# michael-fonder/M4Depth

Measured on AMD Instinct MI355X. Metric: frames/s, higher is better.
Workload: dtype f32

## Files before the change

include/m4depth_hip.h:

```cpp
#ifndef M4DEPTH_HIP_H_
#define M4DEPTH_HIP_H_

#include <stdint.h>

#ifdef __cplusplus
extern "C" {
#endif

#define M4D_ABI_VERSION 6

int m4d_abi_version(void);
long long m4d_launch_count(void);
const char* m4d_build_info(void);


int m4d_backproject_fwd(const float* input, const float* coords, const int dims[6],
                        float* out, void* stream);

int m4d_backproject_bwd(const float* grad, const float* input, const float* coords,
                        const int dims[6], float* input_grad, float* coords_grad, void* stream);


int m4d_dense_image_warp(const float* image, const float* flow, int B, int H, int W, int C,
                         float* out, int32_t* index_out, void* stream);

int m4d_interpolate_bilinear(const float* grid, const float* query, int B, int H, int W, int C,
                             int N, float* out, int32_t* index_out, void* stream);


int m4d_parallax2depth(const float* disp, const float* rot, int rot_c, const float* trans,
                       const float* cam_f, const float* cam_c, int b, int h, int w,
                       float* out, void* stream);
int m4d_depth2parallax(const float* depth, const float* rot, int rot_c, const float* trans,
                       const float* cam_f, const float* cam_c, int b, int h, int w,
                       float* out, void* stream);
int m4d_prev_d2para(const float* prev_d, const float* rot, int rot_c, const float* trans,
                    const float* cam_f, const float* cam_c, int b, int h, int w,
                    float* out, void* stream);
int m4d_reproject_flow(const float* depth, const float* rot, int rot_c, const float* trans,
                       const float* cam_f, const float* cam_c, int b, int h, int w,
                       float* flow, float* proj_minus_rot, float* rot_coord, void* stream);
int m4d_recompute_depth(const float* depth, const float* rot, int rot_c, const float* trans,
                        const float* cam_f, const float* cam_c, int b, int h, int w,
                        float* out, void* stream);


int m4d_dscv_fwd(const float* c1, const float* c2, const float* disp_prev_t, const float* disp,
                 const float* rot, int rot_c, const float* trans, const float* cam_f,
                 const float* cam_c, int b, int h, int w, int C, int search_range, int nbre_cuts,
                 int cv_accum, float* cv, int cv_stride, float* prev_disp,
                 float* log_center, int log_stride, float log_scale,
                 int32_t* index_out, void* stream);

void m4d_dscv_set_variant(int variant);
void m4d_dscv_set_fallback_counter(unsigned int* device_counter);
void m4d_dscv_set_ablation(int mask);
void m4d_dscv_set_stamps(unsigned long long* device_buffer);

int m4d_sncv_fwd(const float* c1, const float* c2, int b, int h, int w, int C, int search_range,
                 int dilation_rate, int nbre_cuts, float* out, int out_stride, void* stream);
int m4d_dscv_sncv_fwd(const float* c1, const float* c2, const float* disp_prev_t, const float* disp,
                      const float* rot, int rot_c, const float* trans, const float* cam_f,
                      const float* cam_c, int b, int h, int w, int C, int search_range, int nbre_cuts,
                      int cv_accum, float* cv, int cv_stride, float* prev_disp,
                      float* log_center, int log_stride, float log_scale,
                      int sncv_search_range, float* sncv_out, int sncv_out_stride, void* stream);

int m4d_conv3x3_wino_bias_act(const float* x, const float* wu, const float* bias, int b, int h, int w,
                              int Cin, int Cout, int CoutPad, float slope, float* out, void* stream);
int m4d_conv3x3_wino2_bias_act(const float* x, const float* wu8, const float* bias, int b, int h, int w,
                               int Cin, int Cout, int CoutPad, float slope, float* out, void* stream);
void m4d_wino_set_stamps(unsigned long long* device_buffer);
int m4d_conv3x3_wino6_bias_act(const float* x, const void* wu6, const float* bias, int b, int h, int w,
                               int Cin, int Cout, int CoutPad, float slope, float* out, void* stream);
int m4d_conv3x3_wino6_bias_act_k(const float* x, const void* wu6, const float* bias, int b, int h, int w,
                                 int Cin, int Cout, int CoutPad, float slope, float* out, int kernel, void* stream);
long long m4d_wino6_persistent_min_units(void);
void m4d_wino6_set_stamps(unsigned long long* device_buffer);
int m4d_conv3x3_wino6_bias_act_ks(const float* x, const void* wu6, const float* bias, int b, int h, int w,
                                  int Cin, int Cout, int CoutPad, float slope, float* out, int kernel,
                                  int stagger_us, int stagger_phases, void* stream);

int m4d_refiner_tail(const float* x32, const float* w6p, const float* b6, const float* w7p, const float* b7,
                     const float* rot, int rot_c, const float* trans, const float* cam_f, const float* cam_c,
                     int b, int h, int w, float scale, float* parallax, float* depth, float* other,
                     float* depth_state, void* stream);
int m4d_refiner_tail6(const float* x32, const void* w6f, const float* b6, const void* w7f, const float* b7,
                      const float* rot, int rot_c, const float* trans, const float* cam_f, const float* cam_c,
                      int b, int h, int w, float scale, float* parallax, float* depth, float* other,
                      float* depth_state, void* stream);

int m4d_refiner_tail6_m(const float* x32, const void* w6f, const float* b6, const void* w7f, const float* b7,
                        const float* rot, int rot_c, const float* trans, const float* cam_f, const float* cam_c,
                        int b, int h, int w, float scale, float* parallax, float* depth, float* other,
                        float* depth_state, const unsigned char* reset, float reset_parallax, void* stream);
int m4d_refiner_tail_m(const float* x32, const float* w6p, const float* b6, const float* w7p, const float* b7,
                       const float* rot, int rot_c, const float* trans, const float* cam_f, const float* cam_c,
                       int b, int h, int w, float scale, float* parallax, float* depth, float* other,
                       float* depth_state, const unsigned char* reset, float reset_parallax, void* stream);
int m4d_level_post_m(const float* refiner_out, const float* rot, int rot_c, const float* trans,
                     const float* cam_f, const float* cam_c, int b, int h, int w, float scale,
                     float* parallax, float* depth, float* other, float* depth_state,
                     const unsigned char* reset, float reset_parallax, void* stream);
int m4d_stream_prepare(const unsigned char* new_traj, int force_all, const float* rot, int rot_c, const float* trans,
                       int b, unsigned char* reset, float* rot_out, float* trans_out, void* stream);


int m4d_dscv_bwd(const float* c1, const float* c2, const float* disp_prev_t, const float* disp,
                 const float* rot, int rot_c, const float* trans, const float* cam_f,
                 const float* cam_c, int b, int h, int w, int C, int search_range, int nbre_cuts,
                 const float* g_cv, int g_cv_stride, const float* g_prev_disp,
                 float* g_c1, float* g_c2, float* g_disp, float* g_disp_prev_t, void* stream);

int m4d_sncv_bwd(const float* c1, const float* c2, const float* out, int out_stride,
                 const float* g, int g_stride, int b, int h, int w, int C, int search_range,
                 int dilation_rate, int nbre_cuts, float slope, float* g_c1, float* g_c2,
                 void* stream);


int m4d_resize_bilinear_v1_bwd(const float* g_out, int b, int ih, int iw, int c, int oh, int ow,
                               float mul, float* g_in, void* stream);
int m4d_level_post_bwd(const float* refiner_out, const float* g_parallax, const float* g_depth,
                       const float* g_other, const float* rot, int rot_c, const float* trans,
                       const float* cam_f, const float* cam_c, int b, int h, int w, float scale,
                       float* g_refiner_out, void* stream);
int m4d_normalize_cuts_bwd(const float* x, const float* g, int b, int h, int w, int C, int nbre_cuts,
                           float* g_x, void* stream);
long long m4d_bias_act_bwd_workspace_floats(long long rows, int C);
int m4d_bias_act_bwd(const float* g, const float* out, long long rows, int C, float slope,
                     float* g_pre, float* g_bias, float* workspace, void* stream);
int m4d_pack_conv_weights(const float* w_ohwi, int O, int I, int transpose, float* wp, void* stream);
int m4d_pack_conv_weights_lat(const float* w_ohwi, int O, int I, int transpose, void* wp, void* stream);
long long m4d_loss_workspace_floats(void);
int m4d_loss_level_fwd(const float* pred_depth, const float* gt_depth, int b, int h, int w, int H, int W,
                       int velodyne, float* workspace, float* out2, void* stream);
int m4d_loss_level_bwd(const float* pred_depth, const float* gt_depth, const float* stats2,
                       const float* g_out, int b, int h, int w, int H, int W, int velodyne,
                       float* g_pred, void* stream);


int m4d_normalize_cuts(const float* x, int b, int h, int w, int C, int nbre_cuts,
                       float* out, void* stream);

int m4d_resize_bilinear_v1(const float* x, int b, int ih, int iw, int c, int oh, int ow,
                           float mul, float* out, void* stream);
int m4d_resize_nearest(const float* x, int b, int ih, int iw, int c, int oh, int ow,
                       float* out, void* stream);

int m4d_level_pre(const float* prev_l_depth, const float* prev_l_parallax, const float* prev_l_other,
                  int ph, int pw, const float* depth_prev_t, const float* trans,
                  const float* cam_f, const float* cam_c, int b, int h, int w,
                  float* para_prev_l, float* depth_prev_l, float* other_prev_l, float* para_prev_t,
                  float* f_input, int f_stride, int log_off, int other_off, float log_scale,
                  float* depth_state_reset, void* stream);
int m4d_level_pre_normalize(const float* prev_l_depth, const float* prev_l_parallax, const float* prev_l_other,
                            int ph, int pw, const float* depth_prev_t, const float* trans,
                            const float* cam_f, const float* cam_c, int b, int h, int w,
                            float* para_prev_l, float* depth_prev_l, float* other_prev_l, float* para_prev_t,
                            float* f_input, int f_stride, int log_off, int other_off, float log_scale,
                            float* depth_state_reset,
                            const float* norm_x, int C, int nbre_cuts, float* norm_out, void* stream);

typedef struct m4d_reset_level {
  const float* features;
  float* state_features;
  float* depth_state;
  float* parallax;
  float* depth;
  float* other;
  int h, w, C, nbre_cuts;
  float parallax_value;
} m4d_reset_level;
int m4d_pyramid_reset_supported(int C, int nbre_cuts);
int m4d_pyramid_reset(const m4d_reset_level* levels, int n_levels, int b, void* stream);

typedef struct { const float* x; float* out; long long pixels; int C, nbre_cuts; } m4d_norm_level;
int m4d_normalize_levels(const m4d_norm_level* levels, int n_levels, void* stream);
int m4d_level_front_small_supported(int C, int nbre_cuts, int dscv_range, int sncv_range);
int m4d_level_front_small(const float* norm_f, const float* prev_f, const float* depth_prev_t,
                          const float* prev_l_parallax, const float* prev_l_other, int ph, int pw,
                          const float* rot, int rot_c, const float* trans, const float* cam_f, const float* cam_c,
                          int b, int h, int w, int C, int nbre_cuts, int dscv_range, int sncv_range, int cv_accum,
                          float* f_input, int f_stride, float log_scale, void* stream);

int m4d_level_front_supported(int C, int nbre_cuts, int dscv_range, int sncv_range, int f_stride);
void m4d_front_set_stamps(unsigned long long* device_buffer);
int m4d_level_front(const float* raw_f, float* norm_out, const float* prev_f, const float* depth_prev_t,
                    const float* prev_l_parallax, const float* prev_l_other, int ph, int pw,
                    const float* rot, int rot_c, const float* trans, const float* cam_f, const float* cam_c,
                    int b, int h, int w, int C, int nbre_cuts, int cv_accum,
                    float* f_input, int f_stride, float log_scale, void* stream);
int m4d_level_front_r(const float* raw_f, float* norm_out, const float* prev_f, const float* depth_prev_t,
                      const float* prev_l_parallax, const float* prev_l_other, int ph, int pw,
                      const float* rot, int rot_c, const float* trans, const float* cam_f, const float* cam_c,
                      int b, int h, int w, int C, int nbre_cuts, int dscv_range, int sncv_range, int cv_accum,
                      float* f_input, int f_stride, float log_scale, void* stream);

int m4d_camera_pyramid(const float* cam_f, const float* cam_c, int b, int levels, float* f_out, float* c_out,
                       void* stream);

int m4d_level_post(const float* refiner_out, const float* rot, int rot_c, const float* trans,
                   const float* cam_f, const float* cam_c, int b, int h, int w, float scale,
                   float* parallax, float* depth, float* other, float* depth_state, void* stream);

int m4d_bias_act(const float* x, const float* bias, long long rows, int C, float slope,
                 float* out, void* stream);

int m4d_bias_act_padded(const float* x, const float* bias, int b, int h, int w, int C, float slope,
                        float* out, int out_h, int out_w, int off_y, int off_x, void* stream);

int m4d_conv3x3_bias_act(const float* x, const float* wp, const float* bias, int b, int h, int w,
                         int Cin, int Cout, int CoutPad, float slope, float* out, void* stream);
long long m4d_conv3x3_workspace_floats(int b, int h, int w, int CoutPad);
int m4d_conv3x3s_bias_act_ws(const float* x, const float* wp, const float* bias, int b, int h, int w,
                             int Cin, int Cout, int CoutPad, int stride, float slope, float* out,
                             float* workspace, long long workspace_floats, void* stream);
int m4d_conv3x3_bias_act_ws(const float* x, const float* wp, const float* bias, int b, int h, int w,
                            int Cin, int Cout, int CoutPad, float slope, float* out, float* workspace,
                            long long workspace_floats, void* stream);
int m4d_conv3x3_lat(const float* x, int s_in, long long x_slab_floats, const float* x_bias, float x_slope,
                    const void* wp, const float* bias, int b, int h, int w, int Cin, int Cout, float slope,
                    int mt, int kw, int s_out, float* out, long long out_slab_floats, void* stream);
int m4d_conv3x3s_lat(const float* x, int s_in, long long x_slab_floats, const float* x_bias, float x_slope,
                     const void* wp, const float* bias, int b, int h, int w, int Cin, int Cout, int stride, float slope,
                     int mt, int kw, int s_out, float* out, long long out_slab_floats, void* stream);
int m4d_partial_finish(const float* x, int s_in, long long x_slab_floats, const float* bias, float slope,
                       long long pixels, int C, float* out, void* stream);

int m4d_conv3x3_small_bias_act(const float* x, const float* wp, const float* bias, int b, int h, int w,
                               int Cin, int Cout, int CoutPad, float slope, float* out, void* stream);
int m4d_conv3x3s_small_bias_act(const float* x, const float* wp, const float* bias, int b, int h, int w,
                                int Cin, int Cout, int CoutPad, int stride, float slope, float* out, void* stream);
int m4d_conv3x3_small6_bias_act(const float* x, const void* wp6, const float* bias, int b, int h, int w,
                                int Cin, int Cout, int CoutPad, float slope, float* out, void* stream);

long long m4d_dinl_workspace_floats(int b, int C);
int m4d_dinl_fwd_padded(const float* x, const float* scale, const float* bias, int b, int h, int w, int C,
                        float slope, float* workspace, float* out, int out_h, int out_w, int off_y,
                        int off_x, void* stream);
int m4d_dinl_fwd(const float* x, const float* scale, const float* bias, int b, int h, int w, int C,
                 float slope, float* workspace, float* out, void* stream);

int m4d_enc_level0_fwd(const float* images, int bsz, long long stride_b, long long stride_t,
                       const float* w1_hwio, const float* bias1, const float* dn_scale, const float* dn_bias,
                       float dn_slope, const float* w2_hwio, const float* bias2, float slope,
                       int b, int h, int w, float* workspace, float* out, void* stream);
int m4d_enc_level0_stats(const float* images, int bsz, long long stride_b, long long stride_t,
                         const float* w1_hwio, const float* bias1, int b, int h, int w, float* workspace,
                         float* mean, float* var, void* stream);
int m4d_enc_level0_apply(const float* images, int bsz, long long stride_b, long long stride_t,
                         const float* w1_hwio, const float* bias1, const float* mean, const float* var,
                         const float* dn_scale, const float* dn_bias, float dn_slope, const float* w2_hwio,
                         const float* bias2, float slope, int b, int h, int w, float* out, void* stream);
int m4d_enc_head_fwd(const float* images, int bsz, long long stride_b, long long stride_t,
                     const float* w_hwio, const float* bias, int b, int h, int w, int C,
                     float* workspace, float* raw_out, void* stream);
int m4d_conv3x3s2_dinl_bias_act(const float* x_raw, const float* mean, const float* var, const float* dn_scale,
                                const float* dn_bias, float dn_slope, const float* wp, const float* bias,
                                int b, int h, int w, int Cout, int CoutPad, float slope, float* out, void* stream);

long long m4d_metrics_workspace_bytes(void);
int m4d_depth_metrics(const float* gt, const float* est, long long n, float max_d, void* workspace,
                      float* out7, float* total7, float count, float* mean7, void* stream);
int m4d_depth_metrics_strided(const float* gt, long long per_image, long long gt_image_stride, const float* est,
                              long long n, float max_d, void* workspace, float* out7, float* total7, float count,
                              float* mean7, void* stream);


long long m4d_conv3x3_wgrad_workspace_floats(int b, int h, int w, int cin, int cout, int stride);
int m4d_conv3x3_wgrad(const float* x, const float* g, int b, int h, int w, int cin, int cout, int stride,
                      float* workspace, long long workspace_floats, float* dw, void* stream);
int m4d_dilate2(const float* g, int b, int oh, int ow, int C, int h, int w, float* out, void* stream);


int m4d_decode_rgb8_resize(const uint8_t* images, int n, int ih, int iw, int oh, int ow, float* out,
                           void* stream);
int m4d_decode_depth_resize(const void* raw, int kind, int n, int ih, int iw, int oh, int ow,
                            const float* rgb_resized, const int crop[4], float* out, void* stream);

#ifdef __cplusplus
}
#endif
#endif
```

m4depth_amd/_lib.py:

```python
from __future__ import annotations

import ctypes
import os

import torch

_HERE = os.path.dirname(os.path.abspath(__file__))
LIB_FLAVOUR = os.environ.get("M4D_LIB_FLAVOUR", "product")
LIB_PATH = os.path.join(_HERE, "libm4depth_hip_exp.so" if LIB_FLAVOUR == "experiments" else "libm4depth_hip.so")

ABI_VERSION = 6

_c_fp = ctypes.c_void_p
_c_int = ctypes.c_int
_c_f = ctypes.c_float

class NormLevel(ctypes.Structure):
    _fields_ = [("x", ctypes.c_void_p), ("out", ctypes.c_void_p), ("pixels", ctypes.c_longlong), ("C", ctypes.c_int),
                ("nbre_cuts", ctypes.c_int)]


class ResetLevel(ctypes.Structure):
    _fields_ = [("features", ctypes.c_void_p), ("state_features", ctypes.c_void_p), ("depth_state", ctypes.c_void_p),
                ("parallax", ctypes.c_void_p), ("depth", ctypes.c_void_p), ("other", ctypes.c_void_p),
                ("h", ctypes.c_int), ("w", ctypes.c_int), ("C", ctypes.c_int), ("nbre_cuts", ctypes.c_int),
                ("parallax_value", ctypes.c_float)]


_SIGNATURES = {
    "m4d_backproject_fwd": [_c_fp, _c_fp, ctypes.POINTER(_c_int), _c_fp, _c_fp],
    "m4d_backproject_bwd": [_c_fp, _c_fp, _c_fp, ctypes.POINTER(_c_int), _c_fp, _c_fp, _c_fp],
    "m4d_dense_image_warp": [_c_fp, _c_fp, _c_int, _c_int, _c_int, _c_int, _c_fp, _c_fp, _c_fp],
    "m4d_interpolate_bilinear": [_c_fp, _c_fp, _c_int, _c_int, _c_int, _c_int, _c_int, _c_fp, _c_fp, _c_fp],
    "m4d_parallax2depth": [_c_fp, _c_fp, _c_int, _c_fp, _c_fp, _c_fp, _c_int, _c_int, _c_int, _c_fp, _c_fp],
    "m4d_depth2parallax": [_c_fp, _c_fp, _c_int, _c_fp, _c_fp, _c_fp, _c_int, _c_int, _c_int, _c_fp, _c_fp],
    "m4d_prev_d2para": [_c_fp, _c_fp, _c_int, _c_fp, _c_fp, _c_fp, _c_int, _c_int, _c_int, _c_fp, _c_fp],
    "m4d_recompute_depth": [_c_fp, _c_fp, _c_int, _c_fp, _c_fp, _c_fp, _c_int, _c_int, _c_int, _c_fp, _c_fp],
    "m4d_reproject_flow": [_c_fp, _c_fp, _c_int, _c_fp, _c_fp, _c_fp, _c_int, _c_int, _c_int, _c_fp, _c_fp, _c_fp, _c_fp],
    "m4d_dscv_fwd": [_c_fp, _c_fp, _c_fp, _c_fp, _c_fp, _c_int, _c_fp, _c_fp, _c_fp,
                     _c_int, _c_int, _c_int, _c_int, _c_int, _c_int, _c_int,
                     _c_fp, _c_int, _c_fp, _c_fp, _c_int, _c_f, _c_fp, _c_fp],
    "m4d_dscv_sncv_fwd": [_c_fp, _c_fp, _c_fp, _c_fp, _c_fp, _c_int, _c_fp, _c_fp, _c_fp,
                          _c_int, _c_int, _c_int, _c_int, _c_int, _c_int, _c_int,
                          _c_fp, _c_int, _c_fp, _c_fp, _c_int, _c_f, _c_int, _c_fp, _c_int, _c_fp],
    "m4d_sncv_fwd": [_c_fp, _c_fp, _c_int, _c_int, _c_int, _c_int, _c_int, _c_int, _c_int, _c_fp, _c_int, _c_fp],
    "m4d_dscv_bwd": [_c_fp, _c_fp, _c_fp, _c_fp, _c_fp, _c_int, _c_fp, _c_fp, _c_fp,
                     _c_int, _c_int, _c_int, _c_int, _c_int, _c_int,
                     _c_fp, _c_int, _c_fp, _c_fp, _c_fp, _c_fp, _c_fp, _c_fp],
    "m4d_sncv_bwd": [_c_fp, _c_fp, _c_fp, _c_int, _c_fp, _c_int, _c_int, _c_int, _c_int, _c_int, _c_int, _c_int,
                     _c_int, _c_f, _c_fp, _c_fp, _c_fp],
    "m4d_resize_bilinear_v1_bwd": [_c_fp, _c_int, _c_int, _c_int, _c_int, _c_int, _c_int, _c_f, _c_fp, _c_fp],
    "m4d_level_post_bwd": [_c_fp, _c_fp, _c_fp, _c_fp, _c_fp, _c_int, _c_fp, _c_fp, _c_fp, _c_int, _c_int, _c_int, _c_f,
                           _c_fp, _c_fp],
    "m4d_normalize_cuts_bwd": [_c_fp, _c_fp, _c_int, _c_int, _c_int, _c_int, _c_int, _c_fp, _c_fp],
    "m4d_bias_act_bwd": [_c_fp, _c_fp, ctypes.c_longlong, _c_int, _c_f, _c_fp, _c_fp, _c_fp, _c_fp],
    "m4d_pack_conv_weights": [_c_fp, _c_int, _c_int, _c_int, _c_fp, _c_fp],
    "m4d_pack_conv_weights_lat": [_c_fp, _c_int, _c_int, _c_int, _c_fp, _c_fp],
    "m4d_loss_level_fwd": [_c_fp, _c_fp, _c_int, _c_int, _c_int, _c_int, _c_int, _c_int, _c_fp, _c_fp, _c_fp],
    "m4d_loss_level_bwd": [_c_fp, _c_fp, _c_fp, _c_fp, _c_int, _c_int, _c_int, _c_int, _c_int, _c_int, _c_fp, _c_fp],
    "m4d_decode_rgb8_resize": [_c_fp, _c_int, _c_int, _c_int, _c_int, _c_int, _c_fp, _c_fp],
    "m4d_decode_depth_resize": [_c_fp, _c_int, _c_int, _c_int, _c_int, _c_int, _c_int, _c_fp, ctypes.POINTER(_c_int),
                                _c_fp, _c_fp],
    "m4d_normalize_cuts": [_c_fp, _c_int, _c_int, _c_int, _c_int, _c_int, _c_fp, _c_fp],
    "m4d_resize_bilinear_v1": [_c_fp, _c_int, _c_int, _c_int, _c_int, _c_int, _c_int, _c_f, _c_fp, _c_fp],
    "m4d_resize_nearest": [_c_fp, _c_int, _c_int, _c_int, _c_int, _c_int, _c_int, _c_fp, _c_fp],
    "m4d_bias_act": [_c_fp, _c_fp, ctypes.c_longlong, _c_int, _c_f, _c_fp, _c_fp],
    "m4d_dinl_fwd": [_c_fp, _c_fp, _c_fp, _c_int, _c_int, _c_int, _c_int, _c_f, _c_fp, _c_fp, _c_fp],
    "m4d_dinl_fwd_padded": [_c_fp, _c_fp, _c_fp, _c_int, _c_int, _c_int, _c_int, _c_f, _c_fp, _c_fp,
                            _c_int, _c_int, _c_int, _c_int, _c_fp],
    "m4d_bias_act_padded": [_c_fp, _c_fp, _c_int, _c_int, _c_int, _c_int, _c_f, _c_fp, _c_int, _c_int, _c_int, _c_int, _c_fp],
    "m4d_conv3x3_bias_act": [_c_fp, _c_fp, _c_fp, _c_int, _c_int, _c_int, _c_int, _c_int, _c_int, _c_f, _c_fp, _c_fp],
    "m4d_conv3x3_bias_act_ws": [_c_fp, _c_fp, _c_fp, _c_int, _c_int, _c_int, _c_int, _c_int, _c_int, _c_f, _c_fp,
                                _c_fp, ctypes.c_longlong, _c_fp],
    "m4d_conv3x3s_bias_act_ws": [_c_fp, _c_fp, _c_fp, _c_int, _c_int, _c_int, _c_int, _c_int, _c_int, _c_int, _c_f,
                                 _c_fp, _c_fp, ctypes.c_longlong, _c_fp],
    "m4d_conv3x3_small_bias_act": [_c_fp, _c_fp, _c_fp, _c_int, _c_int, _c_int, _c_int, _c_int, _c_int, _c_f, _c_fp, _c_fp],
    "m4d_conv3x3s_small_bias_act": [_c_fp, _c_fp, _c_fp, _c_int, _c_int, _c_int, _c_int, _c_int, _c_int, _c_int, _c_f, _c_fp, _c_fp],
    "m4d_conv3x3_small6_bias_act": [_c_fp, _c_fp, _c_fp, _c_int, _c_int, _c_int, _c_int, _c_int, _c_int, _c_f, _c_fp, _c_fp],
    "m4d_conv3x3_lat": [_c_fp, _c_int, ctypes.c_longlong, _c_fp, _c_f, _c_fp, _c_fp, _c_int, _c_int, _c_int, _c_int, _c_int, _c_f,
                        _c_int, _c_int, _c_int, _c_fp, ctypes.c_longlong, _c_fp],
    "m4d_conv3x3s_lat": [_c_fp, _c_int, ctypes.c_longlong, _c_fp, _c_f, _c_fp, _c_fp, _c_int, _c_int, _c_int, _c_int, _c_int, _c_int,
                         _c_f, _c_int, _c_int, _c_int, _c_fp, ctypes.c_longlong, _c_fp],
    "m4d_partial_finish": [_c_fp, _c_int, ctypes.c_longlong, _c_fp, _c_f, ctypes.c_longlong, _c_int, _c_fp, _c_fp],
    "m4d_conv3x3_wino_bias_act": [_c_fp, _c_fp, _c_fp, _c_int, _c_int, _c_int, _c_int, _c_int, _c_int, _c_f, _c_fp, _c_fp],
    "m4d_conv3x3_wino2_bias_act": [_c_fp, _c_fp, _c_fp, _c_int, _c_int, _c_int, _c_int, _c_int, _c_int, _c_f, _c_fp, _c_fp],
    "m4d_conv3x3_wino6_bias_act": [_c_fp, _c_fp, _c_fp, _c_int, _c_int, _c_int, _c_int, _c_int, _c_int, _c_f, _c_fp, _c_fp],
    "m4d_conv3x3_wino6_bias_act_k": [_c_fp, _c_fp, _c_fp, _c_int, _c_int, _c_int, _c_int, _c_int, _c_int, _c_f, _c_fp, _c_int, _c_fp],
    "m4d_conv3x3_wino6_bias_act_ks": [_c_fp, _c_fp, _c_fp, _c_int, _c_int, _c_int, _c_int, _c_int, _c_int, _c_f, _c_fp, _c_int,
                                      _c_int, _c_int, _c_fp],
    "m4d_enc_head_fwd": [_c_fp, _c_int, ctypes.c_longlong, ctypes.c_longlong, _c_fp, _c_fp, _c_int, _c_int, _c_int, _c_int,
                         _c_fp, _c_fp, _c_fp],
    "m4d_enc_level0_stats": [_c_fp, _c_int, ctypes.c_longlong, ctypes.c_longlong, _c_fp, _c_fp, _c_int, _c_int, _c_int, _c_fp, _c_fp, _c_fp,
                             _c_fp],
    "m4d_enc_level0_apply": [_c_fp, _c_int, ctypes.c_longlong, ctypes.c_longlong, _c_fp, _c_fp, _c_fp, _c_fp, _c_fp, _c_fp, _c_f, _c_fp,
                             _c_fp, _c_f, _c_int, _c_int, _c_int, _c_fp, _c_fp],
    "m4d_enc_level0_fwd": [_c_fp, _c_int, ctypes.c_longlong, ctypes.c_longlong, _c_fp, _c_fp, _c_fp, _c_fp, _c_f, _c_fp, _c_fp, _c_f,
                           _c_int, _c_int, _c_int, _c_fp, _c_fp, _c_fp],
    "m4d_conv3x3s2_dinl_bias_act": [_c_fp, _c_fp, _c_fp, _c_fp, _c_fp, _c_f, _c_fp, _c_fp, _c_int, _c_int, _c_int, _c_int, _c_int,
                                    _c_f, _c_fp, _c_fp],
    "m4d_refiner_tail": [_c_fp, _c_fp, _c_fp, _c_fp, _c_fp, _c_fp, _c_int, _c_fp, _c_fp, _c_fp, _c_int, _c_int, _c_int, _c_f,
                         _c_fp, _c_fp, _c_fp, _c_fp, _c_fp],
    "m4d_refiner_tail6": [_c_fp, _c_fp, _c_fp, _c_fp, _c_fp, _c_fp, _c_int, _c_fp, _c_fp, _c_fp, _c_int, _c_int, _c_int, _c_f,
                          _c_fp, _c_fp, _c_fp, _c_fp, _c_fp],
    "m4d_depth_metrics": [_c_fp, _c_fp, ctypes.c_longlong, _c_f, _c_fp, _c_fp, _c_fp, _c_f, _c_fp, _c_fp],
    "m4d_depth_metrics_strided": [_c_fp, ctypes.c_longlong, ctypes.c_longlong, _c_fp, ctypes.c_longlong, _c_f, _c_fp, _c_fp, _c_fp,
                                  _c_f, _c_fp, _c_fp],
    "m4d_level_pre": [_c_fp, _c_fp, _c_fp, _c_int, _c_int, _c_fp, _c_fp, _c_fp, _c_fp, _c_int, _c_int, _c_int,
                      _c_fp, _c_fp, _c_fp, _c_fp, _c_fp, _c_int, _c_int, _c_int, _c_f, _c_fp, _c_fp],
    "m4d_level_pre_normalize": [_c_fp, _c_fp, _c_fp, _c_int, _c_int, _c_fp, _c_fp, _c_fp, _c_fp, _c_int, _c_int, _c_int,
                                _c_fp, _c_fp, _c_fp, _c_fp, _c_fp, _c_int, _c_int, _c_int, _c_f, _c_fp,
                                _c_fp, _c_int, _c_int, _c_fp, _c_fp],
    "m4d_level_front_supported": [_c_int, _c_int, _c_int, _c_int, _c_int],
    "m4d_pyramid_reset_supported": [_c_int, _c_int],
    "m4d_pyramid_reset": [ctypes.POINTER(ResetLevel), _c_int, _c_int, _c_fp],
    "m4d_normalize_levels": [ctypes.POINTER(NormLevel), _c_int, _c_fp],
    "m4d_level_front_small_supported": [_c_int, _c_int, _c_int, _c_int],
    "m4d_level_front_small": [_c_fp, _c_fp, _c_fp, _c_fp, _c_fp, _c_int, _c_int, _c_fp, _c_int, _c_fp, _c_fp, _c_fp,
                              _c_int, _c_int, _c_int, _c_int, _c_int, _c_int, _c_int, _c_int, _c_fp, _c_int, _c_f, _c_fp],
    "m4d_level_front": [_c_fp, _c_fp, _c_fp, _c_fp, _c_fp, _c_fp, _c_int, _c_int, _c_fp, _c_int, _c_fp, _c_fp, _c_fp,
                        _c_int, _c_int, _c_int, _c_int, _c_int, _c_int, _c_fp, _c_int, _c_f, _c_fp],
    "m4d_level_front_r": [_c_fp, _c_fp, _c_fp, _c_fp, _c_fp, _c_fp, _c_int, _c_int, _c_fp, _c_int, _c_fp, _c_fp, _c_fp,
                          _c_int, _c_int, _c_int, _c_int, _c_int, _c_int, _c_int, _c_int, _c_fp, _c_int, _c_f, _c_fp],
    "m4d_conv3x3_wgrad": [_c_fp, _c_fp, _c_int, _c_int, _c_int, _c_int, _c_int, _c_int, _c_fp, ctypes.c_longlong, _c_fp, _c_fp],
    "m4d_dilate2": [_c_fp, _c_int, _c_int, _c_int, _c_int, _c_int, _c_int, _c_fp, _c_fp],
    "m4d_camera_pyramid": [_c_fp, _c_fp, _c_int, _c_int, _c_fp, _c_fp, _c_fp],
    "m4d_level_post": [_c_fp, _c_fp, _c_int, _c_fp, _c_fp, _c_fp, _c_int, _c_int, _c_int, _c_f,
                       _c_fp, _c_fp, _c_fp, _c_fp, _c_fp],
    "m4d_refiner_tail_m": [_c_fp, _c_fp, _c_fp, _c_fp, _c_fp, _c_fp, _c_int, _c_fp, _c_fp, _c_fp, _c_int, _c_int, _c_int, _c_f,
                           _c_fp, _c_fp, _c_fp, _c_fp, _c_fp, _c_f, _c_fp],
    "m4d_refiner_tail6_m": [_c_fp, _c_fp, _c_fp, _c_fp, _c_fp, _c_fp, _c_int, _c_fp, _c_fp, _c_fp, _c_int, _c_int, _c_int, _c_f,
                            _c_fp, _c_fp, _c_fp, _c_fp, _c_fp, _c_f, _c_fp],
    "m4d_level_post_m": [_c_fp, _c_fp, _c_int, _c_fp, _c_fp, _c_fp, _c_int, _c_int, _c_int, _c_f,
                         _c_fp, _c_fp, _c_fp, _c_fp, _c_fp, _c_f, _c_fp],
    "m4d_stream_prepare": [_c_fp, _c_int, _c_fp, _c_int, _c_fp, _c_int, _c_fp, _c_fp, _c_fp, _c_fp],
}

_EXPERIMENT_SIGNATURES = {"m4d_tape_begin": [], "m4d_tape_end": [], "m4d_tape_length": [_c_int], "m4d_tape_replay": [_c_int, _c_fp],
                          "m4d_tape_free": [_c_int]}
_EXPERIMENT_VOID_SIGNATURES = {"m4d_wino6_set_variant": [_c_int], "m4d_wino6_set_half_tile_max_workgroups": [_c_int]}
EXPERIMENT_SYMBOLS = list(_EXPERIMENT_SIGNATURES) + list(_EXPERIMENT_VOID_SIGNATURES)

_LL_SIGNATURES = {"m4d_launch_count": [], "m4d_wino6_persistent_min_units": [], "m4d_conv3x3_workspace_floats": [_c_int, _c_int, _c_int, _c_int],
                  "m4d_dinl_workspace_floats": [_c_int, _c_int], "m4d_metrics_workspace_bytes": [],
                  "m4d_bias_act_bwd_workspace_floats": [ctypes.c_longlong, _c_int], "m4d_loss_workspace_floats": [],
                  "m4d_conv3x3_wgrad_workspace_floats": [_c_int, _c_int, _c_int, _c_int, _c_int, _c_int]}
_VOID_SIGNATURES = {"m4d_dscv_set_variant": [_c_int], "m4d_dscv_set_fallback_counter": [_c_fp],
                    "m4d_dscv_set_ablation": [_c_int], "m4d_dscv_set_stamps": [_c_fp], "m4d_wino_set_stamps": [_c_fp],
                    "m4d_front_set_stamps": [_c_fp], "m4d_wino6_set_stamps": [_c_fp]}

EXPORTED_SYMBOLS = ["m4d_abi_version", "m4d_build_info"] + list(_SIGNATURES) + list(_VOID_SIGNATURES) + list(_LL_SIGNATURES)


def _load():
    if not os.path.isfile(LIB_PATH):
        raise ImportError(
            f"m4depth_amd: native library not found at {LIB_PATH}. Build it with "
            "`python -c 'import __graft_entry__ as g; g.build()'` or `make -C m4depth_amd/csrc`. "
            "There is no CPU / PyTorch fallback for the hot path.")
    lib = ctypes.CDLL(LIB_PATH)
    lib.m4d_abi_version.restype = _c_int
    lib.m4d_abi_version.argtypes = []
    lib.m4d_build_info.restype = ctypes.c_char_p
    lib.m4d_build_info.argtypes = []
    for name, args in _SIGNATURES.items():
        fn = getattr(lib, name)
        fn.restype = _c_int
        fn.argtypes = args
    for name, args in _LL_SIGNATURES.items():
        fn = getattr(lib, name)
        fn.restype = ctypes.c_longlong
        fn.argtypes = args
    for name, args in _VOID_SIGNATURES.items():
        fn = getattr(lib, name)
        fn.restype = None
        fn.argtypes = args
    if hasattr(lib, "m4d_tape_begin"):
        for name, args in _EXPERIMENT_SIGNATURES.items():
            fn = getattr(lib, name)
            fn.restype = _c_int
            fn.argtypes = args
        for name, args in _EXPERIMENT_VOID_SIGNATURES.items():
            fn = getattr(lib, name)
            fn.restype = None
            fn.argtypes = args
    if lib.m4d_abi_version() != ABI_VERSION:
        raise ImportError(f"m4depth_amd: ABI mismatch, library reports {lib.m4d_abi_version()}, binding expects {ABI_VERSION}")
    return lib


lib = _load()
has_experiments = hasattr(lib, "m4d_tape_begin")


def require_experiments(what):
    if not has_experiments:
        raise RuntimeError(f"{what} needs the experiments build of the library: make -C m4depth_amd/csrc EXPERIMENTS=1 "
                           "(-> libm4depth_hip_exp.so, sources in tools/experiments/csrc) and M4D_LIB_FLAVOUR=experiments in "
                           "the environment; the product library exports only the kernels it dispatches")


def build_info() -> str:
    return lib.m4d_build_info().decode()


def stream_ptr():
    return ctypes.c_void_p(torch.cuda.current_stream().cuda_stream)


def dptr(t, name="tensor", dtype=torch.float32):
    if t is None:
        return None
    if not isinstance(t, torch.Tensor):
        raise TypeError(f"{name}: expected a torch.Tensor, got {type(t).__name__}")
    if not t.is_cuda:
        raise RuntimeError(f"{name}: m4depth_amd ops run on the MI355X only (tensor is on {t.device}); "
                           "there is no CPU fallback")
    if t.dtype != dtype:
        raise TypeError(f"{name}: expected dtype {dtype}, got {t.dtype}")
    if not t.is_contiguous():
        raise ValueError(f"{name}: expected a dense row-major (NHWC) tensor, got strides {t.stride()}")
    return ctypes.c_void_p(t.data_ptr())


def check(rc, what):
    if rc != 0:
        raise RuntimeError(f"m4depth_amd: {what} failed with HIP error {rc}"
                           + (" (hipErrorInvalidValue: bad argument)" if rc == 1 else ""))


_capture_copies_ok = [False]


class framework_copies_in_capture:
    def __enter__(self):
        self._old = _capture_copies_ok[0]
        _capture_copies_ok[0] = True
        return self

    def __exit__(self, *exc):
        _capture_copies_ok[0] = self._old
        return False


def as_f32(t, name):
    if not isinstance(t, torch.Tensor):
        raise TypeError(f"{name}: expected a torch.Tensor")
    if t.dtype == torch.float32 and t.is_contiguous():
        return t
    if t.is_cuda and not _capture_copies_ok[0] and torch.cuda.is_current_stream_capturing():
        raise RuntimeError(f"{name}: a non-contiguous / non-float32 tensor (shape {tuple(t.shape)}, strides {t.stride()}, "
                           f"{t.dtype}) reached a kernel wrapper inside a hipGraph capture; it would be copied by a framework "
                           "kernel inside the graph -- make it dense before capturing")
    if t.dtype != torch.float32:
        t = t.float()
    return t if t.is_contiguous() else t.contiguous()
```

m4depth_amd/network.py:

```python
from __future__ import annotations

import ctypes
from collections import namedtuple

import numpy as np
import torch

from . import network_ops as nops
from ._lib import lib, dptr, stream_ptr, check, as_f32
from .synthetic import ENCODER_CHANNELS, REFINER_CHANNELS, f_input_channels, nbre_cuts_for

M4depthAblationParameters = namedtuple('M4depthAblationParameters',
                                       ('DINL', 'SNCV', 'time_recurr', 'normalize_features',
                                        'subdivide_features', 'level_memory'),
                                       defaults=(True, True, True, True, True, True))

_CV_ACCUM = {"fp32_round": 0, "fp16_seq": 1}

import os as _os

kernel_timer = None
debug_tap = None
winograd_conv = _os.environ.get("M4D_WINOGRAD", "1") == "1"


winograd2_min_workgroups = int(_os.environ.get("M4D_WINO2_MIN_WG", "60"))


conv_arith = _os.environ.get("M4D_CONV_ARITH", "bf16x3")
wino6_min_workgroups = int(_os.environ.get("M4D_WINO6_MIN_WG", "30"))
wino6_kernel = int(_os.environ.get("M4D_WINO6_KERNEL", "0"))
wino6_pair_min_units = int(_os.environ.get("M4D_WINO6_PAIR_MIN_UNITS", "0"))
wino6_pair_units = int(_os.environ.get("M4D_WINO6_PAIR_UNITS", "2"))
wino6_min_cout = int(_os.environ.get("M4D_WINO6_MIN_COUT", "32"))
if _os.environ.get("M4D_WINO6_VARIANT") or _os.environ.get("M4D_WINO6_HALF_MAX_WG"):
    from ._lib import require_experiments as _require_experiments
    _require_experiments("M4D_WINO6_VARIANT / M4D_WINO6_HALF_MAX_WG")
    if _os.environ.get("M4D_WINO6_VARIANT"):
        lib.m4d_wino6_set_variant(int(_os.environ["M4D_WINO6_VARIANT"]))
    if _os.environ.get("M4D_WINO6_HALF_MAX_WG"):
        lib.m4d_wino6_set_half_tile_max_workgroups(int(_os.environ["M4D_WINO6_HALF_MAX_WG"]))
_small_conv_split_env = _os.environ.get("M4D_SMALL_CONV_SPLIT", "1") == "1"
small_conv_split = _small_conv_split_env and conv_arith == "bf16x3"


tail_split = _os.environ.get("M4D_TAIL_SPLIT", "1") == "1"

encoder_batch_dispatch = _os.environ.get("M4D_ENCODER_BATCH_DISPATCH", "1") == "1"

import contextlib as _contextlib


@_contextlib.contextmanager
def conv_arithmetic(arith):
    global conv_arith, small_conv_split
    if arith not in ("bf16x3", "f32"):
        raise ValueError(f"conv arithmetic must be 'bf16x3' or 'f32', not {arith!r}")
    old = (conv_arith, small_conv_split)
    conv_arith, small_conv_split = arith, _small_conv_split_env and arith == "bf16x3"
    try:
        yield
    finally:
        conv_arith, small_conv_split = old


def _use_winograd(b, h, w, cin, cout, stride):
    if not winograd_conv or stride != 1 or cin < 16 or cin % 2 != 0:
        return 0
    n32 = -(-cout // 32)
    t16 = b * (-(-h // 16)) * (-(-w // 16))
    if conv_arith == "bf16x3" and cin % 16 == 0 and cin >= 32 and cout >= wino6_min_cout and t16 * (-(-cout // 64)) >= wino6_min_workgroups:
        return 6
    if cin % 4 == 0 and t16 * n32 >= winograd2_min_workgroups:
        return 2
    t8 = b * (-(-h // 8)) * (-(-w // 16))
    if cout % 64 == 0 and t8 * (cout // 64) >= 400:
        return 1
    if cout >= 96 and 400 <= t8 * n32 <= 3000:
        return 1
    return 0


pad_refiner_input = _os.environ.get("M4D_PAD_REFINER_INPUT", "1") == "1"

small_map_conv_pixels = int(_os.environ.get("M4D_CONV_SMALL_PX", "2048"))
small_map_stride2 = _os.environ.get("M4D_CONV_SMALL_S2", "1") == "1"

lat_conv_max_pixels = int(_os.environ.get("M4D_LAT_CONV_PX", "2048"))
lat_conv_narrow_max_pixels = int(_os.environ.get("M4D_LAT_CONV_NARROW_PX", "0"))
lat_conv_s2_max_pixels = int(_os.environ.get("M4D_LAT_CONV_S2_PX", "0"))
lat_conv_mw_max_pixels = int(_os.environ.get("M4D_LAT_CONV_MW_PX", "0"))

fused_cost_volumes = _os.environ.get("M4D_FUSED_COST_VOLUMES", "1") == "1"
small_level_front = _os.environ.get("M4D_SMALL_LEVEL_FRONT", "1") == "1"
fused_level_front = _os.environ.get("M4D_FUSED_LEVEL_FRONT", "1") == "1"

fused_front = _os.environ.get("M4D_FUSED_FRONT", "1") == "1"
fused_front_min_pixels = int(_os.environ.get("M4D_FUSED_FRONT_MIN_PX", "0"))
fused_front_coarse_min_pixels = int(_os.environ.get("M4D_FUSED_FRONT_COARSE_MIN_PX", "6000"))

fused_encoder_head = _os.environ.get("M4D_FUSED_ENCODER_HEAD", "1") == "1"

fused_refiner_tail = _os.environ.get("M4D_FUSED_TAIL", "1") == "1"

level_pipeline_streams = int(_os.environ.get("M4D_LEVEL_PIPELINE", "8"))
_pf = _os.environ.get("M4D_PIPE_FORK_FRAMES", "1,2")
pipeline_fork_frames = None if _pf == "all" else {int(v) for v in _pf.split(",") if v.strip() != ""}
pipeline_skip_implied_encoder_wait = _os.environ.get("M4D_PIPE_SKIP_ENC_WAIT", "1") == "1"
pipeline_merge_reset_frame = _os.environ.get("M4D_PIPE_MERGE_RESET", "1") == "1"
wino6_stagger_us = int(_os.environ.get("M4D_WINO6_STAGGER_US", "9"))
wino6_stagger_phases = int(_os.environ.get("M4D_WINO6_STAGGER_PHASES", "16"))
wino6_stagger_min_wg = int(_os.environ.get("M4D_WINO6_STAGGER_MIN_WG", "200"))
wino6_stagger_max_batch = int(_os.environ.get("M4D_WINO6_STAGGER_MAX_BATCH", "4"))
wino6_stagger_autotune = _os.environ.get("M4D_STAGGER_AUTOTUNE", "1") == "1"
segmented_step = _os.environ.get("M4D_SEGMENTED", "0") == "1"
segmented_resumed_first = _os.environ.get("M4D_SEG_RESUMED_FIRST", "1") == "1"
segmented_resumed_on_main = _os.environ.get("M4D_SEG_RESUMED_ON_MAIN", "0") == "1"
wino6_stagger_force = _os.environ.get("M4D_STAGGER_FORCE", "")
fused_pyramid_reset = _os.environ.get("M4D_FUSED_RESET", "1") == "1"
fused_encoder_level0 = _os.environ.get("M4D_FUSED_ENC0", "1") == "1"
pipeline_encoder_per_frame = _os.environ.get("M4D_PIPELINE_ENCODER", "0") == "1"
pipeline_encoder_split = int(_os.environ.get("M4D_PIPELINE_ENCODER_SPLIT", "2"))
encoder_stats_up_front = _os.environ.get("M4D_ENC_STATS_UP_FRONT", "1") == "1"
encoder_s1_partial_always = _os.environ.get("M4D_ENC_S1_PARTIAL", "0") == "1"


def _stack_frames(samples):
    ims = [s['RGB_im'] for s in samples]
    x0 = ims[0]
    if (x0.is_cuda and x0.dtype == torch.float32 and x0.dim() == 4 and x0[0].is_contiguous()
            and all(x.dtype == x0.dtype and x.shape == x0.shape and x.stride() == x0.stride()
                    and x.untyped_storage().data_ptr() == x0.untyped_storage().data_ptr() for x in ims)):
        if len(ims) == 1:
            return nops.FrameStack(x0.unsqueeze(1))
        st = ims[1].storage_offset() - x0.storage_offset()
        if st > 0 and all(ims[t].storage_offset() - x0.storage_offset() == t * st for t in range(len(ims))):
            b, h, w, c = x0.shape
            return nops.FrameStack(torch.as_strided(x0, (b, len(ims), h, w, c), (x0.stride(0), st, w * c, c, 1),
                                                    x0.storage_offset()))
    return torch.cat([as_f32(x, "RGB_im") for x in ims], dim=0)


def _timed(name, level, thunk):
    kt = kernel_timer
    return thunk() if kt is None else kt.run(name, level, thunk)


def _to_device_f32(x, device):
    if isinstance(x, torch.Tensor):
        return x.to(device=device, dtype=torch.float32)
    return torch.as_tensor(np.asarray(x), dtype=torch.float32, device=device)


def _stamp(*params):
    return tuple((p.data_ptr(), p._version, str(p.device)) for p in params)


class _PackCache:

    def __init__(self):
        self.entries = {}

    def get(self, key, stamp, build):
        hit = self.entries.get(key)
        if hit is not None and hit[0] == stamp:
            return hit[1]
        if torch.cuda.is_available() and torch.cuda.is_current_stream_capturing():
            raise RuntimeError("packed convolution weights are missing or stale inside a hipGraph capture: call "
                               "M4Depth.prepack() before capturing")
        fresh = build()
        if hit is not None:
            old = hit[1]
            olds, news = (old if isinstance(old, tuple) else (old,)), (fresh if isinstance(fresh, tuple) else (fresh,))
            if len(olds) == len(news) and all(isinstance(o, torch.Tensor) == isinstance(n, torch.Tensor) and (
                    not isinstance(o, torch.Tensor) or (o.shape == n.shape and o.device == n.device)) for o, n in zip(olds, news)):
                for o, n in zip(olds, news):
                    if isinstance(o, torch.Tensor):
                        o.copy_(n)
                fresh = old
        self.entries[key] = (stamp, fresh)
        return fresh

    def clear(self):
        self.entries.clear()


class _Conv3x3SameTF(torch.nn.Module):

    def __init__(self, out_channels, stride, in_channels=None):
        super().__init__()
        self.out_channels = out_channels
        self.stride = stride
        self.weight = None
        self.bias = None
        self._cache = _PackCache()
        self.tag = None
        self.small_maps_ok = False
        self.per_image_dispatch = False
        self.dispatch_batch = 1
        self.wino6_stagger_us = None
        if in_channels is not None:
            self._build(in_channels, None)

    def _build(self, in_channels, device):
        w = torch.empty(self.out_channels, in_channels, 3, 3, device=device)
        torch.nn.init.kaiming_normal_(w, nonlinearity='relu')
        self.weight = torch.nn.Parameter(w.contiguous(memory_format=torch.channels_last), requires_grad=False)
        self.bias = torch.nn.Parameter(torch.zeros(self.out_channels, device=device), requires_grad=False)
        self._cache.clear()

    def load_hwio(self, kernel, bias, device):
        w = _to_device_f32(kernel, device).permute(3, 2, 0, 1)
        b = _to_device_f32(bias, device).contiguous()
        if (self.weight is not None and self.bias is not None and self.weight.shape == w.shape and self.bias.shape == b.shape
                and self.weight.device == w.device):
            with torch.no_grad():
                self.weight.copy_(w)
                self.bias.copy_(b)
            return
        self.weight = torch.nn.Parameter(w.contiguous(memory_format=torch.channels_last), requires_grad=False)
        self.bias = torch.nn.Parameter(b, requires_grad=False)
        self._cache.clear()

    def invalidate_packed(self):
        with torch.no_grad():
            if self.weight is not None:
                self.weight.add_(0)

    def _hwio_numpy(self, cin_pad=None):
        hwio = self.weight.detach().permute(2, 3, 1, 0).cpu().numpy()
        if cin_pad is not None and cin_pad > hwio.shape[2]:
            hwio = np.concatenate([hwio, np.zeros(hwio.shape[:2] + (cin_pad - hwio.shape[2], hwio.shape[3]), hwio.dtype)], axis=2)
        return hwio

    def _packed_weights(self, cin_pad=None):
        if cin_pad is not None and cin_pad == self.weight.shape[1]:
            cin_pad = None

        def build():
            wp, cpad = nops.pack_conv_weights(self._hwio_numpy(cin_pad))
            return torch.from_numpy(wp).to(self.weight.device), cpad
        return self._cache.get(("direct", cin_pad), _stamp(self.weight), build)

    def _packed_weights_winograd(self, chunk=16, cin_pad=None):
        if cin_pad is not None and cin_pad == self.weight.shape[1]:
            cin_pad = None

        def build():
            wu, cpad = nops.pack_conv_weights_winograd(self._hwio_numpy(cin_pad), chunk=chunk)
            return torch.from_numpy(wu).to(self.weight.device), cpad
        return self._cache.get(("wino", chunk, cin_pad), _stamp(self.weight), build)

    def _packed_weights_small6(self, cin_pad=None):
        if cin_pad is not None and cin_pad == self.weight.shape[1]:
            cin_pad = None

        def build():
            wp, cpad = nops.pack_conv_weights_small6(self._hwio_numpy(cin_pad))
            return torch.from_numpy(wp.view("int16")).to(self.weight.device), cpad
        return self._cache.get(("small6", cin_pad), _stamp(self.weight), build)

    def _packed_weights_lat(self, cin_pad=None):
        if cin_pad is not None and cin_pad == self.weight.shape[1]:
            cin_pad = None

        def build():
            wp = nops.pack_conv_weights_lat(self._hwio_numpy(cin_pad))
            return torch.from_numpy(wp.view("int16")).to(self.weight.device)
        return self._cache.get(("lat", cin_pad), _stamp(self.weight), build)

    def lat_eligible(self, b, h, w, cin):
        if not (self.small_maps_ok and conv_arith == "bf16x3" and cin >= 16 and cin % 4 == 0 and self.stride in (1, 2)):
            return False
        eff_b = self.dispatch_batch if self.per_image_dispatch else b
        if self.stride == 2:
            opx = eff_b * (-(-h // 2)) * (-(-w // 2))
            return self._lat_mw(b, h, w, cin) or (small_map_stride2 and opx <= lat_conv_s2_max_pixels)
        limit = max(lat_conv_max_pixels, lat_conv_narrow_max_pixels) if self.out_channels <= 32 else lat_conv_max_pixels
        return eff_b * h * w <= limit

    def _lat_mw(self, b, h, w, cin):
        eff_b = self.dispatch_batch if self.per_image_dispatch else b
        return (self.stride == 2 and cin % 16 == 0 and cin <= 64 and self.out_channels <= 64
                and small_map_conv_pixels < eff_b * (-(-h // 2)) * (-(-w // 2)) <= lat_conv_mw_max_pixels)

    def _packed_weights_wino6(self, cin_pad=None):
        if cin_pad is not None and cin_pad == self.weight.shape[1]:
            cin_pad = None

        def build():
            wu, cpad = nops.pack_conv_weights_wino6(self._hwio_numpy(cin_pad))
            return torch.from_numpy(wu.view("int16")).to(self.weight.device), cpad
        return self._cache.get(("wino6", cin_pad), _stamp(self.weight), build)

    def _hwio_device(self):
        return self._cache.get(("hwio",), _stamp(self.weight), lambda: self.weight.detach().permute(2, 3, 1, 0).contiguous())

    def same_pads(self, h, w):
        s = self.stride
        ph = max((-(-h // s) - 1) * s + 3 - h, 0)
        pw = max((-(-w // s) - 1) * s + 3 - w, 0)
        return (ph // 2, ph - ph // 2), (pw // 2, pw - pw // 2)

    def launch_stagger_us(self, b, h, w):
        us = wino6_stagger_us if self.wino6_stagger_us is None else self.wino6_stagger_us
        if us <= 0 or b > wino6_stagger_max_batch:
            return 0
        units = b * (-(-h // 16)) * (-(-w // 16)) * (-(-self.out_channels // 64))
        return int(us) if units >= wino6_stagger_min_wg else 0

    def forward(self, x_nhwc, slope=None, final=True):
        if isinstance(x_nhwc, nops.PartialAct) and not self.lat_eligible(*x_nhwc.shape):
            x_nhwc = x_nhwc.dense()
        if not x_nhwc.is_cuda:
            raise RuntimeError("m4depth_amd convolutions run on the GPU only (libm4depth_hip.so): got a CPU tensor; "
                               "there is no CPU fallback")
        if self.weight is None:
            self._build(x_nhwc.shape[-1], x_nhwc.device)
        if self.stride not in (1, 2):
            raise ValueError(f"stride {self.stride} is not supported by the HIP convolution")
        b_, h_, w_, cin_ = x_nhwc.shape
        act = 1.0 if slope is None else slope
        eff_b = self.dispatch_batch if self.per_image_dispatch else b_
        if self.lat_eligible(b_, h_, w_, cin_):
            wl = self._packed_weights_lat(cin_)
            cfg = nops.lat_config(eff_b, h_, w_, cin_, self.out_channels, final, self.stride, mw=self._lat_mw(b_, h_, w_, cin_))
            return _timed("conv", self.tag, lambda: nops.conv3x3_lat(x_nhwc, wl, self.bias, self.out_channels, act, config=cfg,
                                                                     stride=self.stride))
        wino = _use_winograd(eff_b, h_, w_, cin_, self.out_channels, self.stride)
        if wino == 6:
            wu, cpad = self._packed_weights_wino6(cin_)
            stag = self.launch_stagger_us(b_, h_, w_)
            kern = wino6_kernel
            if kern == 0 and wino6_pair_min_units > 0 and b_ <= wino6_stagger_max_batch and cin_ >= 32:
                units = b_ * (-(-h_ // 16)) * (-(-w_ // 16)) * (cpad // 64)
                if wino6_pair_min_units <= units < int(lib.m4d_wino6_persistent_min_units()):
                    kern = 16 + max(1, min(wino6_pair_units, 15))
            return _timed("conv", self.tag, lambda: nops.conv3x3_wino6_bias_act(
                x_nhwc, wu, self.bias, self.out_channels, cpad, act, kernel=kern, stagger_us=stag,
                stagger_phases=wino6_stagger_phases))
        if wino:
            wu, cpad = self._packed_weights_winograd(16 if wino == 1 else 8, cin_)
            fn = nops.conv3x3_wino_bias_act if wino == 1 else nops.conv3x3_wino2_bias_act
            return _timed("conv", self.tag, lambda: fn(x_nhwc, wu, self.bias, self.out_channels, cpad, act))
        wp, cpad = self._packed_weights(cin_)
        if (self.small_maps_ok and self.stride == 1 and eff_b * h_ * w_ <= small_map_conv_pixels and 16 <= cin_ <= 256
                and cin_ % 4 == 0):
            if small_conv_split:
                wp6, cpad6 = self._packed_weights_small6(cin_)
                return _timed("conv", self.tag, lambda: nops.conv3x3_small6_bias_act(
                    x_nhwc, wp6, self.bias, self.out_channels, cpad6, act))
            return _timed("conv", self.tag, lambda: nops.conv3x3_small_bias_act(
                x_nhwc, wp, self.bias, self.out_channels, cpad, act))
        if (self.small_maps_ok and self.stride == 2 and small_map_stride2 and 16 <= cin_ <= 256 and cin_ % 4 == 0
                and eff_b * (-(-h_ // 2)) * (-(-w_ // 2)) <= small_map_conv_pixels):
            return _timed("conv", self.tag, lambda: nops.conv3x3_small_bias_act(
                x_nhwc, wp, self.bias, self.out_channels, cpad, act, stride=2))
        return _timed("conv", self.tag, lambda: nops.conv3x3_bias_act(
            x_nhwc, wp, self.bias, self.out_channels, cpad, act, stride=self.stride))


class DomainNormalization(torch.nn.Module):

    def __init__(self, regularizer_weight=0.0004):
        super().__init__()
        self.regularizer_weight = regularizer_weight
        self.scale = None
        self.bias = None

    def _build(self, channels, device):
        self.scale = torch.nn.Parameter(torch.ones(1, 1, 1, channels, device=device), requires_grad=False)
        self.bias = torch.nn.Parameter(torch.zeros(1, 1, 1, channels, device=device), requires_grad=False)

    def forward(self, f_map, slope=1.0):
        if self.scale is None:
            self._build(f_map.shape[-1], f_map.device)
        if not f_map.is_cuda:
            raise RuntimeError("m4depth_amd DomainNormalization runs on the GPU only (libm4depth_hip.so): got a CPU tensor; "
                               "there is no CPU fallback")
        if f_map.shape[-1] not in (16, 32):
            raise ValueError(f"DomainNormalization: the HIP kernel is instantiated for 16 and 32 channels, not {f_map.shape[-1]}")
        return nops.dinl_act(f_map, self.scale, self.bias, slope)


class FeaturePyramid(torch.nn.Module):

    def __init__(self, settings, regularizer_weight=0.0004, trainable=True):
        super().__init__()
        self.use_dinl = settings["ablation"].DINL
        self.out_sizes = ENCODER_CHANNELS[:settings["nbre_lvls"]]
        cin = [3] + self.out_sizes[:-1]
        self.conv_layers_s1 = torch.nn.ModuleList([_Conv3x3SameTF(n, 1, ci) for n, ci in zip(self.out_sizes, cin)])
        self.conv_layers_s2 = torch.nn.ModuleList([_Conv3x3SameTF(n, 2, n) for n in self.out_sizes])
        self.dn_layers = torch.nn.ModuleList([DomainNormalization(regularizer_weight) for _ in self.out_sizes])
        for conv in list(self.conv_layers_s1) + list(self.conv_layers_s2):
            conv.per_image_dispatch = True
            conv.small_maps_ok = True

    def set_sequence_batch(self, b):
        b = max(int(b), 1) if encoder_batch_dispatch else 1
        for conv in list(self.conv_layers_s1) + list(self.conv_layers_s2):
            conv.dispatch_batch = b

    def _head_ok(self, images):
        return (self.use_dinl and fused_encoder_head and images.is_cuda and images.shape[-1] == 3
                and self.conv_layers_s1[0].out_channels == 16 and self.conv_layers_s2[0].out_channels <= 32
                and self.conv_layers_s1[0].weight is not None)

    def head_stats(self, images):
        if not (self._head_ok(images) and fused_encoder_level0 and self.conv_layers_s2[0].out_channels == 16):
            return None
        conv_s1 = self.conv_layers_s1[0]
        return _timed("enc0_stats", 0, lambda: nops.encoder_level0_stats(images, conv_s1._hwio_device(), conv_s1.bias))

    def forward(self, images, head_stats=None):
        head_ok = self._head_ok(images)
        if isinstance(images, nops.FrameStack):
            feature_maps = images if head_ok else images.dense()
        else:
            feature_maps = as_f32(images, "images")
        outputs = []
        for i, (conv_s1, conv_s2, dn_layer) in enumerate(zip(self.conv_layers_s1, self.conv_layers_s2, self.dn_layers)):
            if i == 0 and head_ok:
                if dn_layer.scale is None:
                    dn_layer._build(16, feature_maps.device)
                if fused_encoder_level0 and conv_s2.out_channels == 16:
                    feature_maps = _timed("enc0", 0, lambda: nops.encoder_level0(
                        feature_maps, conv_s1._hwio_device(), conv_s1.bias, dn_layer.scale, dn_layer.bias,
                        conv_s2._hwio_device(), conv_s2.bias, 0.1, stats=head_stats))
                    outputs.append(feature_maps)
                    continue
                wp2, cpad2 = conv_s2._packed_weights()
                feature_maps = nops.encoder_head(feature_maps, conv_s1._hwio_device(), conv_s1.bias, dn_layer.scale, dn_layer.bias,
                                                 wp2, conv_s2.bias, conv_s2.out_channels, cpad2, 0.1)
                outputs.append(feature_maps)
                continue
            if self.use_dinl and i == 0:
                tmp = dn_layer(conv_s1(feature_maps), slope=0.1)
            else:
                fb, fh, fw = feature_maps.shape[:3]
                takes_slabs = conv_s2.lat_eligible(fb, fh, fw, conv_s1.out_channels)
                tmp = conv_s1(feature_maps, slope=0.1, final=not (takes_slabs or encoder_s1_partial_always))
            feature_maps = conv_s2(tmp, slope=0.1)
            outputs.append(feature_maps)
        return outputs


class DispRefiner(torch.nn.Module):

    def __init__(self, regularizer_weight=0.0004, in_channels=None):
        super().__init__()
        chans = REFINER_CHANNELS
        cin = [in_channels] + chans[:-1]
        self.prep_conv_layers = torch.nn.ModuleList([_Conv3x3SameTF(n, 1, ci) for n, ci in zip(chans[:3], cin[:3])])
        self.est_d_conv_layers = torch.nn.ModuleList([_Conv3x3SameTF(n, 1, ci) for n, ci in zip(chans[3:], cin[3:])])
        for conv in list(self.prep_conv_layers) + list(self.est_d_conv_layers):
            conv.small_maps_ok = True

    def forward(self, feature_map):
        prev_out = feature_map
        for conv in self.prep_conv_layers:
            prev_out = conv(prev_out, slope=0.1)
        prep = prev_out
        n = len(self.est_d_conv_layers)
        for i, conv in enumerate(self.est_d_conv_layers):
            prev_out = conv(prev_out, slope=0.1 if i < n - 1 else None, final=(i == n - 1))
        return [prev_out, prep]


class DepthEstimatorLevel(torch.nn.Module):

    def __init__(self, settings, depth, regularizer_weight=0.0004):
        super().__init__()
        self.is_training = settings["is_training"]
        self.ablation = settings["ablation"]
        self.dscv_range = int(settings.get("dscv_range", 4))
        self.sncv_range = int(settings.get("sncv_range", 3))
        self.cv_accum = settings.get("cv_accum", "fp32_round")
        self.lvl_depth = depth
        self.lvl_mul = depth - 3
        self.nbre_cuts = nbre_cuts_for(depth, self.ablation.subdivide_features)
        self.f_in = f_input_channels(self.nbre_cuts, self.dscv_range, self.sncv_range,
                                     self.ablation.level_memory, self.ablation.SNCV, self.ablation.time_recurr)
        self.disp_refiner = DispRefiner(regularizer_weight=regularizer_weight, in_channels=self.f_in)
        for i, conv in enumerate(list(self.disp_refiner.prep_conv_layers) + list(self.disp_refiner.est_d_conv_layers)):
            conv.tag = f"lvl{depth}.conv{i}"
        self.prev_f_maps = None
        self.depth_prev_t = None
        self._own = None
        self.last_f_input = None
        self.last_cv_inputs = None
        self.last_front_inputs = None

    def _ensure_state(self, shape, device):
        if self._own is None or tuple(self._own[0].shape) != tuple(shape) or self._own[0].device != device:
            b, h, w, c = shape
            self._own = [torch.zeros(shape, dtype=torch.float32, device=device), torch.empty(shape, dtype=torch.float32, device=device)]
            self.prev_f_maps = self._own[0]
            self.depth_prev_t = torch.ones((b, h, w, 1), dtype=torch.float32, device=device)

    @property
    def _spare_f(self):
        if self._own is None:
            return None
        return self._own[1] if self.prev_f_maps is self._own[0] else self._own[0]

    def reset_state(self):
        self.prev_f_maps = None
        self.depth_prev_t = None
        self._own = None

    def reset_job(self, curr_f_maps):
        if self.is_training or not fused_level_front or not self.ablation.normalize_features:
            return None
        if not isinstance(curr_f_maps, torch.Tensor) or not curr_f_maps.is_cuda or curr_f_maps.dim() != 4:
            return None
        b, h, w, c = curr_f_maps.shape
        if not lib.m4d_pyramid_reset_supported(c, self.nbre_cuts):
            return None
        self._ensure_state((b, h, w, c), curr_f_maps.device)
        return {"features": curr_f_maps, "cuts": self.nbre_cuts, "state_features": self._spare_f, "depth_state": self.depth_prev_t}

    def reset_commit(self):
        self.prev_f_maps = self._spare_f

    def _tail_weights(self, convs, split=False):
        def build():
            k6 = convs[5].weight.detach().permute(2, 3, 1, 0).cpu().numpy()
            k7 = convs[6].weight.detach().permute(2, 3, 1, 0).cpu().numpy()
            w6, w7 = nops.pack_refiner_tail_weights(k6, k7)
            dev = convs[5].weight.device
            return torch.from_numpy(w6).to(dev), torch.from_numpy(w7).to(dev)
        def build6():
            k6 = convs[5].weight.detach().permute(2, 3, 1, 0).cpu().numpy()
            k7 = convs[6].weight.detach().permute(2, 3, 1, 0).cpu().numpy()
            w6, w7 = nops.pack_refiner_tail_weights6(k6, k7)
            dev = convs[5].weight.device
            return torch.from_numpy(w6.view("int16")).to(dev), torch.from_numpy(w7.view("int16")).to(dev)
        if getattr(self, "_tail_cache", None) is None:
            self._tail_cache = _PackCache()
        if split:
            return self._tail_cache.get("tail6", _stamp(convs[5].weight, convs[6].weight), build6)
        return self._tail_cache.get("tail", _stamp(convs[5].weight, convs[6].weight), build)

    def _vector_processing(self, f_map, out=None):
        if self.ablation.normalize_features:
            return nops.normalize_cuts(f_map, self.nbre_cuts, out=out)
        if out is not None:
            out.copy_(f_map)
            return out
        return f_map

    def _front_by_size(self, b, h, w, c):
        k = self.nbre_cuts
        F_st = (self.f_in + 7) // 8 * 8 if pad_refiner_input else self.f_in
        return (fused_front and b * h * w > (fused_front_min_pixels if k <= 2 else max(fused_front_min_pixels, fused_front_coarse_min_pixels))
                and bool(lib.m4d_level_front_supported(c, k, self.dscv_range, self.sncv_range, F_st)))

    def wants_prenormalized(self, b, h, w, c):
        ab = self.ablation
        return (small_level_front and fused_cost_volumes and fused_level_front and not self.is_training
                and ab.SNCV and ab.time_recurr and ab.normalize_features and ab.level_memory
                and b * h * w <= 6000 and not self._front_by_size(b, h, w, c)
                and bool(lib.m4d_pyramid_reset_supported(c, self.nbre_cuts))
                and bool(lib.m4d_level_front_small_supported(c, self.nbre_cuts, self.dscv_range, self.sncv_range)))

    def forward(self, curr_f_maps, prev_l_est, rot, trans, camera, new_traj, prev_f_maps=None, prev_t_depth=None,
                curr_f_normalized=None, reset_mask=None, reset_parallax=None):
        curr_f_maps = as_f32(curr_f_maps, "curr_f_maps")
        b, h, w, c = curr_f_maps.shape
        dev = curr_f_maps.device
        k = self.nbre_cuts
        if reset_mask is not None and (self.is_training or prev_f_maps is not None or prev_t_depth is not None):
            raise RuntimeError("DepthEstimatorLevel: a reset mask is for inference on the level's own state (not training mode)")
        use_state = (not self.is_training) and prev_f_maps is None and prev_t_depth is None
        if not self.is_training:
            self._ensure_state((b, h, w, c), dev)
        nt = new_traj
        if reset_mask is not None:
            nt = False
        elif isinstance(nt, torch.Tensor):
            nt = bool(nt.reshape(-1)[0].item())
        elif not isinstance(nt, bool):
            nt = bool(np.asarray(nt).reshape(-1)[0])
        ab = self.ablation
        F_in = self.f_in
        F_st = (F_in + 7) // 8 * 8 if (pad_refiner_input and dev.type == "cuda" and not self.is_training) else F_in
        use_front = (fused_front and use_state and not nt and dev.type == "cuda" and self._spare_f is not None
                     and ab.SNCV and ab.time_recurr and ab.normalize_features and ab.level_memory
                     and b * h * w > (fused_front_min_pixels if k <= 2 else max(fused_front_min_pixels, fused_front_coarse_min_pixels))
                     and bool(lib.m4d_level_front_supported(c, k, self.dscv_range, self.sncv_range, F_st)))
        use_small = (curr_f_normalized is not None and not use_front and use_state and not nt and dev.type == "cuda"
                     and kernel_timer_allows_small_front() and self.wants_prenormalized(b, h, w, c)
                     and tuple(curr_f_normalized.shape) == (b, h, w, c))
        norm_job = None
        if use_front:
            curr_f = self._spare_f
        elif use_small:
            curr_f = as_f32(curr_f_normalized, "curr_f_normalized")
        elif (fused_level_front and self.ablation.normalize_features and dev.type == "cuda" and not self.is_training
                and prev_f_maps is None and self._spare_f is not None and c % self.nbre_cuts == 0):
            curr_f = self._spare_f
            norm_job = (curr_f_maps, self.nbre_cuts, curr_f)
        else:
            curr_f = self._vector_processing(curr_f_maps, out=self._spare_f if not self.is_training else None)
        if prev_f_maps is not None:
            prev_f_maps = self._vector_processing(as_f32(prev_f_maps, "prev_f_maps"))
        if use_state:
            prev_t_depth = self.depth_prev_t
            prev_f_maps = self.prev_f_maps

        if prev_t_depth is None or nt:
            para_prev_l, depth_prev_l, other_prev_l, _ = _timed("pre", "reset", lambda: nops.level_pre(
                prev_l_est, None, None, None, b, h, w, dev, normalize=norm_job,
                depth_state_reset=None if self.is_training else self.depth_prev_t))
            if not self.is_training:
                self.prev_f_maps = curr_f
            return {"depth": depth_prev_l, "parallax": para_prev_l, "other": other_prev_l}

        r = self.dscv_range
        ncp = 2 * r + 1
        if F_st != F_in:
            f_buf = nops.zeroed_workspace(("f_input", self.lvl_depth), (b, h, w, F_st), dev)
        else:
            f_buf = torch.empty((b, h, w, F_in), dtype=torch.float32, device=dev)
        f_input = f_buf
        log_off = ncp * k
        other_off = log_off + 1 if self.ablation.level_memory else -1
        sncv_off = log_off + 1 + (4 if self.ablation.level_memory else 0)
        scale = float(2.0 ** self.lvl_mul)
        if not use_front and not use_small:
            para_prev_l, depth_prev_l, other_prev_l, para_prev_t = _timed("pre", self.lvl_depth, lambda: nops.level_pre(
                prev_l_est, as_f32(prev_t_depth, "prev_t_depth"), trans, camera, b, h, w, dev,
                f_input=f_input, log_off=log_off, other_off=other_off, log_scale=scale, normalize=norm_job))
        rot_t = as_f32(rot, "rot")
        tr = as_f32(trans, "trans").reshape(b, 3)
        cf = as_f32(camera["f"], "camera['f']").reshape(b, 2)
        cc = as_f32(camera["c"], "camera['c']").reshape(b, 2)
        if rot_t.dim() != 2 or rot_t.shape[1] not in (3, 4):
            raise ValueError('Rotation must be expressed as a small angle (x,y,z) or a quaternion (w,x,y,z)')
        fin_ptr = f_input.data_ptr()
        time_recurr = self.ablation.time_recurr
        log_ptr = ctypes.c_void_p(fin_ptr + 4 * (F_in - 1)) if time_recurr else None
        prev_f = as_f32(prev_f_maps, "prev_f_maps")
        kt_on = kernel_timer is not None and getattr(kernel_timer, "enabled", True)
        if use_front:
            pp = po = None
            ph = pw = 0
            if prev_l_est is not None:
                pp = as_f32(prev_l_est["parallax"], "prev_l_est['parallax']")
                po = as_f32(prev_l_est["other"], "prev_l_est['other']")
                ph, pw = pp.shape[1:3]
            check(_timed("front", self.lvl_depth, lambda: lib.m4d_level_front_r(
                dptr(curr_f_maps, "curr_f_maps"), dptr(curr_f), dptr(prev_f), dptr(as_f32(prev_t_depth, "prev_t_depth")),
                dptr(pp), dptr(po), ph, pw, dptr(rot_t), rot_t.shape[1], dptr(tr), dptr(cf), dptr(cc),
                b, h, w, c, k, self.dscv_range, self.sncv_range, _CV_ACCUM[self.cv_accum], ctypes.c_void_p(fin_ptr), F_st, scale,
                stream_ptr())), "m4d_level_front_r")
            para_prev_t = para_prev_l = None
        elif use_small:
            pp = po = None
            ph = pw = 0
            if prev_l_est is not None:
                pp = as_f32(prev_l_est["parallax"], "prev_l_est['parallax']")
                po = as_f32(prev_l_est["other"], "prev_l_est['other']")
                ph, pw = pp.shape[1:3]
            check(_timed("dscv_sncv", self.lvl_depth, lambda: lib.m4d_level_front_small(
                dptr(curr_f), dptr(prev_f), dptr(as_f32(prev_t_depth, "prev_t_depth")), dptr(pp), dptr(po), ph, pw,
                dptr(rot_t), rot_t.shape[1], dptr(tr), dptr(cf), dptr(cc), b, h, w, c, k, self.dscv_range, self.sncv_range,
                _CV_ACCUM[self.cv_accum], ctypes.c_void_p(fin_ptr), F_st, scale, stream_ptr())), "m4d_level_front_small")
            para_prev_t = para_prev_l = None
        elif fused_cost_volumes and self.ablation.SNCV and dev.type == "cuda" and b * h * w <= 6000:
            check(_timed("dscv_sncv", self.lvl_depth, lambda: lib.m4d_dscv_sncv_fwd(
                dptr(curr_f), dptr(prev_f), dptr(para_prev_t), dptr(para_prev_l), dptr(rot_t), rot_t.shape[1],
                dptr(tr), dptr(cf), dptr(cc), b, h, w, c, r, k, _CV_ACCUM[self.cv_accum], ctypes.c_void_p(fin_ptr),
                F_st, None, log_ptr, F_st, scale, self.sncv_range, ctypes.c_void_p(fin_ptr + 4 * sncv_off), F_st,
                stream_ptr())), "m4d_dscv_sncv_fwd")
        else:
            check(_timed("dscv", self.lvl_depth, lambda: lib.m4d_dscv_fwd(
                dptr(curr_f), dptr(prev_f), dptr(para_prev_t), dptr(para_prev_l), dptr(rot_t), rot_t.shape[1],
                dptr(tr), dptr(cf), dptr(cc), b, h, w, c, r, k, _CV_ACCUM[self.cv_accum], ctypes.c_void_p(fin_ptr),
                F_st, None, log_ptr, F_st, scale, None, stream_ptr())), "m4d_dscv_fwd")
            if self.ablation.SNCV:
                check(_timed("sncv", self.lvl_depth, lambda: lib.m4d_sncv_fwd(
                    dptr(curr_f), dptr(curr_f), b, h, w, c, self.sncv_range, 1, k,
                    ctypes.c_void_p(fin_ptr + 4 * sncv_off), F_st, stream_ptr())), "m4d_sncv_fwd")
        self.last_f_input = f_input if F_st == F_in else f_input[..., :F_in]
        self.last_cv_inputs = (curr_f, prev_f, para_prev_t, para_prev_l, rot_t, tr, cf, cc)
        self.last_front_inputs = (curr_f_maps, prev_l_est, prev_t_depth)
        if debug_tap is not None:
            debug_tap("encoder_map", self.lvl_depth, curr_f_maps)
            debug_tap("f_input", self.lvl_depth, self.last_f_input)
        mask_kw = {} if reset_mask is None else {"reset": reset_mask, "reset_parallax": float(reset_parallax)}
        convs = list(self.disp_refiner.prep_conv_layers) + list(self.disp_refiner.est_d_conv_layers)
        if (fused_refiner_tail and dev.type == "cuda" and len(convs) == 7 and convs[5].weight is not None
                and tuple(convs[5].weight.shape[:2]) == (16, 32) and tuple(convs[6].weight.shape[:2]) == (5, 16)):
            x = f_input
            for ci, conv in enumerate(convs[:5]):
                x = conv(x, slope=0.1, final=(ci == 4))
                if debug_tap is not None:
                    debug_tap(f"refiner_conv{ci + 1}", self.lvl_depth, x.dense() if isinstance(x, nops.PartialAct) else x)
            split = tail_split and conv_arith == "bf16x3"
            w6p, w7p = self._tail_weights(convs, split)
            tail_fn = nops.refiner_tail6 if split else nops.refiner_tail
            para_curr_l, depth, other = _timed("tail", self.lvl_depth, lambda: tail_fn(
                x, w6p, convs[5].bias, w7p, convs[6].bias, rot_t, tr, {"f": cf, "c": cc}, scale,
                depth_state=self.depth_prev_t if not self.is_training else None, **mask_kw))
        else:
            prev_out = self.disp_refiner(f_input)
            para_curr_l, depth, other = _timed("post", self.lvl_depth, lambda: nops.level_post(
                prev_out[0], rot_t, tr, {"f": cf, "c": cc}, scale, depth_state=self.depth_prev_t if not self.is_training else None,
                **mask_kw))
        if not self.is_training:
            self.prev_f_maps = curr_f
        return {"other": other, "depth": depth, "parallax": para_curr_l}


def kernel_timer_allows_small_front():
    return True


class DepthEstimatorPyramid(torch.nn.Module):

    def __init__(self, settings, regularizer_weight=0.0004, trainable=True):
        super().__init__()
        self.levels = torch.nn.ModuleList(
            [DepthEstimatorLevel(settings, i + 1, regularizer_weight=regularizer_weight)
             for i in range(settings["nbre_lvls"])])
        self.is_training = settings["is_training"]
        self.is_unsupervised = False

    def prenormalize(self, pyr, bsz):
        if self.is_training or pyr is None or not isinstance(pyr[0], torch.Tensor) or not pyr[0].is_cuda:
            return None
        jobs = [(lvl, t) for lvl, t in enumerate(pyr[:len(self.levels)])
                if t.dim() == 4 and self.levels[lvl].wants_prenormalized(bsz, t.shape[1], t.shape[2], t.shape[3])]
        if not jobs:
            return None
        outs = _timed("norm", "levels", lambda: nops.normalize_levels([(t, self.levels[lvl].nbre_cuts) for lvl, t in jobs]))
        res = [None] * len(pyr)
        for (lvl, _), o in zip(jobs, outs):
            res[lvl] = o
        return res

    @staticmethod
    def _frame_slice(npyr, j, bsz):
        return None if npyr is None else [None if t is None else t[j * bsz:(j + 1) * bsz] for t in npyr]

    def pipeline_streams_for(self, traj_samples, dev):
        n_streams = level_pipeline_streams if (dev.type == "cuda" and not self.is_training and len(traj_samples) > 1
                                               and not (kernel_timer is not None and getattr(kernel_timer, "enabled", True))) else 0
        if n_streams < 2:
            return 0
        frames = len(traj_samples)
        if frames <= n_streams:
            return frames
        return 0 if torch.cuda.is_current_stream_capturing() else n_streams

    def forward(self, f_maps_pyrs, traj_samples, camera, training=False, encoder=None, n_maps_pyrs=None):
        d_est_seq = []
        n_lvls = len(self.levels)
        dev = camera["f"].device
        if isinstance(camera["f"], torch.Tensor) and camera["f"].is_cuda:
            local_cameras = nops.camera_pyramid(camera, n_lvls)
        else:
            local_cameras = [{"f": camera["f"] / 2. ** (lvl + 1), "c": camera["c"] / 2. ** (lvl + 1)}
                             for lvl in range(n_lvls)]
        n_pipe = self.pipeline_streams_for(traj_samples, dev)
        if n_pipe >= 2:
            return self._forward_pipelined(f_maps_pyrs, traj_samples, local_cameras, n_pipe, encoder, n_maps_pyrs)
        if f_maps_pyrs is None:
            f_maps_pyrs = [encoder(sample['RGB_im']) for sample in traj_samples]
        if n_maps_pyrs is None:
            n_maps_pyrs = [None] * len(f_maps_pyrs)
        for seq_i, (f_pyr_curr, sample) in enumerate(zip(f_maps_pyrs, traj_samples)):
            rot = sample['rot']
            trans = sample['trans']
            cnter = float(n_lvls)
            d_est_curr = None
            fused = self._reset_all_levels(f_pyr_curr, sample["new_traj"])
            if fused is not None:
                d_est_seq.append(fused[::-1])
                continue
            for l in range(n_lvls):
                lvl = n_lvls - 1 - l
                f_maps_curr, level = f_pyr_curr[lvl], self.levels[lvl]
                f_maps_prev = None
                d_est_prev = None
                if self.is_training and seq_i != 0:
                    f_maps_prev = f_maps_pyrs[seq_i - 1][-l - 1]
                    d_est_prev = d_est_seq[-1][-l - 1]["depth"]
                local_camera = local_cameras[lvl]
                d_est = None if d_est_curr is None else dict(d_est_curr[-1])
                if l == 0 and n_maps_pyrs[seq_i] is None and not self.is_training:
                    n_maps_pyrs[seq_i] = self.prenormalize(f_pyr_curr, f_pyr_curr[0].shape[0])
                n_curr = None if n_maps_pyrs[seq_i] is None else n_maps_pyrs[seq_i][lvl]
                est = level(f_maps_curr, d_est, rot, trans, local_camera, sample["new_traj"],
                            prev_f_maps=f_maps_prev, prev_t_depth=d_est_prev, curr_f_normalized=n_curr)
                d_est_curr = [est] if d_est_curr is None else d_est_curr + [est]
                cnter -= 1.
            d_est_seq.append(d_est_curr[::-1])
        return d_est_seq

    def _reset_all_levels(self, f_pyr, new_traj):
        if not fused_pyramid_reset or self.is_training:
            return None
        nt = new_traj
        if isinstance(nt, torch.Tensor):
            nt = bool(nt.reshape(-1)[0].item())
        elif not isinstance(nt, bool):
            nt = bool(np.asarray(nt).reshape(-1)[0])
        if not nt or not isinstance(f_pyr[0], torch.Tensor) or not f_pyr[0].is_cuda:
            return None
        order = list(range(len(self.levels) - 1, -1, -1))
        jobs = [self.levels[lvl].reset_job(as_f32(f_pyr[lvl], "curr_f_maps")) for lvl in order]
        if any(j is None for j in jobs):
            return None
        ests = _timed("pre", "reset", lambda: nops.pyramid_reset(jobs, jobs[0]["features"].shape[0]))
        for lvl in order:
            self.levels[lvl].reset_commit()
        return ests

    def ensure_stream_state(self, f_pyr):
        fresh = False
        for lvl, level in enumerate(self.levels):
            before = level._own
            level._ensure_state(tuple(f_pyr[lvl].shape), f_pyr[lvl].device)
            fresh = fresh or level._own is not before
        return fresh

    def stream_forward(self, f_pyr, sample, local_cameras, reset_mask):
        if self.is_training:
            raise RuntimeError("stream_forward is inference only: the model is in training mode")
        n_lvls = len(self.levels)
        self.ensure_stream_state(f_pyr)
        bsz = f_pyr[0].shape[0]
        jobs = [lvl for lvl in range(n_lvls)
                if self.levels[lvl].wants_prenormalized(bsz, f_pyr[lvl].shape[1], f_pyr[lvl].shape[2], f_pyr[lvl].shape[3])]
        n_curr = [None] * n_lvls
        if jobs:
            outs = _timed("norm", "levels", lambda: nops.normalize_levels(
                [(f_pyr[lvl], self.levels[lvl].nbre_cuts) for lvl in jobs], outs=[self.levels[lvl]._spare_f for lvl in jobs]))
            for lvl, o in zip(jobs, outs):
                n_curr[lvl] = o
        ests = []
        pv = 1.0
        for lvl in range(n_lvls - 1, -1, -1):
            d_est = None if not ests else dict(ests[-1])
            ests.append(self.levels[lvl](f_pyr[lvl], d_est, sample["rot"], sample["trans"], local_cameras[lvl], None,
                                         curr_f_normalized=n_curr[lvl], reset_mask=reset_mask, reset_parallax=pv))
            pv *= 2.0
        return ests[::-1]

    def _forward_pipelined(self, f_maps_pyrs, traj_samples, local_cameras, n_streams, encoder=None, n_maps_pyrs=None,
                           resume=None):
        n_lvls = len(self.levels)
        main = torch.cuda.current_stream()
        if getattr(self, "_streams", None) is None or len(self._streams) < n_streams:
            self._streams = [torch.cuda.Stream() for _ in range(n_streams)]
        streams = self._streams[:n_streams]
        keep = []
        fork = torch.cuda.Event()
        fork.record(main)
        keep.append(fork)
        n_fr = len(traj_samples)
        ran = set() if resume is None else {(f, l) for f, ests in resume.items() for l in range(len(ests))}

        def is_reset(f):
            nt = traj_samples[f]["new_traj"]
            return bool(nt.reshape(-1)[0].item()) if isinstance(nt, torch.Tensor) else bool(np.asarray(nt).reshape(-1)[0])
        stream_of = list(range(n_fr))
        if resume is not None and segmented_resumed_on_main:
            stream_of = [-1 if 0 < len(resume.get(f, [])) < n_lvls else f for f in range(n_fr)]
        if pipeline_merge_reset_frame and resume is None:
            for f in range(n_fr - 1):
                if is_reset(f) and not is_reset(f + 1):
                    stream_of[f] = f + 1

        def launches_encoder(f):
            return f_maps_pyrs is None or (f_maps_pyrs[f] is None and (f == 0 or f_maps_pyrs[f - 1] is not None))

        def needs_fork(i_st):
            hosted = [f for f in range(n_fr) if stream_of[f] % n_streams == i_st]
            if resume is not None:
                return True
            if i_st == 0 or i_st >= n_fr or f_maps_pyrs is None:
                return True
            if any(f == 0 or launches_encoder(f) for f in hosted):
                return True
            return pipeline_fork_frames is None or i_st in pipeline_fork_frames
        active = [i_st for i_st in range(len(streams))
                  if resume is None or any((f, l) not in ran for f in range(n_fr)
                                           if stream_of[f] >= 0 and stream_of[f] % n_streams == i_st for l in range(n_lvls))]
        for i_st in active:
            if needs_fork(i_st):
                streams[i_st].wait_event(fork)
        done = {}
        late_encoder = None
        n_pyrs = list(n_maps_pyrs) if n_maps_pyrs is not None else [None] * n_fr
        f_pyrs = [None] * n_fr if resume is None else list(f_maps_pyrs)
        d_est = [None] * n_fr
        if resume is not None:
            for f, ests in resume.items():
                d_est[f] = list(ests)
        order = [(seq_i, diag - seq_i) for diag in range(n_fr + n_lvls - 1)
                 for seq_i in range(max(0, diag - n_lvls + 1), min(n_fr, diag + 1))]

        if pipeline_merge_reset_frame:
            merged = [f for f in range(n_fr) if stream_of[f] != f and f == 0]
            order = [(f, l) for f in merged for l in range(n_lvls)] + [(f, l) for (f, l) in order if f not in merged]
        fused_reset_frames = set()
        order = [cell for cell in order if cell not in ran]
        if resume is not None and segmented_resumed_first:
            part = {f for f in resume if 0 < len(resume[f]) < n_lvls}
            order = [c for c in order if c[0] in part] + [c for c in order if c[0] not in part]
        for seq_i, l in order:
            lvl = n_lvls - 1 - l
            sample = traj_samples[seq_i]
            st = main if stream_of[seq_i] < 0 else streams[stream_of[seq_i] % n_streams]
            with torch.cuda.stream(st):
                if l == 0:
                    if f_maps_pyrs is None:
                        f_pyrs[seq_i] = encoder(sample['RGB_im'])
                        n_pyrs[seq_i] = self.prenormalize(f_pyrs[seq_i], sample['RGB_im'].shape[0])
                    elif f_maps_pyrs[seq_i] is not None:
                        f_pyrs[seq_i] = f_maps_pyrs[seq_i]
                    elif f_pyrs[seq_i] is None:
                        rest = [i for i in range(seq_i, n_fr) if f_maps_pyrs[i] is None]
                        bsz = sample['RGB_im'].shape[0]
                        tail = encoder(_stack_frames([traj_samples[i] for i in rest]))
                        ntail = self.prenormalize(tail, bsz)
                        for j, i in enumerate(rest):
                            f_pyrs[i] = [lvl[j * bsz:(j + 1) * bsz] for lvl in tail]
                            n_pyrs[i] = self._frame_slice(ntail, j, bsz)
                        enc_done = torch.cuda.Event()
                        enc_done.record(st)
                        keep.append(enc_done)
                        late_encoder = (seq_i, enc_done)
                    elif not (pipeline_skip_implied_encoder_wait and seq_i - 1 >= late_encoder[0]):
                        st.wait_event(late_encoder[1])
                if seq_i > 0 and stream_of[seq_i - 1] != stream_of[seq_i] and (seq_i - 1, l) not in ran:
                    st.wait_event(done[(seq_i - 1, lvl)])
                if l == 0 and seq_i == 0:
                    fused = self._reset_all_levels(f_pyrs[seq_i], sample["new_traj"])
                    if fused is not None:
                        d_est[seq_i] = fused
                        ev = torch.cuda.Event()
                        ev.record(st)
                        for any_lvl in range(n_lvls):
                            done[(seq_i, any_lvl)] = ev
                        fused_reset_frames.add(seq_i)
                if seq_i in fused_reset_frames:
                    continue
                prev = None if d_est[seq_i] is None else dict(d_est[seq_i][-1])
                est = self.levels[lvl](f_pyrs[seq_i][lvl], prev, sample['rot'], sample['trans'], local_cameras[lvl],
                                       sample["new_traj"],
                                       curr_f_normalized=None if n_pyrs[seq_i] is None else n_pyrs[seq_i][lvl])
                ev = torch.cuda.Event()
                ev.record(st)
                done[(seq_i, lvl)] = ev
                d_est[seq_i] = [est] if d_est[seq_i] is None else d_est[seq_i] + [est]
        d_est_seq = [ests[::-1] for ests in d_est]
        for st in (streams[i_st] for i_st in active):
            ev = torch.cuda.Event()
            ev.record(st)
            main.wait_event(ev)
            keep.append(ev)
        keep.extend(done.values())
        self._events = keep
        if not torch.cuda.is_current_stream_capturing():
            for ests in d_est_seq:
                for est in ests:
                    for t in est.values():
                        t.record_stream(main)
        return d_est_seq


class M4Depth(torch.nn.Module):

    def __init__(self, depth_type="map", nbre_levels=6, is_training=False, ablation_settings=None,
                 dscv_range=4, sncv_range=3, cv_accum="fp32_round"):
        super().__init__()
        self.ablation_settings = M4depthAblationParameters() if ablation_settings is None else ablation_settings
        self.model_settings = {
            "nbre_lvls": nbre_levels,
            "is_training": is_training,
            "ablation": self.ablation_settings,
            "dscv_range": dscv_range,
            "sncv_range": sncv_range,
            "cv_accum": cv_accum,
        }
        self.depth_type = depth_type
        self.encoder = FeaturePyramid(self.model_settings, regularizer_weight=0.)
        self.d_estimator = DepthEstimatorPyramid(self.model_settings, regularizer_weight=0.)
        self.step_counter = 0
        self.compiled_metrics = []
        self.last_estimates = None
        self.wino6_stagger_us = None

    def load_numpy_weights(self, weights, device):
        for i in range(self.model_settings["nbre_lvls"]):
            self.encoder.conv_layers_s1[i].load_hwio(weights[f"enc.s1.{i}.kernel"], weights[f"enc.s1.{i}.bias"], device)
            self.encoder.conv_layers_s2[i].load_hwio(weights[f"enc.s2.{i}.kernel"], weights[f"enc.s2.{i}.bias"], device)
        dn = self.encoder.dn_layers[0]
        sc = _to_device_f32(weights["enc.dn.0.scale"], device).reshape(1, 1, 1, -1)
        bi = _to_device_f32(weights["enc.dn.0.bias"], device).reshape(1, 1, 1, -1)
        if dn.scale is not None and dn.scale.shape == sc.shape and dn.scale.device == sc.device:
            with torch.no_grad():
                dn.scale.copy_(sc)
                dn.bias.copy_(bi)
        else:
            dn.scale = torch.nn.Parameter(sc, requires_grad=False)
            dn.bias = torch.nn.Parameter(bi, requires_grad=False)
        for lvl in self.d_estimator.levels:
            convs = list(lvl.disp_refiner.prep_conv_layers) + list(lvl.disp_refiner.est_d_conv_layers)
            for i, conv in enumerate(convs):
                conv.load_hwio(weights[f"lvl.{lvl.lvl_depth}.conv.{i}.kernel"], weights[f"lvl.{lvl.lvl_depth}.conv.{i}.bias"], device)
        return self.prepack()

    def prepack(self):
        for conv in self.modules():
            if isinstance(conv, _Conv3x3SameTF) and conv.weight is not None and conv.weight.is_cuda:
                cin = conv.weight.shape[1]
                conv._packed_weights()
                if small_conv_split and conv.small_maps_ok and conv.stride == 1 and 16 <= cin <= 256 and cin % 4 == 0:
                    conv._packed_weights_small6()
                if conv.small_maps_ok and conv_arith == "bf16x3" and cin >= 16 and cin % 4 == 0 and (
                        (conv.stride == 1 and max(lat_conv_max_pixels, lat_conv_narrow_max_pixels) > 0)
                        or (conv.stride == 2 and max(lat_conv_s2_max_pixels, lat_conv_mw_max_pixels) > 0)):
                    conv._packed_weights_lat()
                if cin == 3 or (conv.stride == 2 and cin == 16 and conv.out_channels == 16):
                    conv._hwio_device()
                if conv.stride == 1 and cin >= 16 and cin % 2 == 0:
                    conv._packed_weights_winograd(16)
                    if cin % 4 == 0:
                        conv._packed_weights_winograd(8)
                    if cin % 16 == 0 and cin >= 32 and conv.out_channels >= min(wino6_min_cout, 32):
                        conv._packed_weights_wino6()
        for lvl in self.d_estimator.levels:
            convs = list(lvl.disp_refiner.prep_conv_layers) + list(lvl.disp_refiner.est_d_conv_layers)
            c0 = convs[0] if convs else None
            if pad_refiner_input and c0 is not None and c0.weight is not None and c0.weight.is_cuda and c0.weight.shape[1] % 8 != 0:
                cin_pad = (c0.weight.shape[1] + 7) // 8 * 8
                c0._packed_weights(cin_pad)
                c0._packed_weights_winograd(16, cin_pad)
                c0._packed_weights_winograd(8, cin_pad)
                if small_conv_split and cin_pad <= 256:
                    c0._packed_weights_small6(cin_pad)
                if conv_arith == "bf16x3" and lat_conv_max_pixels > 0:
                    c0._packed_weights_lat(cin_pad)
                if cin_pad % 16 == 0 and cin_pad >= 32 and c0.out_channels >= min(wino6_min_cout, 32):
                    c0._packed_weights_wino6(cin_pad)
            if len(convs) == 7 and convs[5].weight is not None and convs[5].weight.is_cuda \
                    and tuple(convs[5].weight.shape[:2]) == (16, 32) and tuple(convs[6].weight.shape[:2]) == (5, 16):
                lvl._tail_weights(convs, tail_split and conv_arith == "bf16x3")
        return self

    def invalidate_packed(self):
        for conv in self.modules():
            if isinstance(conv, _Conv3x3SameTF):
                conv.invalidate_packed()
        return self.prepack()

    def weights_stamp(self):
        return tuple((c.weight.data_ptr(), c.weight._version) for c in self.modules()
                     if isinstance(c, _Conv3x3SameTF) and c.weight is not None)

    def load_tf_checkpoint(self, prefix_or_dir, device):
        from . import tf_checkpoint as TC
        prefix = prefix_or_dir
        if _os.path.isdir(prefix_or_dir):
            prefix = TC.latest_checkpoint(prefix_or_dir)
            if prefix is None:
                raise FileNotFoundError(f"no checkpoint state in {prefix_or_dir}")
        return self.load_numpy_weights(TC.load_m4depth_weights(prefix, self.model_settings["nbre_lvls"]), device)

    def numpy_weights(self):
        def hwio(conv):
            return conv.weight.detach().permute(2, 3, 1, 0).cpu().numpy().copy(), conv.bias.detach().cpu().numpy().copy()
        out = {}
        for i in range(self.model_settings["nbre_lvls"]):
            out[f"enc.s1.{i}.kernel"], out[f"enc.s1.{i}.bias"] = hwio(self.encoder.conv_layers_s1[i])
            out[f"enc.s2.{i}.kernel"], out[f"enc.s2.{i}.bias"] = hwio(self.encoder.conv_layers_s2[i])
        dn = self.encoder.dn_layers[0]
        out["enc.dn.0.scale"] = dn.scale.detach().reshape(-1).cpu().numpy().copy()
        out["enc.dn.0.bias"] = dn.bias.detach().reshape(-1).cpu().numpy().copy()
        for lvl in self.d_estimator.levels:
            convs = list(lvl.disp_refiner.prep_conv_layers) + list(lvl.disp_refiner.est_d_conv_layers)
            for i, conv in enumerate(convs):
                out[f"lvl.{lvl.lvl_depth}.conv.{i}.kernel"], out[f"lvl.{lvl.lvl_depth}.conv.{i}.bias"] = hwio(conv)
        return out

    def reset_state(self):
        for lvl in self.d_estimator.levels:
            lvl.reset_state()

    def set_wino6_stagger(self, us):
        for conv in self.modules():
            if isinstance(conv, _Conv3x3SameTF):
                conv.wino6_stagger_us = None if us is None else int(us)
        self.wino6_stagger_us = None if us is None else int(us)
        return self

    def forward(self, data, training=False):
        if training and self.model_settings["is_training"] and torch.is_grad_enabled() \
                and any(p.requires_grad for p in self.parameters()):
            from . import training as TR
            self.step_counter += 1
            return TR.model_forward_train(self, data[0], data[1])
        with torch.no_grad():
            return self._forward_inference(data, training)

    def _forward_inference(self, data, training=False):
        traj_samples, camera = data[0], data[1]
        self.step_counter += 1
        traj_samples = [dict(s, rot=as_f32(s["rot"], "rot"), trans=as_f32(s["trans"], "trans"))
                        if isinstance(s.get("rot"), torch.Tensor) and isinstance(s.get("trans"), torch.Tensor) else s
                        for s in traj_samples]
        n_fr = len(traj_samples)
        dev = camera["f"].device
        late_encoder_fn = self.encoder
        n_maps_pyrs = None
        same_shape = all(s['RGB_im'].shape == traj_samples[0]['RGB_im'].shape for s in traj_samples)
        self.encoder.set_sequence_batch(traj_samples[0]['RGB_im'].shape[0])
        if pipeline_encoder_per_frame and self.d_estimator.pipeline_streams_for(traj_samples, dev) >= 2:
            f_maps_pyrs = None
        elif pipeline_encoder_split > 0 and n_fr > pipeline_encoder_split and same_shape \
                and self.d_estimator.pipeline_streams_for(traj_samples, dev) >= 2:
            k = pipeline_encoder_split
            bsz = traj_samples[0]['RGB_im'].shape[0]
            stats = self.encoder.head_stats(_stack_frames(traj_samples)) if encoder_stats_up_front else None
            if stats is not None:
                head = self.encoder(_stack_frames(traj_samples[:k]), head_stats=(stats[0][:k * bsz], stats[1][:k * bsz]))
                late_stats = (stats[0][k * bsz:], stats[1][k * bsz:])
                late_encoder_fn = lambda images: self.encoder(images, head_stats=late_stats)
            else:
                head = self.encoder(_stack_frames(traj_samples[:k]))
            f_maps_pyrs = [[lvl[t * bsz:(t + 1) * bsz] for lvl in head] for t in range(k)] + [None] * (n_fr - k)
            nhead = None if training else self.d_estimator.prenormalize(head, bsz)
            n_maps_pyrs = [self.d_estimator._frame_slice(nhead, t, bsz) for t in range(k)] + [None] * (n_fr - k)
        elif n_fr > 1 and same_shape:
            bsz = traj_samples[0]['RGB_im'].shape[0]
            stacked = self.encoder(_stack_frames(traj_samples))
            f_maps_pyrs = [[lvl[t * bsz:(t + 1) * bsz] for lvl in stacked] for t in range(n_fr)]
            nst = None if training else self.d_estimator.prenormalize(stacked, bsz)
            n_maps_pyrs = [self.d_estimator._frame_slice(nst, t, bsz) for t in range(n_fr)]
        else:
            f_maps_pyrs = [self.encoder(sample['RGB_im']) for sample in traj_samples]
        d_maps_pyrs = self.d_estimator(f_maps_pyrs, traj_samples, camera, training, encoder=late_encoder_fn,
                                       n_maps_pyrs=n_maps_pyrs)
        self.last_estimates = d_maps_pyrs
        if training:
            return d_maps_pyrs
        h, w = traj_samples[-1]['RGB_im'].shape[1:3]
        return {"depth": _timed("resize", 0, lambda: nops.resize_nearest(d_maps_pyrs[-1][0]["depth"], h, w))}

    def compile(self, metrics=None, optimizer=None, **_unused):
        self.compiled_metrics = list(metrics or [])
        self.optimizer = optimizer

    def m4depth_loss(self, gts, preds):
        from . import training as TR
        return TR.m4depth_loss(gts, preds, self.depth_type)

    def train_step(self, data, grad_sync=None):
        from . import training as TR
        if getattr(self, "optimizer", None) is None:
            raise RuntimeError("train_step: compile the model with an optimizer first")
        return TR.train_step(self, data, self.optimizer, grad_sync)

    def _update_metrics(self, gt_raw, est_raw, max_d=80.):
        from . import metrics as MT
        ms = self.compiled_metrics
        default = (len(ms) == 7 and gt_raw.is_cuda and isinstance(ms[0], MT.AbsRelError) and isinstance(ms[1], MT.SqRelError)
                   and isinstance(ms[2], MT.RootMeanSquaredError) and isinstance(ms[3], MT.RootMeanSquaredLogError)
                   and all(isinstance(ms[4 + i], MT.ThresholdRelError) and ms[4 + i].threshold == i + 1 for i in range(3)))
        if default:
            acc = getattr(self, "_metric_acc", None)
            shared = (acc is not None and acc.device == gt_raw.device and all(
                m.total is not None and m.total.data_ptr() == acc[i].data_ptr() and m.count == ms[0].count
                for i, m in enumerate(ms)))
            if not shared and all(m.total is None for m in ms):
                acc = self._metric_acc = torch.zeros(7, dtype=torch.float32, device=gt_raw.device)
                for i, m in enumerate(ms):
                    m.total = acc[i]
                    m.count = 0
                shared = True
            if shared:
                self._metric_mean = torch.empty(7, dtype=torch.float32, device=gt_raw.device)
                nops.depth_metrics(gt_raw, est_raw, max_d, total=acc, count=ms[0].count + 1, mean=self._metric_mean)
                for m in ms:
                    m.count += 1
                self._metric_mean_count = ms[0].count
            else:
                vals = nops.depth_metrics(gt_raw, est_raw, max_d)
                self._metric_acc = None
                for i, m in enumerate(ms):
                    m._update(vals[i])
            return
        gt = torch.clamp(gt_raw, 0.0, max_d)
        est = torch.clamp(est_raw, 0.001, max_d)
        for m in ms:
            m.update_state(gt, est)

    def _metric_results(self):
        ms = self.compiled_metrics
        acc = getattr(self, "_metric_acc", None)
        if acc is not None and ms and all(m.total is not None and m.total.data_ptr() == acc[i].data_ptr()
                                          and m.count == ms[0].count for i, m in enumerate(ms)):
            if getattr(self, "_metric_mean_count", -1) == ms[0].count and ms[0].count > 0:
                res = self._metric_mean
            else:
                res = acc / float(max(ms[0].count, 1))
            return {m.name: res[i] for i, m in enumerate(ms)}
        return {m.name: m.result() for m in ms}

    @torch.no_grad()
    def test_step(self, data):
        if data["depth"].dim() == 5:
            seq_len = data["depth"].shape[1]
            traj_samples = [{} for _ in range(seq_len)]
            for key in ["depth", "RGB_im", "new_traj", "rot", "trans"]:
                for i, item in enumerate(torch.unbind(data[key], dim=1)):
                    traj_samples[i][key] = item
            preds = self([traj_samples, data["camera"]], training=False)
            gt = data["depth"][:, -1]
            est = preds["depth"]
            new_traj = False
        else:
            preds = self([[data], data["camera"]], training=False)
            gt = data["depth"]
            est = preds["depth"]
            nt = data["new_traj"]
            new_traj = bool(nt.reshape(-1)[0].item()) if isinstance(nt, torch.Tensor) else bool(np.asarray(nt).reshape(-1)[0])
        if not new_traj:
            self._update_metrics(gt, est, 80.)
        return self._metric_results()

    def _stream_inputs(self, frame):
        if self.model_settings["is_training"] or self.d_estimator.is_training:
            raise RuntimeError("stream_step: streaming inference needs a model built with is_training=False")
        if not isinstance(frame, dict):
            raise TypeError("stream_step: expected a dict frame")
        for k in ("RGB_im", "rot", "trans", "new_traj", "camera"):
            if k not in frame:
                raise KeyError(f"stream_step: the frame has no '{k}'")
        rgb = frame["RGB_im"]
        if not isinstance(rgb, torch.Tensor) or rgb.dim() != 4 or rgb.shape[-1] != 3:
            raise ValueError(f"stream_step: RGB_im must be a [b,H,W,3] tensor, got {tuple(getattr(rgb, 'shape', ()))}")
        b = rgb.shape[0]
        want = {"rot": None, "trans": (b, 3), "new_traj": (b,)}
        tensors = {"RGB_im": rgb, "rot": frame["rot"], "trans": frame["trans"], "new_traj": frame["new_traj"],
                   "camera['f']": frame["camera"]["f"], "camera['c']": frame["camera"]["c"]}
        for k, t in tensors.items():
            if not isinstance(t, torch.Tensor):
                raise TypeError(f"stream_step: {k} must be a torch.Tensor")
        rot = frame["rot"]
        if rot.dim() != 2 or rot.shape[0] != b or rot.shape[1] not in (3, 4):
            raise ValueError(f"stream_step: rot must be [b,3] or [b,4] with b = {b}, got {tuple(rot.shape)}")
        for k in ("trans", "new_traj"):
            if tuple(frame[k].shape) != want[k]:
                raise ValueError(f"stream_step: {k} must have shape {want[k]}, got {tuple(frame[k].shape)}")
        if frame["new_traj"].dtype not in (torch.bool, torch.uint8):
            raise TypeError(f"stream_step: new_traj must be bool or uint8, got {frame['new_traj'].dtype}")
        for k in ("f", "c"):
            if tuple(frame["camera"][k].shape) != (b, 2):
                raise ValueError(f"stream_step: camera['{k}'] must have shape ({b}, 2), got {tuple(frame['camera'][k].shape)}")
        for k, t in tensors.items():
            if not t.is_cuda:
                raise RuntimeError(f"stream_step: {k} is on {t.device}; streaming inference runs on the MI355X (no host reads, "
                                   "no CPU fallback): move the frame to the device first")
        return frame

    @torch.no_grad()
    def stream_step(self, frame, out=None, force_reset=False):
        frame = self._stream_inputs(frame)
        self.step_counter += 1
        rgb = frame["RGB_im"]
        b, h, w = rgb.shape[:3]
        self.encoder.set_sequence_batch(b)
        f_pyr = self.encoder(rgb)
        force = self.d_estimator.ensure_stream_state(f_pyr) or bool(force_reset)
        reset, rot, trans = nops.stream_prepare(frame["new_traj"], force, frame["rot"], frame["trans"])
        local_cameras = nops.camera_pyramid(frame["camera"], len(self.d_estimator.levels))
        ests = self.d_estimator.stream_forward(f_pyr, {"rot": rot, "trans": trans}, local_cameras, reset)
        self.last_estimates = [ests]
        self.last_reset_mask = reset
        depth = _timed("resize", 0, lambda: nops.resize_nearest(ests[0]["depth"], h, w, out=out))
        return {"depth": depth, "new_traj": frame["new_traj"]}

    @torch.no_grad()
    def predict_step(self, data):
        preds = self([[data], data["camera"]], training=False)
        return {"image": data["RGB_im"], "depth": preds["depth"], "new_traj": data["new_traj"]}

    def graphed_test_step(self, data, runner):
        est = runner(data)
        self._update_metrics(data["depth"][:, -1], est, 80.)
        return self._metric_results()

    def evaluate(self, dataset):
        for m in self.compiled_metrics:
            m.reset_state()
        out = {}
        for batch in dataset:
            out = self.test_step(batch)
        return [float(out[m.name]) for m in self.compiled_metrics]


class GraphedSequence:

    def __init__(self, model, example, warmup=2, autotune=None):
        self.model = model
        nt = example["new_traj"]
        self.new_traj = nt.clone() if isinstance(nt, torch.Tensor) else torch.as_tensor(np.asarray(nt))
        self._rot = as_f32(example["rot"], "rot").transpose(0, 1).clone(memory_format=torch.contiguous_format)
        self._trans = as_f32(example["trans"], "trans").transpose(0, 1).clone(memory_format=torch.contiguous_format)
        self.static = {"RGB_im": example["RGB_im"].clone(), "rot": self._rot.transpose(0, 1), "trans": self._trans.transpose(0, 1)}
        self.camera = {k: as_f32(v, f"camera[{k}]").clone() for k, v in example["camera"].items()}
        self.seq_len = self.static["RGB_im"].shape[1]
        model.prepack()
        self.stream = torch.cuda.Stream()
        self.stream.wait_stream(torch.cuda.current_stream())
        with torch.cuda.stream(self.stream):
            for _ in range(max(warmup, 1)):
                self._run()
        torch.cuda.current_stream().wait_stream(self.stream)
        torch.cuda.synchronize()
        self.capture_passes = 1
        self.stagger_autotune_ms = None
        batch = int(self.static["RGB_im"].shape[0])
        model_us = getattr(model, "wino6_stagger_us", None)
        base_us = wino6_stagger_us if model_us is None else model_us
        if self.wants_autotune(batch, base_us, autotune):
            self._capture_autotuned(base_us)
        else:
            self.graph, self.depth = self._capture()
            self.stagger_us = base_us if batch <= wino6_stagger_max_batch else 0
        self.weights_stamp = model.weights_stamp()

    @staticmethod
    def wants_autotune(batch, stagger_us, autotune=None):
        want = wino6_stagger_autotune if autotune is None else bool(autotune)
        return bool(want and stagger_us > 0 and batch <= wino6_stagger_max_batch)

    def _capture(self):
        graph = torch.cuda.CUDAGraph()
        with torch.cuda.graph(graph, stream=self.stream):
            out = self._run()
        return graph, out

    def _inspection_state(self):
        lv = self.model.d_estimator.levels
        return (self.model.last_estimates,
                [(l.last_f_input, l.last_cv_inputs, getattr(l, "last_front_inputs", None), l.prev_f_maps) for l in lv])

    def _restore_inspection_state(self, state):
        self.model.last_estimates = state[0]
# ... 447 lines not shown
```

m4depth_amd/network_ops.py:

```python
from __future__ import annotations

import ctypes

import torch

from ._lib import lib, dptr, stream_ptr, check, as_f32


def normalize_cuts(x, nbre_cuts, out=None):
    x = as_f32(x, "x")
    b, h, w, C = x.shape
    if C % nbre_cuts != 0:
        raise ValueError(f"nbre_cuts={nbre_cuts} does not divide the {C} feature channels")
    if out is None:
        out = torch.empty_like(x)
    check(lib.m4d_normalize_cuts(dptr(x, "x"), b, h, w, C, int(nbre_cuts), dptr(out, "out"), stream_ptr()),
          "m4d_normalize_cuts")
    return out


def resize_bilinear_v1(x, out_h, out_w, mul=1.0):
    x = as_f32(x, "x")
    b, ih, iw, c = x.shape
    out = torch.empty((b, out_h, out_w, c), dtype=torch.float32, device=x.device)
# ... 16 lines not shown

def level_pre(prev_l_est, depth_prev_t, trans, camera, b, h, w, device, f_input=None, log_off=0,
              other_off=-1, log_scale=1.0, normalize=None, depth_state_reset=None):
    para = torch.empty((b, h, w, 1), dtype=torch.float32, device=device)
    depth = torch.empty_like(para)
    other = torch.empty((b, h, w, 4), dtype=torch.float32, device=device)
    para_t = torch.empty_like(para) if depth_prev_t is not None else None
    if prev_l_est is not None:
        pd = as_f32(prev_l_est["depth"], "prev_l_est['depth']")
        pp = as_f32(prev_l_est["parallax"], "prev_l_est['parallax']")
        po = as_f32(prev_l_est["other"], "prev_l_est['other']")
        ph, pw = pd.shape[1:3]
    else:
        pd = pp = po = None
        ph = pw = 0
    tr = f = c = None
    if depth_prev_t is not None:
        tr = as_f32(trans, "trans").reshape(b, 3)
        f = as_f32(camera["f"], "camera['f']").reshape(b, 2)
        c = as_f32(camera["c"], "camera['c']").reshape(b, 2)
    f_stride = f_input.shape[-1] if f_input is not None else 0
    if normalize is not None:
        raw, cuts, nout = normalize
        raw = as_f32(raw, "curr_f_maps")
        check(lib.m4d_level_pre_normalize(dptr(pd), dptr(pp), dptr(po), ph, pw, dptr(depth_prev_t, "depth_prev_t"), dptr(tr),
                                          dptr(f), dptr(c), b, h, w, dptr(para), dptr(depth), dptr(other), dptr(para_t),
                                          dptr(f_input, "f_input"), f_stride, int(log_off), int(other_off), float(log_scale),
                                          dptr(depth_state_reset, "depth_state_reset"), dptr(raw, "curr_f_maps"), int(raw.shape[-1]), int(cuts), dptr(nout, "normalised features"),
                                          stream_ptr()), "m4d_level_pre_normalize")
        return para, depth, other, para_t
    check(lib.m4d_level_pre(dptr(pd), dptr(pp), dptr(po), ph, pw, dptr(depth_prev_t, "depth_prev_t"), dptr(tr),
                            dptr(f), dptr(c), b, h, w, dptr(para), dptr(depth), dptr(other), dptr(para_t),
                            dptr(f_input, "f_input"), f_stride, int(log_off), int(other_off), float(log_scale),
                            dptr(depth_state_reset, "depth_state_reset"), stream_ptr()), "m4d_level_pre")
    return para, depth, other, para_t


def pyramid_reset(levels, b):
    from ._lib import ResetLevel
    n = len(levels)
    arr = (ResetLevel * n)()
    ests = []
    pv = 1.0
    for i, lv in enumerate(levels):
        f = as_f32(lv["features"], "curr_f_maps")
        bb, h, w, c = f.shape
        if bb != b:
            raise ValueError("pyramid_reset: batch mismatch")
        para = torch.empty((b, h, w, 1), dtype=torch.float32, device=f.device)
        depth = torch.empty_like(para)
        other = torch.empty((b, h, w, 4), dtype=torch.float32, device=f.device)
        arr[i] = ResetLevel(dptr(f, "curr_f_maps").value, dptr(lv["state_features"], "state_features").value,
                            dptr(lv["depth_state"], "depth_state").value, dptr(para).value, dptr(depth).value, dptr(other).value,
                            h, w, c, int(lv["cuts"]), pv)
        ests.append({"depth": depth, "parallax": para, "other": other})
        pv *= 2.0
    check(lib.m4d_pyramid_reset(arr, n, int(b), stream_ptr()), "m4d_pyramid_reset")
    return ests


def normalize_levels(maps, outs=None):
    from ._lib import NormLevel
    n = len(maps)
    arr = (NormLevel * n)()
    dests, outs = outs, []
    for i, (x, cuts) in enumerate(maps):
        x = as_f32(x, "features")
        out = torch.empty_like(x) if dests is None else dests[i]
        if tuple(out.shape) != tuple(x.shape):
            raise ValueError(f"normalize_levels: destination {i} has shape {tuple(out.shape)}, the map {tuple(x.shape)}")
        arr[i] = NormLevel(dptr(x, "features").value, dptr(out).value, int(x.shape[0] * x.shape[1] * x.shape[2]), int(x.shape[3]), int(cuts))
        outs.append(out)
    check(lib.m4d_normalize_levels(arr, n, stream_ptr()), "m4d_normalize_levels")
    return outs


def _reset_mask(reset, b, depth_state):
    if reset.dtype == torch.bool:
        reset = reset.view(torch.uint8)
    if tuple(reset.shape) != (b,):
        raise ValueError(f"reset mask must have shape ({b},), got {tuple(reset.shape)}")
    if depth_state is None:
        raise ValueError("a masked level close writes the reset samples' depth_state: depth_state is required")
    return dptr(reset, "reset", torch.uint8)


def level_post(refiner_out, rot, trans, camera, scale, depth_state=None, reset=None, reset_parallax=1.0):
    ro = as_f32(refiner_out, "refiner_out")
    b, h, w, five = ro.shape
    if five != 5:
        raise ValueError(f"refiner output must have 5 channels, got {five}")
    rot = as_f32(rot, "rot")
    tr = as_f32(trans, "trans").reshape(b, 3)
    f = as_f32(camera["f"], "camera['f']").reshape(b, 2)
    c = as_f32(camera["c"], "camera['c']").reshape(b, 2)
    para = torch.empty((b, h, w, 1), dtype=torch.float32, device=ro.device)
    depth = torch.empty_like(para)
    other = torch.empty((b, h, w, 4), dtype=torch.float32, device=ro.device)
    if reset is not None:
        rp = _reset_mask(reset, b, depth_state)
        check(lib.m4d_level_post_m(dptr(ro), dptr(rot, "rot"), rot.shape[1], dptr(tr), dptr(f), dptr(c), b, h, w,
                                   float(scale), dptr(para), dptr(depth), dptr(other), dptr(depth_state, "depth_state"),
                                   rp, float(reset_parallax), stream_ptr()), "m4d_level_post_m")
        return para, depth, other
    check(lib.m4d_level_post(dptr(ro), dptr(rot, "rot"), rot.shape[1], dptr(tr), dptr(f), dptr(c), b, h, w,
                             float(scale), dptr(para), dptr(depth), dptr(other), dptr(depth_state, "depth_state"),
                             stream_ptr()), "m4d_level_post")
    return para, depth, other


def bias_act_(x, bias, slope=0.1):
    C = x.shape[-1]
    rows = x.numel() // C
    check(lib.m4d_bias_act(dptr(x, "x"), dptr(bias, "bias"), rows, C, float(slope), dptr(x, "x"), stream_ptr()),
          "m4d_bias_act")
    return x


_ws_cache = {}


def _workspace(key, nbytes, device):
    k = (key, device, torch.cuda.current_stream(device).cuda_stream if device.type == "cuda" else 0)
    ws = _ws_cache.get(k)
    if ws is None or ws.numel() * 4 < nbytes:
        ws = torch.empty((nbytes + 3) // 4, dtype=torch.float32, device=device)
        _ws_cache[k] = ws
    return ws


_zero_ws_cache = {}


def zeroed_workspace(key, shape, device):
    k = (key, tuple(shape), device, torch.cuda.current_stream(device).cuda_stream if device.type == "cuda" else 0)
    buf = _zero_ws_cache.get(k)
    if buf is None:
        buf = torch.zeros(tuple(shape), dtype=torch.float32, device=device)
        _zero_ws_cache[k] = buf
    return buf


def dinl_act(x, scale, bias, slope=1.0, out=None, offset=(0, 0)):
    x = as_f32(x, "x")
    b, h, w, C = x.shape
    ws = _workspace("dinl", 4 * int(lib.m4d_dinl_workspace_floats(b, C)), x.device)
    if out is None:
        out = torch.empty_like(x)
    check(lib.m4d_dinl_fwd_padded(dptr(x, "x"), dptr(scale.reshape(-1), "scale"), dptr(bias.reshape(-1), "bias"),
                                  b, h, w, C, float(slope), dptr(ws), dptr(out, "out"), out.shape[1], out.shape[2],
                                  int(offset[0]), int(offset[1]), stream_ptr()), "m4d_dinl_fwd_padded")
    return out


def bias_act_padded(x, bias, slope, out, offset=(0, 0)):
    b, h, w, C = x.shape
    check(lib.m4d_bias_act_padded(dptr(x, "x"), dptr(bias, "bias"), b, h, w, C, float(slope), dptr(out, "out"),
                                  out.shape[1], out.shape[2], int(offset[0]), int(offset[1]), stream_ptr()),
          "m4d_bias_act_padded")
    return out


def depth_metrics(gt, est, max_d=80.0, total=None, count=0, mean=None):
    est = as_f32(est, "est")
    if gt.numel() != est.numel():
        raise ValueError(f"gt {tuple(gt.shape)} and est {tuple(est.shape)} differ in size")
    ws = _workspace("metrics", int(lib.m4d_metrics_workspace_bytes()), est.device)
    out = torch.empty(7, dtype=torch.float32, device=est.device)
    if (gt.is_cuda and gt.dtype == torch.float32 and gt.dim() >= 2 and not gt.is_contiguous() and gt[0].is_contiguous()
            and gt.stride(0) >= gt[0].numel()):
        check(lib.m4d_depth_metrics_strided(ctypes.c_void_p(gt.data_ptr()), gt[0].numel(), gt.stride(0), dptr(est, "est"),
                                            gt.numel(), float(max_d), dptr(ws), dptr(out), dptr(total, "total"), float(count),
                                            dptr(mean, "mean"), stream_ptr()), "m4d_depth_metrics_strided")
        return out
    gt = as_f32(gt, "gt")
    check(lib.m4d_depth_metrics(dptr(gt, "gt"), dptr(est, "est"), gt.numel(), float(max_d), dptr(ws), dptr(out),
                                dptr(total, "total"), float(count), dptr(mean, "mean"), stream_ptr()), "m4d_depth_metrics")
    return out


def pack_conv_weights(kernel_hwio):
    import numpy as np
    k = np.asarray(kernel_hwio, dtype=np.float32)
    assert k.shape[:2] == (3, 3)
    cin, cout = k.shape[2], k.shape[3]
    nch = -(-cin // 16)
    cpad = -(-cout // 32) * 32
    full = np.zeros((3, 3, nch * 16, cpad), np.float32)
    full[:, :, :cin, :cout] = k
    perm = np.array([0, 2, 4, 6, 8, 10, 12, 14, 1, 3, 5, 7, 9, 11, 13, 15])
    w = full.reshape(9, nch, 16, cpad)[:, :, perm, :]
    return np.ascontiguousarray(w.transpose(1, 0, 3, 2)), cpad


def conv3x3_bias_act(x, wp, bias, cout, cout_pad, slope=0.1, stride=1):
    x = as_f32(x, "x")
    b, h, w, cin = x.shape
    oh, ow = -(-h // stride), -(-w // stride)
    out = torch.empty((b, oh, ow, cout), dtype=torch.float32, device=x.device)
    ws = None
    ws_floats = 0
    if b * oh * ow <= 16384:
        ws_floats = int(lib.m4d_conv3x3_workspace_floats(b, oh, ow, int(cout_pad)))
        ws = _workspace("conv_splitk", 4 * ws_floats, x.device)
    check(lib.m4d_conv3x3s_bias_act_ws(dptr(x, "x"), dptr(wp, "wp"), dptr(bias, "bias"), b, h, w, cin, int(cout),
                                       int(cout_pad), int(stride), float(slope), dptr(out), dptr(ws), ws_floats,
                                       stream_ptr()), "m4d_conv3x3s_bias_act_ws")
    return out


def conv3x3_small_bias_act(x, wp, bias, cout, cout_pad, slope=0.1, stride=1):
    x = as_f32(x, "x")
    b, h, w, cin = x.shape
    out = torch.empty((b, -(-h // stride), -(-w // stride), cout), dtype=torch.float32, device=x.device)
    check(lib.m4d_conv3x3s_small_bias_act(dptr(x, "x"), dptr(wp, "wp"), dptr(bias, "bias"), b, h, w, cin, int(cout),
                                          int(cout_pad), int(stride), float(slope), dptr(out), stream_ptr()),
          "m4d_conv3x3s_small_bias_act")
    return out


_WINO_G = [[1.0, 0.0, 0.0], [0.5, 0.5, 0.5], [0.5, -0.5, 0.5], [0.0, 0.0, 1.0]]


_WINO_SKEW = 64


def pack_conv_weights_winograd(kernel_hwio, chunk=16):
    import numpy as np
    k = np.asarray(kernel_hwio, dtype=np.float64)
    assert k.shape[:2] == (3, 3)
    cin, cout = k.shape[2], k.shape[3]
    G = np.array(_WINO_G, np.float64)
    U = np.einsum('ij,jkco,lk->ilco', G, k, G)
    nch = -(-cin // chunk)
    cpad = -(-cout // 32) * 32
    full = np.zeros((16, nch * chunk, cpad), np.float32)
    full[:, :cin, :cout] = U.reshape(16, cin, cout).astype(np.float32)
    w = np.ascontiguousarray(full.reshape(16, nch, chunk, cpad).transpose(1, 0, 3, 2))
    if chunk == 8:
        skewed = np.zeros((nch, 16, cpad * chunk + _WINO_SKEW), np.float32)
        skewed[:, :, :cpad * chunk] = w.reshape(nch, 16, cpad * chunk)
        return skewed, cpad
    return w, cpad


def conv3x3_wino_bias_act(x, wu, bias, cout, cout_pad, slope=0.1):
    x = as_f32(x, "x")
    b, h, w, cin = x.shape
    out = torch.empty((b, h, w, cout), dtype=torch.float32, device=x.device)
    check(lib.m4d_conv3x3_wino_bias_act(dptr(x, "x"), dptr(wu, "wu"), dptr(bias, "bias"), b, h, w, cin, int(cout),
                                        int(cout_pad), float(slope), dptr(out), stream_ptr()), "m4d_conv3x3_wino_bias_act")
    return out


def conv3x3_wino2_bias_act(x, wu8, bias, cout, cout_pad, slope=0.1):
    x = as_f32(x, "x")
    b, h, w, cin = x.shape
    out = torch.empty((b, h, w, cout), dtype=torch.float32, device=x.device)
    check(lib.m4d_conv3x3_wino2_bias_act(dptr(x, "x"), dptr(wu8, "wu8"), dptr(bias, "bias"), b, h, w, cin, int(cout),
                                         int(cout_pad), float(slope), dptr(out), stream_ptr()), "m4d_conv3x3_wino2_bias_act")
    return out


def split_bf16x3(v):
    import numpy as np

    def bf16_rn(x):
        u = x.view(np.uint32).astype(np.uint64)
        return (((u + 0x7FFF + ((u >> 16) & 1)) >> 16) & 0xFFFF).astype(np.uint16)

    def widen(b):
        return (b.astype(np.uint32) << 16).view(np.float32)
    v = np.ascontiguousarray(v, dtype=np.float32)
    if not np.isfinite(v).all():
        raise ValueError("split_bf16x3: non-finite float32 value (NaN / Inf weights cannot be split into bf16 terms)")
    v = np.where(np.abs(v) < np.float32(2.0 ** -110), np.float32(0.0), v)
    p1 = bf16_rn(v)
    r1 = v - widen(p1)
    p2 = bf16_rn(r1)
    r2 = r1 - widen(p2)
    p3 = bf16_rn(r2)
    if not np.array_equal(widen(p3), r2):
        raise ValueError("split_bf16x3: a float32 value is not the exact sum of three bf16 terms")
    return np.stack([p1, p2, p3])


def pack_conv_weights_wino6(kernel_hwio):
    import numpy as np
    k = np.asarray(kernel_hwio, dtype=np.float64)
    assert k.shape[:2] == (3, 3)
    cin, cout = k.shape[2], k.shape[3]
    G = np.array(_WINO_G, np.float64)
    U = np.einsum('ij,jkco,lk->ilco', G, k, G)
    nch, ng = -(-cin // 16), -(-cout // 64)
    cpad = ng * 64
    full = np.zeros((16, nch * 16, cpad), np.float32)
    full[:, :cin, :cout] = U.reshape(16, cin, cout).astype(np.float32)
    parts = split_bf16x3(full)
    parts = parts.reshape(3, 16, nch, 2, 8, ng, 2, 32)
    w = np.ascontiguousarray(parts.transpose(2, 5, 1, 6, 0, 3, 7, 4))
    return w.reshape(nch, ng, 16, 2, 3, 64, 8), cpad


def pack_conv_weights_small6(kernel_hwio):
    import numpy as np
    k = np.asarray(kernel_hwio, dtype=np.float32)
    assert k.shape[:2] == (3, 3)
    cin, cout = k.shape[2], k.shape[3]
    nch = -(-cin // 16)
    cpad = -(-cout // 32) * 32
    full = np.zeros((9, nch * 16, cpad), np.float32)
    full[:, :cin, :cout] = k.reshape(9, cin, cout)
    parts = split_bf16x3(full).reshape(3, 9, nch, 16, cpad)
    return np.ascontiguousarray(parts.transpose(2, 1, 4, 0, 3)), cpad


def pack_conv_weights_lat(kernel_hwio):
    import numpy as np
    k = np.asarray(kernel_hwio, dtype=np.float32)
    assert k.shape[:2] == (3, 3)
    cin, cout = k.shape[2], k.shape[3]
    nch, ng = -(-cin // 16), -(-cout // 32)
    full = np.zeros((9, nch * 16, ng * 32), np.float32)
    full[:, :cin, :cout] = k.reshape(9, cin, cout)
    parts = split_bf16x3(full).reshape(3, 9, nch, 2, 8, ng, 32)
    return np.ascontiguousarray(parts.transpose(5, 2, 1, 0, 3, 6, 4)).reshape(ng, nch, 9, 3, 64, 8)


class PartialAct:

    def __init__(self, slabs, bias, slope):
        self.slabs, self.bias, self.slope = slabs, bias, 1.0 if slope is None else float(slope)

    @property
    def shape(self):
        return self.slabs.shape[1:]

    @property
    def is_cuda(self):
        return self.slabs.is_cuda

    @property
    def device(self):
        return self.slabs.device

    def dense(self):
        S, b, h, w, C = self.slabs.shape
        out = torch.empty((b, h, w, C), dtype=torch.float32, device=self.slabs.device)
        check(lib.m4d_partial_finish(dptr(self.slabs, "slabs"), S, b * h * w * C, dptr(self.bias, "bias"), self.slope,
                                     b * h * w, C, dptr(out), stream_ptr()), "m4d_partial_finish")
        return out


def _lat_halo_pixels(mt, stride):
    mtx, mty = (2 if mt >= 4 else 1), (2 if mt >= 2 else 1)
    return ((8 * mtx - 1) * stride + 3) * ((4 * mty - 1) * stride + 3)


import os as _os
lat_max_workgroups = int(_os.environ.get("M4D_LAT_MAX_WG", "256"))


def lat_config(b, h, w, cin, cout, final=False, stride=1, mw=False):
    n_chunks, n_groups = -(-cin // 16), -(-cout // 32)
    oh, ow = -(-h // stride), -(-w // stride)
    if mw:
        return 8, 1, 1
    s_out = 1 if final else min(4, n_chunks)
    while s_out > 1 and (s_out - 1) * (-(-n_chunks // s_out)) >= n_chunks:
        s_out -= 1
    cps = -(-n_chunks // s_out)
    kw = 1 if cps <= 1 else (2 if cps <= 2 else 4)

    def wgs(mt, kw):
        mtx, mty = (2 if mt == 4 else 1), (2 if mt >= 2 else 1)
        tiles = b * (-(-oh // (4 * mty))) * (-(-ow // (8 * mtx)))
        return tiles * (-(-n_groups // (4 // kw))) * s_out

    def fits(mt, kw):
        return 2 * kw * _lat_halo_pixels(mt, stride) * 96 <= 160 * 1024
    mt = 1
    while (wgs(mt, kw) > lat_max_workgroups or not fits(mt, kw)) and kw > 1:
        kw //= 2
    while wgs(mt, kw) > lat_max_workgroups and mt < 4 and fits(mt * 2, kw):
        mt *= 2
    return mt, kw, s_out


def conv3x3_lat(x, wp, bias, cout, slope=0.1, final=False, config=None, stride=1):
    if isinstance(x, PartialAct):
        xs, s_in, x_bias, x_slope = x.slabs, x.slabs.shape[0], x.bias, x.slope
        b, h, w, cin = x.shape
        slab = b * h * w * cin
    else:
        xs = as_f32(x, "x")
        s_in, x_bias, x_slope = 1, None, 1.0
        b, h, w, cin = xs.shape
        slab = 0
    mt, kw, s_out = config if config is not None else lat_config(b, h, w, cin, cout, final, stride)
    act = 1.0 if slope is None else float(slope)
    oh, ow = -(-h // stride), -(-w // stride)
    out = torch.empty((s_out, b, oh, ow, cout), dtype=torch.float32, device=xs.device)
    check(lib.m4d_conv3x3s_lat(dptr(xs, "x"), s_in, slab, dptr(x_bias, "x_bias"), float(x_slope), dptr(wp, "wp", torch.int16),
                               dptr(bias, "bias"), b, h, w, cin, int(cout), int(stride), act, mt, kw, s_out, dptr(out),
                               b * oh * ow * int(cout), stream_ptr()), "m4d_conv3x3s_lat")
    return out[0] if s_out == 1 else PartialAct(out, bias, act)


def conv3x3_small6_bias_act(x, wp6, bias, cout, cout_pad, slope=0.1):
    x = as_f32(x, "x")
    b, h, w, cin = x.shape
    out = torch.empty((b, h, w, cout), dtype=torch.float32, device=x.device)
    check(lib.m4d_conv3x3_small6_bias_act(dptr(x, "x"), dptr(wp6, "wp6", torch.int16), dptr(bias, "bias"), b, h, w, cin, int(cout),
                                          int(cout_pad), float(slope), dptr(out), stream_ptr()), "m4d_conv3x3_small6_bias_act")
    return out


def conv3x3_wino6_bias_act(x, wu6, bias, cout, cout_pad, slope=0.1, kernel=0, stagger_us=0, stagger_phases=16):
    x = as_f32(x, "x")
    b, h, w, cin = x.shape
    out = torch.empty((b, h, w, cout), dtype=torch.float32, device=x.device)
    check(lib.m4d_conv3x3_wino6_bias_act_ks(dptr(x, "x"), dptr(wu6, "wu6", torch.int16), dptr(bias, "bias"), b, h, w, cin,
                                            int(cout), int(cout_pad), float(slope), dptr(out), int(kernel), int(stagger_us),
                                            int(stagger_phases), stream_ptr()),
          "m4d_conv3x3_wino6_bias_act_ks")
    return out


class FrameStack:

    def __init__(self, frames):
        if frames.dim() != 5 or frames.dtype != torch.float32 or not frames[0, 0].is_contiguous():
            raise ValueError("FrameStack: expected a float32 [b,T,H,W,3] view with dense frames")
        self.frames = frames

    @property
    def shape(self):
        bsz, t, h, w, c = self.frames.shape
        return (bsz * t, h, w, c)

    @property
    def is_cuda(self):
        return self.frames.is_cuda

    @property
    def device(self):
        return self.frames.device

    def dense(self):
        bsz, t, h, w, c = self.frames.shape
        return self.frames.transpose(0, 1).reshape(bsz * t, h, w, c)


def encoder_head(images, w_hwio, bias1, dn_scale, dn_bias, wp2, bias2, cout2, cout2_pad, slope=0.1):
    if isinstance(images, FrameStack):
        fr = images.frames
        bsz = fr.shape[0]
        stride_b, stride_t = fr.stride(0), fr.stride(1)
        b, h, w, c3 = images.shape
        img_ptr = ctypes.c_void_p(fr.data_ptr())
        if not fr.is_cuda:
            raise RuntimeError("images: m4depth_amd ops run on the MI355X only; there is no CPU fallback")
        images_dev = fr.device
    else:
        images = as_f32(images, "images")
        b, h, w, c3 = images.shape
        bsz, stride_b, stride_t = b, h * w * c3, 0
        img_ptr = dptr(images, "images")
        images_dev = images.device
    if c3 != 3:
        raise ValueError(f"encoder_head expects RGB images, got {c3} channels")
    C = bias1.numel()
    ws = _workspace("dinl", 4 * int(lib.m4d_dinl_workspace_floats(b, C)), images_dev)
    raw = torch.empty((b, h, w, C), dtype=torch.float32, device=images_dev)
    check(lib.m4d_enc_head_fwd(img_ptr, int(bsz), int(stride_b), int(stride_t), dptr(w_hwio, "w_hwio"), dptr(bias1, "bias"),
                               b, h, w, C, dptr(ws), dptr(raw), stream_ptr()), "m4d_enc_head_fwd")
    total = int(lib.m4d_dinl_workspace_floats(b, C))
    mean = ws[total - 2 * b * C: total - b * C]
    var = ws[total - b * C: total]
    oh, ow = -(-h // 2), -(-w // 2)
    out = torch.empty((b, oh, ow, cout2), dtype=torch.float32, device=images_dev)
    check(lib.m4d_conv3x3s2_dinl_bias_act(dptr(raw), dptr(mean), dptr(var), dptr(dn_scale.reshape(-1), "dn_scale"),
                                          dptr(dn_bias.reshape(-1), "dn_bias"), float(slope), dptr(wp2, "wp"), dptr(bias2, "bias"),
                                          b, h, w, int(cout2), int(cout2_pad), float(slope), dptr(out), stream_ptr()),
          "m4d_conv3x3s2_dinl_bias_act")
    return out


def _image_batch_address(images):
    if isinstance(images, FrameStack):
        fr = images.frames
        if not fr.is_cuda:
            raise RuntimeError("images: m4depth_amd ops run on the MI355X only; there is no CPU fallback")
        return ctypes.c_void_p(fr.data_ptr()), fr.shape[0], fr.stride(0), fr.stride(1), tuple(images.shape), fr.device
    images = as_f32(images, "images")
    b, h, w, c3 = images.shape
    return dptr(images, "images"), b, h * w * c3, 0, (b, h, w, c3), images.device


def encoder_level0_stats(images, w1_hwio, bias1):
    img_ptr, bsz, stride_b, stride_t, (b, h, w, c3), dev = _image_batch_address(images)
    if c3 != 3 or bias1.numel() != 16:
        raise ValueError("encoder_level0_stats expects RGB images and a 3->16 convolution")
    ws = _workspace("dinl", 4 * int(lib.m4d_dinl_workspace_floats(b, 16)), dev)
    mean = torch.empty((b, 16), dtype=torch.float32, device=dev)
    var = torch.empty((b, 16), dtype=torch.float32, device=dev)
    check(lib.m4d_enc_level0_stats(img_ptr, int(bsz), int(stride_b), int(stride_t), dptr(w1_hwio, "w1_hwio"), dptr(bias1, "bias1"),
                                   b, h, w, dptr(ws), dptr(mean), dptr(var), stream_ptr()), "m4d_enc_level0_stats")
    return mean, var


def encoder_level0(images, w1_hwio, bias1, dn_scale, dn_bias, w2_hwio, bias2, slope=0.1, stats=None):
    img_ptr, bsz, stride_b, stride_t, (b, h, w, c3), images_dev = _image_batch_address(images)
    if c3 != 3 or bias1.numel() != 16 or bias2.numel() != 16 or tuple(w2_hwio.shape) != (3, 3, 16, 16):
        raise ValueError("encoder_level0 expects RGB images and 3->16 / 16->16 convolutions")
    out = torch.empty((b, -(-h // 2), -(-w // 2), 16), dtype=torch.float32, device=images_dev)
    if stats is not None:
        mean, var = stats
        if tuple(mean.shape) != (b, 16) or tuple(var.shape) != (b, 16):
            raise ValueError(f"encoder_level0: statistics of {tuple(mean.shape)} for {b} images")
        check(lib.m4d_enc_level0_apply(img_ptr, int(bsz), int(stride_b), int(stride_t), dptr(w1_hwio, "w1_hwio"), dptr(bias1, "bias1"),
                                       dptr(mean, "mean"), dptr(var, "var"), dptr(dn_scale.reshape(-1), "dn_scale"),
                                       dptr(dn_bias.reshape(-1), "dn_bias"), float(slope), dptr(w2_hwio, "w2_hwio"),
                                       dptr(bias2, "bias2"), float(slope), b, h, w, dptr(out), stream_ptr()), "m4d_enc_level0_apply")
        return out
    ws = _workspace("dinl", 4 * int(lib.m4d_dinl_workspace_floats(b, 16)), images_dev)
    check(lib.m4d_enc_level0_fwd(img_ptr, int(bsz), int(stride_b), int(stride_t), dptr(w1_hwio, "w1_hwio"), dptr(bias1, "bias1"),
                                 dptr(dn_scale.reshape(-1), "dn_scale"), dptr(dn_bias.reshape(-1), "dn_bias"), float(slope),
                                 dptr(w2_hwio, "w2_hwio"), dptr(bias2, "bias2"), float(slope), b, h, w, dptr(ws), dptr(out),
                                 stream_ptr()), "m4d_enc_level0_fwd")
    return out


def pack_refiner_tail_weights(k6_hwio, k7_hwio):
    import numpy as np
    k6 = np.asarray(k6_hwio, np.float32)
    k7 = np.asarray(k7_hwio, np.float32)
    assert k6.shape == (3, 3, 32, 16) and k7.shape == (3, 3, 16, 5), (k6.shape, k7.shape)
    w6 = np.ascontiguousarray(k6.reshape(9, 32, 16).transpose(0, 2, 1))
    w7 = np.zeros((9, 16, 16), np.float32)
    w7[:, :5, :] = k7.reshape(9, 16, 5).transpose(0, 2, 1)
    return w6, w7


def pack_refiner_tail_weights6(k6_hwio, k7_hwio):
    import numpy as np
    k6 = np.asarray(k6_hwio, np.float32)
    k7 = np.asarray(k7_hwio, np.float32)
    assert k6.shape == (3, 3, 32, 16) and k7.shape == (3, 3, 16, 5), (k6.shape, k7.shape)
    p6 = split_bf16x3(k6.reshape(9, 4, 8, 16))
    w6 = np.ascontiguousarray(p6.transpose(1, 0, 2, 4, 3)).reshape(9, 3, 64, 8)
    full7 = np.zeros((10, 16, 8), np.float32)
    full7[:9, :, :5] = k7.reshape(9, 16, 5)
    p7 = split_bf16x3(full7.reshape(5, 2, 2, 8, 8))
    w7 = np.ascontiguousarray(p7.transpose(1, 0, 2, 3, 5, 4)).reshape(5, 3, 4, 8, 8)
    return w6, w7


def refiner_tail6(x32, w6f, b6, w7f, b7, rot, trans, camera, scale, depth_state=None, reset=None, reset_parallax=1.0):
    x = as_f32(x32, "x32")
    b, h, w, c = x.shape
    if c != 32:
        raise ValueError(f"refiner_tail6 expects the 32-channel refiner activation, got {c} channels")
    rot = as_f32(rot, "rot")
    tr = as_f32(trans, "trans").reshape(b, 3)
    f = as_f32(camera["f"], "camera['f']").reshape(b, 2)
    cc = as_f32(camera["c"], "camera['c']").reshape(b, 2)
    para = torch.empty((b, h, w, 1), dtype=torch.float32, device=x.device)
    depth = torch.empty_like(para)
    other = torch.empty((b, h, w, 4), dtype=torch.float32, device=x.device)
    if reset is not None:
        rp = _reset_mask(reset, b, depth_state)
        check(lib.m4d_refiner_tail6_m(dptr(x, "x32"), dptr(w6f, "w6f", torch.int16), dptr(b6, "b6"), dptr(w7f, "w7f", torch.int16),
                                      dptr(b7, "b7"), dptr(rot, "rot"), rot.shape[1], dptr(tr), dptr(f), dptr(cc), b, h, w, float(scale),
                                      dptr(para), dptr(depth), dptr(other), dptr(depth_state, "depth_state"), rp,
                                      float(reset_parallax), stream_ptr()), "m4d_refiner_tail6_m")
        return para, depth, other
    check(lib.m4d_refiner_tail6(dptr(x, "x32"), dptr(w6f, "w6f", torch.int16), dptr(b6, "b6"), dptr(w7f, "w7f", torch.int16),
                                dptr(b7, "b7"), dptr(rot, "rot"), rot.shape[1], dptr(tr), dptr(f), dptr(cc), b, h, w, float(scale),
                                dptr(para), dptr(depth), dptr(other), dptr(depth_state, "depth_state"), stream_ptr()),
          "m4d_refiner_tail6")
    return para, depth, other


def refiner_tail(x32, w6p, b6, w7p, b7, rot, trans, camera, scale, depth_state=None, reset=None, reset_parallax=1.0):
    x = as_f32(x32, "x32")
    b, h, w, c = x.shape
    if c != 32:
        raise ValueError(f"refiner_tail expects the 32-channel refiner activation, got {c} channels")
    rot = as_f32(rot, "rot")
    tr = as_f32(trans, "trans").reshape(b, 3)
    f = as_f32(camera["f"], "camera['f']").reshape(b, 2)
    cc = as_f32(camera["c"], "camera['c']").reshape(b, 2)
    para = torch.empty((b, h, w, 1), dtype=torch.float32, device=x.device)
    depth = torch.empty_like(para)
    other = torch.empty((b, h, w, 4), dtype=torch.float32, device=x.device)
    if reset is not None:
        rp = _reset_mask(reset, b, depth_state)
        check(lib.m4d_refiner_tail_m(dptr(x, "x32"), dptr(w6p, "w6p"), dptr(b6, "b6"), dptr(w7p, "w7p"), dptr(b7, "b7"),
                                     dptr(rot, "rot"), rot.shape[1], dptr(tr), dptr(f), dptr(cc), b, h, w, float(scale),
                                     dptr(para), dptr(depth), dptr(other), dptr(depth_state, "depth_state"), rp,
                                     float(reset_parallax), stream_ptr()), "m4d_refiner_tail_m")
        return para, depth, other
    check(lib.m4d_refiner_tail(dptr(x, "x32"), dptr(w6p, "w6p"), dptr(b6, "b6"), dptr(w7p, "w7p"), dptr(b7, "b7"),
                               dptr(rot, "rot"), rot.shape[1], dptr(tr), dptr(f), dptr(cc), b, h, w, float(scale),
                               dptr(para), dptr(depth), dptr(other), dptr(depth_state, "depth_state"), stream_ptr()),
          "m4d_refiner_tail")
    return para, depth, other


def camera_pyramid(camera, levels):
    f = as_f32(camera["f"], "camera['f']")
    c = as_f32(camera["c"], "camera['c']")
    b = f.shape[0]
    out = torch.empty((2, levels, b, 2), dtype=torch.float32, device=f.device)
    check(lib.m4d_camera_pyramid(dptr(f.reshape(b, 2), "camera['f']"), dptr(c.reshape(b, 2), "camera['c']"), b, int(levels),
                                 dptr(out[0]), dptr(out[1]), stream_ptr()), "m4d_camera_pyramid")
    return [{"f": out[0, l], "c": out[1, l]} for l in range(levels)]


def stream_prepare(new_traj, force_all, rot, trans):
    rot = as_f32(rot, "rot")
    tr = as_f32(trans, "trans")
    if rot.dim() != 2 or rot.shape[1] not in (3, 4):
        raise ValueError('Rotation must be expressed as a small angle (x,y,z) or a quaternion (w,x,y,z)')
    b = rot.shape[0]
    if tuple(tr.shape) != (b, 3):
        raise ValueError(f"stream_prepare: trans must have shape ({b}, 3), got {tuple(tr.shape)}")
    nt = new_traj.view(torch.uint8) if new_traj.dtype == torch.bool else new_traj
    if tuple(nt.shape) != (b,):
        raise ValueError(f"stream_prepare: new_traj must have shape ({b},), got {tuple(nt.shape)}")
    reset = torch.empty((b,), dtype=torch.uint8, device=rot.device)
    rot_out = torch.empty_like(rot)
    tr_out = torch.empty_like(tr)
    check(lib.m4d_stream_prepare(dptr(nt, "new_traj", torch.uint8), int(bool(force_all)), dptr(rot, "rot"), rot.shape[1],
                                 dptr(tr, "trans"), b, dptr(reset, "reset", torch.uint8), dptr(rot_out), dptr(tr_out), stream_ptr()),
          "m4d_stream_prepare")
    return reset, rot_out, tr_out
```

m4depth_amd/training.py:

```python
from __future__ import annotations

import ctypes

import numpy as np
import torch
import torch.nn.functional as F

from . import network_ops as nops
from ._lib import lib, dptr, stream_ptr, check, as_f32
from .depth_operations import get_parallax_sweeping_cv, cost_volume, prev_d2para, depth2parallax

def _same_pads(h, w, s):
    ph = max((-(-h // s) - 1) * s + 3 - h, 0)
    pw = max((-(-w // s) - 1) * s + 3 - w, 0)
    return ph // 2, ph - ph // 2, pw // 2, pw - pw // 2


def _packed(cache, weight, transpose):
    key = ("bwd" if transpose else "fwd", weight.data_ptr(), weight._version)
    hit = cache.get(key)
    if hit is None:
        O, I = weight.shape[0], weight.shape[1]
        w_ohwi = weight.detach().permute(0, 2, 3, 1).contiguous()
        K, N = (O, I) if transpose else (I, O)
        n_pad = -(-N // 32) * 32
        wp = torch.empty((-(-K // 16), 9, n_pad, 16), dtype=torch.float32, device=weight.device)
        check(lib.m4d_pack_conv_weights(dptr(w_ohwi, "weight"), O, I, int(transpose), dptr(wp), stream_ptr()),
              "m4d_pack_conv_weights")
        hit = (wp, n_pad)
        cache[key] = hit
    return hit


def _packed_lat(cache, weight, transpose):
    key = ("bwd_lat" if transpose else "fwd_lat", weight.data_ptr(), weight._version)
    hit = cache.get(key)
    if hit is None:
        O, I = weight.shape[0], weight.shape[1]
        w_ohwi = weight.detach().permute(0, 2, 3, 1).contiguous()
        K, N = (O, I) if transpose else (I, O)
        hit = torch.empty((-(-N // 32), -(-K // 16), 9, 3, 64, 8), dtype=torch.int16, device=weight.device)
        check(lib.m4d_pack_conv_weights_lat(dptr(w_ohwi, "weight"), O, I, int(transpose), dptr(hit, "wp", torch.int16), stream_ptr()),
              "m4d_pack_conv_weights_lat")
        cache[key] = hit
    return hit


def _lat_ok(b, h, w, cin, stride):
    from . import network as net
    return (stride == 1 and net.conv_arith == "bf16x3" and cin >= 16 and cin % 4 == 0 and b * h * w <= net.lat_conv_max_pixels
            and train_lat_convs)


import os as _os
train_lat_convs = _os.environ.get("M4D_TRAIN_LAT_CONVS", "1") == "1"


class _ConvBiasAct(torch.autograd.Function):

    @staticmethod
    def forward(ctx, x, weight, bias, stride, slope, cache):
        cout = weight.shape[0]
        b, h, w, cin = x.shape
        if _lat_ok(b, h, w, cin, stride):
            out = nops.conv3x3_lat(x, _packed_lat(cache, weight, False), bias.detach(), cout, slope, final=True)
        else:
            wp, n_pad = _packed(cache, weight, False)
            out = nops.conv3x3_bias_act(x, wp, bias.detach(), cout, n_pad, slope, stride=stride)
        ctx.save_for_backward(x, weight, out)
        ctx.cfg = (stride, slope, cache)
        return out

    @staticmethod
    def backward(ctx, g):
        x, weight, out = ctx.saved_tensors
        stride, slope, cache = ctx.cfg
        b, h, w, cin = x.shape
        cout = weight.shape[0]
        oh, ow = out.shape[1:3]
        g = as_f32(g, "grad")
        rows = g.numel() // cout
        gp = torch.empty_like(g)
        g_bias = torch.empty(cout, dtype=torch.float32, device=g.device)
        ws = nops._workspace("bias_bwd", 4 * int(lib.m4d_bias_act_bwd_workspace_floats(rows, cout)), g.device)
        check(lib.m4d_bias_act_bwd(dptr(g, "grad"), dptr(out), rows, cout, float(slope), dptr(gp), dptr(g_bias), dptr(ws),
                                   stream_ptr()), "m4d_bias_act_bwd")
        g = gp
        g_x = None
        if ctx.needs_input_grad[0]:
            zero = cache.get(("zero", cin))
            if zero is None:
                zero = torch.zeros(cin, dtype=torch.float32, device=x.device)
                cache[("zero", cin)] = zero
            gd = g
            if stride == 2:
                gd = torch.empty((b, h, w, cout), dtype=torch.float32, device=g.device)
                check(lib.m4d_dilate2(dptr(g), b, oh, ow, cout, h, w, dptr(gd), stream_ptr()), "m4d_dilate2")
            if _lat_ok(b, h, w, cout, 1) and stride == 1:
                g_x = nops.conv3x3_lat(gd, _packed_lat(cache, weight, True), zero, cin, 1.0, final=True)
            else:
                wp, n_pad = _packed(cache, weight, True)
                g_x = nops.conv3x3_bias_act(gd, wp, zero, cin, n_pad, 1.0, stride=1)
        g_w = None
        if ctx.needs_input_grad[1]:
            g_w = torch.empty_strided(tuple(weight.shape), (9 * cin, 1, 3 * cin, cin), dtype=torch.float32, device=x.device)
            n_ws = int(lib.m4d_conv3x3_wgrad_workspace_floats(b, h, w, cin, cout, stride))
            wsg = nops._workspace("wgrad", 4 * n_ws, x.device)
            check(lib.m4d_conv3x3_wgrad(dptr(x), dptr(g), b, h, w, cin, cout, stride, dptr(wsg), n_ws,
                                        ctypes.c_void_p(g_w.data_ptr()), stream_ptr()), "m4d_conv3x3_wgrad")
        return g_x, g_w, g_bias, None, None, None


def conv_bias_act(conv, x, slope, cache):
    if conv.weight is None:
        conv._build(x.shape[-1], x.device)
    return _ConvBiasAct.apply(as_f32(x, "x"), conv.weight, conv.bias, conv.stride, 1.0 if slope is None else slope, cache)


class _UpsampleV1(torch.autograd.Function):

    @staticmethod
    def forward(ctx, x, h, w, mul):
        ctx.cfg = (tuple(x.shape), h, w, mul)
        return nops.resize_bilinear_v1(x, h, w, mul)

    @staticmethod
    def backward(ctx, g):
        (b, ih, iw, c), h, w, mul = ctx.cfg
        g = as_f32(g, "grad")
        g_in = torch.empty((b, ih, iw, c), dtype=torch.float32, device=g.device)
        check(lib.m4d_resize_bilinear_v1_bwd(dptr(g, "grad"), b, ih, iw, c, h, w, float(mul), dptr(g_in), stream_ptr()),
              "m4d_resize_bilinear_v1_bwd")
        return g_in, None, None, None


def _upsample2_v1(x, h, w, mul=1.0):
    return _UpsampleV1.apply(as_f32(x, "x"), int(h), int(w), float(mul))


class _NormalizeCuts(torch.autograd.Function):

    @staticmethod
    def forward(ctx, x, k):
        ctx.save_for_backward(x)
        ctx.k = k
        return nops.normalize_cuts(x, k)

    @staticmethod
    def backward(ctx, g):
        (x,) = ctx.saved_tensors
        b, h, w, c = x.shape
        g = as_f32(g, "grad")
        gx = torch.empty_like(x)
        check(lib.m4d_normalize_cuts_bwd(dptr(x), dptr(g, "grad"), b, h, w, c, ctx.k, dptr(gx), stream_ptr()),
              "m4d_normalize_cuts_bwd")
        return gx, None


def _normalize_cuts(x, k):
    return _NormalizeCuts.apply(as_f32(x, "x"), int(k))


class _LevelPost(torch.autograd.Function):

    @staticmethod
    def forward(ctx, ro, rot, trans, f, c, scale):
        para, depth, other = nops.level_post(ro, rot, trans, {"f": f, "c": c}, scale)
        ctx.save_for_backward(ro, rot, trans, f, c)
        ctx.scale = scale
        return para, depth, other

    @staticmethod
    def backward(ctx, g_para, g_depth, g_other):
        ro, rot, trans, f, c = ctx.saved_tensors
        b, h, w, _ = ro.shape
        gs = [None if g is None else as_f32(g, "grad") for g in (g_para, g_depth, g_other)]
        g_ro = torch.empty_like(ro)
        check(lib.m4d_level_post_bwd(dptr(ro), dptr(gs[0]), dptr(gs[1]), dptr(gs[2]), dptr(rot, "rot"), rot.shape[1],
                                     dptr(trans), dptr(f), dptr(c), b, h, w, float(ctx.scale), dptr(g_ro), stream_ptr()),
              "m4d_level_post_bwd")
        return g_ro, None, None, None, None, None


class _LevelL1(torch.autograd.Function):

    @staticmethod
    def forward(ctx, pred, gt, velodyne):
        b, h, w, _ = pred.shape
        H, W = gt.shape[1:3]
        ws = nops._workspace("loss", 4 * int(lib.m4d_loss_workspace_floats()), pred.device)
        out2 = torch.empty(2, dtype=torch.float32, device=pred.device)
        check(lib.m4d_loss_level_fwd(dptr(pred, "pred"), dptr(gt, "gt"), b, h, w, H, W, int(velodyne), dptr(ws), dptr(out2),
                                     stream_ptr()), "m4d_loss_level_fwd")
        ctx.save_for_backward(pred, gt, out2)
        ctx.velodyne = velodyne
        return out2[0]

    @staticmethod
    def backward(ctx, g):
        pred, gt, out2 = ctx.saved_tensors
        b, h, w, _ = pred.shape
        H, W = gt.shape[1:3]
        g = as_f32(g, "grad").reshape(1)
        g_pred = torch.empty_like(pred)
        check(lib.m4d_loss_level_bwd(dptr(pred), dptr(gt), dptr(out2), dptr(g, "grad"), b, h, w, H, W, int(ctx.velodyne),
                                     dptr(g_pred), stream_ptr()), "m4d_loss_level_bwd")
        return g_pred, None, None


def level_forward_train(level, curr_f_maps, prev_l_est, rot, trans, camera, prev_f_maps, prev_t_depth, cache):
    b, h, w, c = curr_f_maps.shape
    dev = curr_f_maps.device
    k = level.nbre_cuts
    vp = (lambda t: _normalize_cuts(t, k)) if level.ablation.normalize_features else (lambda t: t)
    curr_f = vp(curr_f_maps)
    if prev_l_est is None:
        para_prev_l = torch.ones((b, h, w, 1), device=dev)
        depth_prev_l = torch.full((b, h, w, 1), 1000., device=dev)
        other_prev_l = torch.zeros((b, h, w, 4), device=dev)
    else:
        other_prev_l = _upsample2_v1(prev_l_est["other"], h, w)
        para_prev_l = _upsample2_v1(prev_l_est["parallax"], h, w, 2.)
        depth_prev_l = _upsample2_v1(prev_l_est["depth"], h, w)
    if prev_t_depth is None:
        return {"depth": depth_prev_l, "parallax": para_prev_l, "other": other_prev_l}
    prev_f = vp(prev_f_maps)
    scale = float(2.0 ** level.lvl_mul)
    with torch.no_grad():
        para_prev_t = prev_d2para(prev_t_depth.detach().contiguous(), rot, trans, camera)
    cv, para_reproj = get_parallax_sweeping_cv(curr_f.contiguous(), prev_f.contiguous(), para_prev_t,
                                               para_prev_l.contiguous(), rot, trans, camera, level.dscv_range,
                                               nbre_cuts=k, cv_accum=level.cv_accum)
    feats = [cv, torch.log(para_prev_l * scale)]
    if level.ablation.level_memory:
        feats.append(other_prev_l)
    if level.ablation.SNCV:
        cf = curr_f.contiguous()
        feats.append(cost_volume(cf, cf, level.sncv_range, nbre_cuts=k))
    if level.ablation.time_recurr:
        r = level.dscv_range
        feats.append(torch.log(para_reproj[..., r:r + 1] * scale))
    x = torch.cat(feats, dim=3)
    convs = list(level.disp_refiner.prep_conv_layers) + list(level.disp_refiner.est_d_conv_layers)
    for i, conv in enumerate(convs):
        x = conv_bias_act(conv, x, 0.1 if i < len(convs) - 1 else None, cache)
    rot_t = as_f32(rot, "rot")
    para_curr, depth, other = _LevelPost.apply(x, rot_t, as_f32(trans, "trans").reshape(b, 3),
                                               as_f32(camera["f"], "f").reshape(b, 2),
                                               as_f32(camera["c"], "c").reshape(b, 2), scale)
    return {"other": other, "depth": depth, "parallax": para_curr}


def dinl_autograd(dn, f_map):
    mean = f_map.mean(dim=(1, 2), keepdim=True)
    centred = f_map - mean
    var = (centred * centred).mean(dim=(1, 2), keepdim=True)
    n = centred / (var + 1e-12)
    ss = (n * n).sum(dim=-1, keepdim=True)
    n = n * torch.rsqrt(torch.clamp_min(ss, 1e-12))
    return dn.scale * n + dn.bias


def encoder_forward_train(encoder, images, cache):
    fm = as_f32(images, "images")
    outs = []
    for i, (c1, c2, dn) in enumerate(zip(encoder.conv_layers_s1, encoder.conv_layers_s2, encoder.dn_layers)):
        if encoder.use_dinl and i == 0:
            t = conv_bias_act(c1, fm, None, cache)
            if dn.scale is None:
                dn._build(t.shape[-1], t.device)
            t = F.leaky_relu(dinl_autograd(dn, t), 0.1)
        else:
            t = conv_bias_act(c1, fm, 0.1, cache)
        fm = conv_bias_act(c2, t, 0.1, cache)
        outs.append(fm)
    return outs


def model_forward_train(model, traj_samples, camera):
    cache = model.__dict__.setdefault("_train_cache", {})
    for key in [k for k in cache if k[0] in ("fwd", "bwd")]:
        del cache[key]
    pyrs = [encoder_forward_train(model.encoder, s["RGB_im"], cache) for s in traj_samples]
    levels = model.d_estimator.levels
    L = len(levels)
    cams = [{"f": as_f32(camera["f"], "f") / 2. ** (lvl + 1), "c": as_f32(camera["c"], "c") / 2. ** (lvl + 1)}
            for lvl in range(L)]
    d_est_seq = []
    for seq_i, (f_pyr, sample) in enumerate(zip(pyrs, traj_samples)):
        d_est_curr = None
        for l in range(L):
            lvl = L - 1 - l
            f_prev = d_prev = None
            if seq_i != 0:
                f_prev = pyrs[seq_i - 1][lvl]
                d_prev = d_est_seq[-1][lvl]["depth"]
            prev = None if d_est_curr is None else dict(d_est_curr[-1])
            est = level_forward_train(levels[lvl], f_pyr[lvl], prev, sample["rot"], sample["trans"], cams[lvl],
                                      f_prev, d_prev, cache)
            d_est_curr = [est] if d_est_curr is None else d_est_curr + [est]
        d_est_seq.append(d_est_curr[::-1])
    return d_est_seq


def m4depth_loss(gts, preds, depth_type="map"):
    l1_loss = 0.
    velodyne = depth_type == "velodyne"
    for gt, pred_pyr in zip(gts[1:], preds[1:]):
        gt_d = as_f32(gt["depth"], "gt depth")
        for i, pred in enumerate(pred_pyr):
            term = _LevelL1.apply(as_f32(pred["depth"], "pred depth"), gt_d, velodyne)
            l1_loss = l1_loss + term * ((0.64 / (2. ** (i - 1))) / float(len(gts) - 1))
    return l1_loss


def unstack_sequence(data):
    T = data["depth"].shape[1]
    out = [{} for _ in range(T)]
    for key in ("depth", "RGB_im", "new_traj", "rot", "trans"):
        for i in range(T):
            out[i][key] = data[key][:, i]
    return out


def set_trainable(model, flag=True):
    for p in model.parameters():
        p.requires_grad_(flag)
    return model


def train_step(model, data, optimizer, grad_sync=None):
    from .metrics import RootMeanSquaredLogError
    traj_samples = unstack_sequence(data)
    with torch.no_grad():
        gts = [{"depth": s["depth"], "parallax": depth2parallax(s["depth"], s["rot"], s["trans"], data["camera"])}
               for s in traj_samples]
    with torch.enable_grad():
        preds = model_forward_train(model, traj_samples, data["camera"])
        loss = m4depth_loss(gts, preds, model.depth_type)
    optimizer.zero_grad(set_to_none=True)
    loss.backward()
    if grad_sync is not None:
        grad_sync([p for g in optimizer.param_groups for p in g["params"]])
    optimizer.step()
    model.step_counter += 1
    with torch.no_grad():
        gt = gts[-1]["depth"]
        est = nops.resize_nearest(preds[-1][0]["depth"].detach().contiguous(), gt.shape[1], gt.shape[2])
        gt_c = torch.clamp(gt, 0.0, 80.)
        est_c = torch.clamp(est, 0.001, 80.)
        if not getattr(model, "compiled_metrics", None):
            model.compiled_metrics = [RootMeanSquaredLogError()]
        for m in model.compiled_metrics:
# ... 58 lines not shown
```

Baseline: 1665.

## Add f16x2 split-precision Winograd conv kernel selectable via conv_arith

```diff
diff --git a/include/m4depth_hip.h b/include/m4depth_hip.h
--- a/include/m4depth_hip.h
+++ b/include/m4depth_hip.h
@@ -80,6 +80,9 @@
 int m4d_conv3x3_wino6_bias_act_ks(const float* x, const void* wu6, const float* bias, int b, int h, int w,
                                   int Cin, int Cout, int CoutPad, float slope, float* out, int kernel,
                                   int stagger_us, int stagger_phases, void* stream);
+int m4d_conv3x3_winof16_bias_act_ks(const float* x, const void* wuh, const float* bias, int b, int h, int w,
+                                    int Cin, int Cout, int CoutPad, float slope, float* out,
+                                    int stagger_us, int stagger_phases, void* stream);
 
 int m4d_refiner_tail(const float* x32, const float* w6p, const float* b6, const float* w7p, const float* b7,
                      const float* rot, int rot_c, const float* trans, const float* cam_f, const float* cam_c,
diff --git a/m4depth_amd/_lib.py b/m4depth_amd/_lib.py
--- a/m4depth_amd/_lib.py
+++ b/m4depth_amd/_lib.py
@@ -88,6 +88,8 @@
     "m4d_conv3x3_wino6_bias_act_k": [_c_fp, _c_fp, _c_fp, _c_int, _c_int, _c_int, _c_int, _c_int, _c_int, _c_f, _c_fp, _c_int, _c_fp],
     "m4d_conv3x3_wino6_bias_act_ks": [_c_fp, _c_fp, _c_fp, _c_int, _c_int, _c_int, _c_int, _c_int, _c_int, _c_f, _c_fp, _c_int,
                                       _c_int, _c_int, _c_fp],
+    "m4d_conv3x3_winof16_bias_act_ks": [_c_fp, _c_fp, _c_fp, _c_int, _c_int, _c_int, _c_int, _c_int, _c_int, _c_f, _c_fp,
+                                        _c_int, _c_int, _c_fp],
     "m4d_enc_head_fwd": [_c_fp, _c_int, ctypes.c_longlong, ctypes.c_longlong, _c_fp, _c_fp, _c_int, _c_int, _c_int, _c_int,
                          _c_fp, _c_fp, _c_fp],
     "m4d_enc_level0_stats": [_c_fp, _c_int, ctypes.c_longlong, ctypes.c_longlong, _c_fp, _c_fp, _c_int, _c_int, _c_int, _c_fp, _c_fp, _c_fp,
diff --git a/m4depth_amd/csrc/m4d_wino_f16.hip b/m4depth_amd/csrc/m4d_wino_f16.hip
--- /dev/null
+++ b/m4depth_amd/csrc/m4d_wino_f16.hip
@@ -0,0 +1,451 @@
+#include <cstdlib>
+#include "m4d_common.h"
+#include "../../include/m4depth_hip.h"
+
+namespace {
+
+typedef float f32x16 __attribute__((ext_vector_type(16)));
+typedef _Float16 f16x8 __attribute__((ext_vector_type(8)));
+typedef unsigned u32x4 __attribute__((ext_vector_type(4)));
+typedef int i32x4 __attribute__((ext_vector_type(4)));
+
+struct WinoF16Args {
+  const float* x; const unsigned char* wu; const short* wexp; const float* bias; float* out;
+  int b, h, w, Cin, Cout, CoutPad, n_chunks, tiles_x, tiles_y;
+  float slope;
+  int phases;
+  int stagger;
+};
+
+constexpr int kT = 16, kH = kT + 2;
+constexpr int kJ = 10;
+constexpr int kPix = 5;
+constexpr int kRow = 2 * kJ * kPix;
+constexpr int kRawUsed = kH * kRow;
+constexpr int kRawDma = 29;
+constexpr int kRawK = 4;
+constexpr int kRawSlots = kRawDma * 64;
+constexpr int kFrag = 4 * 1024;
+constexpr int kBRingBytes = 4 * kFrag;
+constexpr int kBRingOff = 2 * kRawSlots * 16;
+constexpr int kEpiBytes = (4 * 4 * 2 * 32 * 36 + 32) * 4;
+constexpr int kPmOff = kEpiBytes;
+constexpr int kTsOff = kPmOff + kH * kH * 4;
+constexpr int kLdsBytes = kTsOff + 16 * 64 * 4;
+static_assert(kBRingOff + 4 * kBRingBytes <= kEpiBytes, "the K loop's LDS lies inside the epilogue's");
+static_assert(kLdsBytes <= 160 * 1024, "LDS budget of one CU");
+
+__device__ __forceinline__ void split2_pair(float v0, float v1, float S, unsigned& hi, unsigned& lo) {
+  asm("v_fma_mixlo_f16 %0, %1, %2, 0" : "=v"(hi) : "v"(v0), "v"(S));
+  asm("v_fma_mixhi_f16 %0, %1, %2, 0" : "+v"(hi) : "v"(v1), "v"(S));
+  asm("v_fma_mixlo_f16 %0, %1, %2, -%3 op_sel_hi:[0,0,1]" : "=v"(lo) : "v"(v0), "v"(S), "v"(hi));
+  asm("v_fma_mixhi_f16 %0, %1, %2, -%3 op_sel:[0,0,1] op_sel_hi:[0,0,1]" : "+v"(lo) : "v"(v1), "v"(S), "v"(hi));
+}
+
+__device__ __forceinline__ float max3_abs(float m, float a, float b) {
+  asm("v_max3_f32 %0, %0, |%1|, |%2|" : "+v"(m) : "v"(a), "v"(b));
+  return m;
+}
+
+__global__ void __launch_bounds__(512) __attribute__((amdgpu_waves_per_eu(2, 2)))
+conv3x3_winof16_kernel(const WinoF16Args a) {
+  extern __shared__ __align__(16) float lds[];
+  asm volatile("" : : "s"(a.x), "s"(a.wu), "s"(a.out), "s"(a.bias));
+  if (a.stagger > 0 && blockIdx.y == 0 && blockIdx.x < 256) {
+    const unsigned phase = (blockIdx.x >> 3) & (unsigned)(a.phases - 1);
+    const unsigned long long t_end = wall_clock64() + (unsigned long long)(phase * (unsigned)a.stagger) / (unsigned)a.phases;
+    for (int spin = 0; spin < 512 && wall_clock64() < t_end; ++spin) __builtin_amdgcn_s_sleep(16);
+  }
+  float4* raw = reinterpret_cast<float4*>(lds);
+  unsigned* pm = reinterpret_cast<unsigned*>(reinterpret_cast<unsigned char*>(lds) + kPmOff);
+  int* ts = reinterpret_cast<int*>(reinterpret_cast<unsigned char*>(lds) + kTsOff);
+  const unsigned lds_base = (unsigned)(size_t)(__attribute__((address_space(3))) float*)lds;
+
+  const int t = threadIdx.x, lane = t & 63;
+  const int wv = __builtin_amdgcn_readfirstlane(t >> 6);
+  const int pr = wv & 3, mt = wv >> 2;
+  const int m = lane & 31, kh = lane >> 5;
+  const int n_tiles = a.tiles_x * a.tiles_y, n_groups = a.CoutPad / 64;
+  int tile, ng;
+  {
+    const int L = blockIdx.x;
+    if ((n_tiles & 7) == 0) {
+      const int xcd = L & 7, idx = L >> 3;
+      tile = xcd * (n_tiles >> 3) + idx / n_groups;
+      ng = idx % n_groups;
+    } else {
+      tile = L / n_groups;
+      ng = L % n_groups;
+    }
+  }
+  const int tile_y = (tile / a.tiles_x) * kT, tile_x = (tile % a.tiles_x) * kT;
+  const int bi = blockIdx.y;
+  const int n = a.n_chunks, last = n - 1;
+  const float* ximg = a.x + (long long)bi * a.h * a.w * a.Cin;
+
+  i32x4 rsrc;
+  {
+    const unsigned long long xa = (unsigned long long)ximg;
+    rsrc[0] = __builtin_amdgcn_readfirstlane((int)(xa & 0xffffffffull));
+    rsrc[1] = __builtin_amdgcn_readfirstlane((int)((xa >> 32) & 0xffffull));
+    rsrc[2] = a.h * a.w * a.Cin * 4;
+    rsrc[3] = 0x00020000;
+  }
+  unsigned rvoff[kRawK];
+#pragma unroll
+  for (int k = 0; k < kRawK; ++k) {
+    const int i = min(wv + 8 * k, kRawDma - 1);
+    const int s = i * 64 + lane;
+    const int pix = s / kPix, q = s - pix * kPix;
+    const int hy = pix / (2 * kJ), r2 = pix - hy * (2 * kJ);
+    const int e = r2 / kJ, j = r2 - e * kJ;
+    const int hx = 2 * j + e;
+    const int gy = tile_y - 1 + hy, gx = tile_x - 1 + hx;
+    const bool ok = s < kRawUsed && q < 4 && j < 9 && gy >= 0 && gy < a.h && gx >= 0 && gx < a.w;
+    rvoff[k] = ok ? (unsigned)(((gy * a.w + gx) * a.Cin + q * 4) * 4) : 0x80000000u;
+  }
+  auto raw_dma = [&](int chunk, int buf, int k) {
+    const int i = min(wv + 8 * k, kRawDma - 1);
+    const unsigned lds_dst = lds_base + (unsigned)((buf * kRawSlots + i * 64) * 16);
+    asm volatile("s_mov_b32 m0, %1\n\ts_nop 0\n\tbuffer_load_dwordx4 %0, %2, %3 offen lds"
+                 : : "v"(rvoff[k]), "s"(lds_dst), "s"(rsrc), "s"(chunk * 64) : "memory", "m0");
+  };
+
+  const int ra = pr == 0 ? 0 : (pr == 2 ? 2 : 1);
+  const int rb_ = pr == 0 ? 2 : (pr == 1 ? 2 : (pr == 2 ? 1 : 3));
+  const float sgn = pr == 1 ? 1.f : -1.f;
+  const int ty0 = m >> 3, tx = m & 7;
+  const int src0 = (8 * mt + 2 * ty0) * kRow + tx * kPix + 2 * kh;
+
+  float tv[4][8];
+  auto read_t = [&](const float4* rbuf, int c0) {
+#pragma unroll
+    for (int qq = 0; qq < 2; ++qq)
+#pragma unroll
+      for (int cc = 0; cc < 2; ++cc) {
+        const int c = c0 + 2 * cc;
+        const int s = src0 + qq + ((c & 1) * kJ + (c >> 1)) * kPix;
+        const float4 da = rbuf[s + ra * kRow], db = rbuf[s + rb_ * kRow];
+        tv[c][4 * qq + 0] = __builtin_fmaf(sgn, db.x, da.x);
+        tv[c][4 * qq + 1] = __builtin_fmaf(sgn, db.y, da.y);
+        tv[c][4 * qq + 2] = __builtin_fmaf(sgn, db.z, da.z);
+        tv[c][4 * qq + 3] = __builtin_fmaf(sgn, db.w, da.w);
+      }
+  };
+  float Sc[4];
+  auto gen_pair = [&](int c, int e, u32x4 (&A)[2]) {
+    float v[2];
+#pragma unroll
+    for (int h = 0; h < 2; ++h) {
+      const int ch = 2 * e + h;
+      v[h] = c == 0 ? tv[0][ch] - tv[2][ch] : c == 1 ? tv[1][ch] + tv[2][ch] : c == 2 ? tv[2][ch] - tv[1][ch] : tv[1][ch] - tv[3][ch];
+    }
+    unsigned p_hi, p_lo;
+    split2_pair(v[0], v[1], Sc[c], p_hi, p_lo);
+    A[0][e] = p_hi; A[1][e] = p_lo;
+  };
+
+  const long long w_pos = kFrag;
+  const long long w_chunk = (long long)n_groups * 16 * w_pos;
+  const unsigned char* wc = a.wu + ((long long)ng * 16 + 4 * pr) * w_pos;
+  const unsigned bring = lds_base + (unsigned)(kBRingOff + pr * kBRingBytes);
+  const unsigned char* bring_p = reinterpret_cast<const unsigned char*>(lds) + kBRingOff + pr * kBRingBytes;
+  const unsigned bl = (unsigned)lane * 16u;
+  const bool half = __builtin_amdgcn_readfirstlane(ng * 64 + 32 >= a.Cout ? 1 : 0) != 0;
+  const unsigned bl_dma = (half && mt == 1) ? 0u : bl + (unsigned)mt * 2048u;
+  auto b_dma = [&](const unsigned char* gsrc, int slot) {
+    asm volatile("s_mov_b32 m0, %1\n\ts_nop 0\n\t"
+                 "global_load_lds_dwordx4 %0, %2\n\tglobal_load_lds_dwordx4 %0, %2 offset:1024"
+                 : : "v"(bl_dma), "s"(bring + (unsigned)(slot * kFrag) + (unsigned)mt * 2048u), "s"(gsrc) : "memory", "m0");
+  };
+  f16x8 B0[2][2], B1[2];
+  auto frag = [&](int slot, int nt, int part) {
+    return *reinterpret_cast<const f16x8*>(bring_p + slot * kFrag + (nt * 2 + part) * 1024 + bl);
+  };
+#define M4D_WF_WAIT(nn) asm volatile("s_waitcnt vmcnt(" #nn ") lgkmcnt(0)" ::: "memory")
+
+  f32x16 acc[4][2];
+
+#pragma unroll
+  for (int k = 0; k < kRawK; ++k) raw_dma(0, 0, k);
+  b_dma(wc, 0);
+  b_dma(wc + w_pos, 1);
+  b_dma(wc + 2 * w_pos, 2);
+#pragma unroll
+  for (int k = 0; k < kRawK; ++k) raw_dma(min(1, last), 1, k);
+  b_dma(wc + 3 * w_pos, 3);
+  static_assert(kRawK == 4, "the vmcnt counts below assume 4 raw-halo pieces + 2 fragment pieces per position");
+
+  {
+    const int g = t & 7, p0 = t >> 3, nq = a.Cin >> 2;
+    constexpr int kR = (kH * kH + 63) / 64;
+    int poff[kR];
+    bool pv[kR];
+    float mx[kR];
+#pragma unroll
+    for (int r = 0; r < kR; ++r) {
+      const int p = p0 + 64 * r, hy = p / kH, hx = p - hy * kH;
+      const int gy = tile_y - 1 + hy, gx = tile_x - 1 + hx;
+      pv[r] = p < kH * kH && gy >= 0 && gy < a.h && gx >= 0 && gx < a.w;
+      poff[r] = pv[r] ? (gy * a.w + gx) * a.Cin : 0;
+      mx[r] = 0.f;
+    }
+#pragma unroll 2
+    for (int q = g; q < nq; q += 8) {
+#pragma unroll
+      for (int r = 0; r < kR; ++r) {
+        const float4 v = *reinterpret_cast<const float4*>(ximg + poff[r] + 4 * q);
+        mx[r] = max3_abs(max3_abs(mx[r], v.x, v.y), v.z, v.w);
+      }
+    }
+#pragma unroll
+    for (int r = 0; r < kR; ++r) {
+      unsigned u = pv[r] ? min(__float_as_uint(mx[r]), 0x7f7fffffu) : 0u;
+      u = max(u, (unsigned)__builtin_amdgcn_update_dpp(0, (int)u, 0x141, 0xf, 0xf, false));
+      u = max(u, (unsigned)__builtin_amdgcn_update_dpp(0, (int)u, 0xb1, 0xf, 0xf, false));
+      u = max(u, (unsigned)__builtin_amdgcn_update_dpp(0, (int)u, 0x4e, 0xf, 0xf, false));
+      const int p = p0 + 64 * r;
+      if (g == 0 && p < kH * kH) pm[p] = u;
+    }
+  }
+  __syncthreads();
+  {
+    const unsigned* row = pm + 2 * (4 * mt + ty0) * kH + 2 * tx;
+    unsigned cm[4];
+#pragma unroll
+    for (int j = 0; j < 4; ++j) cm[j] = max(row[ra * kH + j], row[rb_ * kH + j]);
+    const unsigned um[4] = {max(cm[0], cm[2]), max(cm[1], cm[2]), max(cm[1], cm[2]), max(cm[1], cm[3])};
+#pragma unroll
+    for (int c = 0; c < 4; ++c) {
+      const int s = min(139 - (int)(um[c] >> 23), 126);
+      Sc[c] = __uint_as_float((unsigned)(s + 127) << 23);
+      if (kh == 0) ts[(pr * 4 + c) * 64 + mt * 32 + m] = -s;
+    }
+  }
+  M4D_WF_WAIT(0);
+  __syncthreads();
+  u32x4 A[2][2];
+
+  auto pin_a = [&](u32x4 (&X)[2]) {
+#pragma unroll
+    for (int part = 0; part < 2; ++part) asm volatile("" : "+v"(X[part]));
+  };
+  auto pin_t = [&](int c0) {
+#pragma unroll
+    for (int cc = 0; cc < 2; ++cc)
+#pragma unroll
+      for (int e = 0; e < 8; ++e) asm volatile("" : "+v"(tv[c0 + 2 * cc][e]));
+  };
+#define M4D_WF_MFMA(c, ap, bv)                                                                                         \
+  _Pragma("unroll") for (int nt = 0; nt < NTL; ++nt)                                                                   \
+    acc[c][nt] = __builtin_amdgcn_mfma_f32_32x32x16_f16(__builtin_bit_cast(f16x8, A[(c) & 1][ap]), bv[nt], acc[c][nt], 0, 0, 0);
+#define M4D_WF_MFMA0(c, ap, bv)                                                                                        \
+  _Pragma("unroll") for (int nt = 0; nt < NTL; ++nt)                                                                   \
+    acc[c][nt] = __builtin_amdgcn_mfma_f32_32x32x16_f16(__builtin_bit_cast(f16x8, A[(c) & 1][ap]), bv[nt],             \
+                                                        FIRST ? f32x16{} : acc[c][nt], 0, 0, 0);
+#define M4D_WF_PIPE(valu)                                                                                              \
+  _Pragma("unroll") for (int i_ = 0; i_ < NTL; ++i_) {                                                                 \
+    __builtin_amdgcn_sched_group_barrier(0x008, 1, 0);                                                                 \
+    __builtin_amdgcn_sched_group_barrier(0x002, (valu) * (2 / NTL), 0);                                                \
+  }
+#define M4D_WF_BLOCK0(c, cn, next_slot, valu, NEXT)                                                                    \
+  if (NEXT) { B0[((c) & 1) ^ 1][0] = frag(next_slot, 0, 0); if (NTL == 2) B0[((c) & 1) ^ 1][1] = frag(next_slot, 1, 0);    \
+              gen_pair(cn, 0, A[((c) & 1) ^ 1]); gen_pair(cn, 1, A[((c) & 1) ^ 1]); }                                    \
+  M4D_WF_MFMA0(c, 1, B0[(c) & 1])                                                                                      \
+  if (NEXT) { asm volatile("" : "+v"(A[((c) & 1) ^ 1][0][0]), "+v"(A[((c) & 1) ^ 1][0][1]),                              \
+                                "+v"(A[((c) & 1) ^ 1][1][0]), "+v"(A[((c) & 1) ^ 1][1][1])); M4D_WF_PIPE(valu) }        \
+  __builtin_amdgcn_sched_barrier(0);
+#define M4D_WF_BLOCK1(c, cn, valu, NEXT)                                                                               \
+  if (NEXT) { gen_pair(cn, 2, A[((c) & 1) ^ 1]); }                                                                     \
+  M4D_WF_MFMA(c, 0, B1)                                                                                                \
+  if (NEXT) { asm volatile("" : "+v"(A[((c) & 1) ^ 1][0][2]), "+v"(A[((c) & 1) ^ 1][1][2])); M4D_WF_PIPE(valu) }        \
+  __builtin_amdgcn_sched_barrier(0);
+#define M4D_WF_BLOCK2(c, cn, next_slot, valu, NEXT)                                                                    \
+  if (NEXT) { B1[0] = frag(next_slot, 0, 1); if (NTL == 2) B1[1] = frag(next_slot, 1, 1);                                \
+              gen_pair(cn, 3, A[((c) & 1) ^ 1]); }                                                                     \
+  M4D_WF_MFMA(c, 0, B0[(c) & 1])                                                                                       \
+  if (NEXT) { pin_a(A[((c) & 1) ^ 1]); M4D_WF_PIPE(valu) }                                                             \
+  __builtin_amdgcn_sched_barrier(0);
+
+  auto k_loop = [&](auto ntl_tag) __attribute__((always_inline)) {
+  constexpr int NTL = decltype(ntl_tag)::value;
+  asm volatile("" ::: "memory");
+  read_t(raw, 0);
+  read_t(raw, 1);
+#pragma unroll
+  for (int nt = 0; nt < NTL; ++nt) { B0[0][nt] = frag(0, nt, 0); B1[nt] = frag(0, nt, 1); }
+#pragma unroll
+  for (int e = 0; e < 4; ++e) gen_pair(0, e, A[0]);
+  asm volatile("s_waitcnt lgkmcnt(0)" ::: "memory");
+  auto chunk_body = [&](int chunk, auto first_tag, auto last_tag) __attribute__((always_inline)) {
+    constexpr bool FIRST = decltype(first_tag)::value != 0, LAST = decltype(last_tag)::value != 0;
+    const unsigned char* wn = chunk < last ? wc + w_chunk : wc;
+    const int rnext_c = min(chunk + 2, last);
+    const float4* rnext = raw + ((chunk + 1) & 1) * kRawSlots;
+    __builtin_amdgcn_s_barrier();
+    M4D_WF_BLOCK0(0, 1, 1, 2, true)
+    if (!LAST) raw_dma(rnext_c, chunk & 1, 0);
+    M4D_WF_BLOCK1(0, 1, 1, true)
+    if (!LAST) b_dma(wn, 0);
+    M4D_WF_BLOCK2(0, 1, 1, 1, true)
+    if (!LAST) M4D_WF_WAIT(6);
+    else M4D_WF_WAIT(3);
+    __builtin_amdgcn_s_barrier();
+    M4D_WF_BLOCK0(1, 2, 2, 2, true)
+    if (!LAST) raw_dma(rnext_c, chunk & 1, 1);
+    M4D_WF_BLOCK1(1, 2, 1, true)
+    if (!LAST) b_dma(wn + w_pos, 1);
+    M4D_WF_BLOCK2(1, 2, 2, 1, true)
+    if (!LAST) M4D_WF_WAIT(6);
+    else M4D_WF_WAIT(0);
+    __builtin_amdgcn_s_barrier();
+    M4D_WF_BLOCK0(2, 3, 3, 2, true)
+    if (!LAST) { raw_dma(rnext_c, chunk & 1, 2); read_t(rnext, 0); }
+    M4D_WF_BLOCK1(2, 3, 5, true)
+    if (!LAST) { b_dma(wn + 2 * w_pos, 2); pin_t(0); }
+    M4D_WF_BLOCK2(2, 3, 3, 5, true)
+    if (!LAST) M4D_WF_WAIT(6);
+    else asm volatile("s_waitcnt lgkmcnt(0)" ::: "memory");
+    __builtin_amdgcn_s_barrier();
+    M4D_WF_BLOCK0(3, 0, 0, 2, !LAST)
+    if (!LAST) { raw_dma(rnext_c, chunk & 1, 3); read_t(rnext, 1); }
+    M4D_WF_BLOCK1(3, 0, 5, !LAST)
+    if (!LAST) { b_dma(wn + 3 * w_pos, 3); pin_t(1); }
+    M4D_WF_BLOCK2(3, 0, 0, 5, !LAST)
+    if (!LAST) M4D_WF_WAIT(6);
+    if (!LAST) wc = wn;
+  };
+  chunk_body(0, m4d_int<1>{}, m4d_int<0>{});
+  if (n > 1) {
+    for (int chunk = 1; chunk < last; ++chunk) chunk_body(chunk, m4d_int<0>{}, m4d_int<0>{});
+    chunk_body(last, m4d_int<0>{}, m4d_int<1>{});
+  }
+  };
+  if (half) k_loop(m4d_int<1>{}); else k_loop(m4d_int<2>{});
+#undef M4D_WF_MFMA
+#undef M4D_WF_MFMA0
+#undef M4D_WF_BLOCK0
+#undef M4D_WF_BLOCK1
+#undef M4D_WF_BLOCK2
+#undef M4D_WF_PIPE
+  M4D_WF_WAIT(0);
+#undef M4D_WF_WAIT
+  __syncthreads();
+
+  const int cq16 = half ? (t & 7) : (t & 15);
+  const int co = ng * 64 + 4 * cq16;
+  float bs[4];
+  int wt[4];
+#pragma unroll
+  for (int e = 0; e < 4; ++e) { bs[e] = a.bias[min(co + e, a.Cout - 1)]; wt[e] = a.wexp[co + e]; }
+  constexpr int kMS = 36;
+  constexpr int kRbMT = 4 * 2 * 32 * kMS;
+  constexpr int kRbSkew = 32;
+  float* Rb = lds;
+  {
+    int4 ne[4][4];
+#pragma unroll
+    for (int c = 0; c < 4; ++c)
+#pragma unroll
+      for (int g4 = 0; g4 < 4; ++g4) ne[c][g4] = *reinterpret_cast<const int4*>(ts + (pr * 4 + c) * 64 + mt * 32 + 8 * g4 + 4 * kh);
+#pragma unroll
+    for (int nt = 0; nt < 2; ++nt) {
+      if (nt == 1 && half) break;
+#pragma unroll
+      for (int c = 0; c < 4; ++c)
+#pragma unroll
+        for (int r = 0; r < 16; ++r) {
+          const int4 q = ne[c][r >> 2];
+          const int ex = (r & 3) == 0 ? q.x : (r & 3) == 1 ? q.y : (r & 3) == 2 ? q.z : q.w;
+          acc[c][nt][r] = __builtin_ldexpf(acc[c][nt][r], ex);
+        }
+    }
+  }
+#pragma unroll
+  for (int nt = 0; nt < 2; ++nt) {
+    if (nt == 1 && half) break;
+    float* rbuf = Rb + (nt * 2 + mt) * kRbMT + nt * kRbSkew;
+#pragma unroll
+    for (int r = 0; r < 16; ++r) {
+      const float m0 = acc[0][nt][r], m1 = acc[1][nt][r], m2 = acc[2][nt][r], m3 = acc[3][nt][r];
+      const int trow = (r & 3) + 8 * (r >> 2) + 4 * kh;
+      rbuf[((pr * 2 + 0) * 32 + trow) * kMS + m] = (m0 + m1) + m2;
+      rbuf[((pr * 2 + 1) * 32 + trow) * kMS + m] = (m1 - m2) - m3;
+    }
+  }
+  __syncthreads();
+  float* oimg = a.out + (long long)bi * a.h * a.w * a.Cout;
+  const bool vec_ok = (a.Cout & 3) == 0;
+  const bool whole = tile_x + kT <= a.w && tile_y + kT <= a.h;
+  const bool fast = whole && vec_ok && ng * 64 + (half ? 32 : 64) <= a.Cout;
+  const int ont = cq16 >> 3, cq = cq16 & 7;
+#pragma unroll
+  for (int it = 0; it < 2; ++it) {
+    if (it == 1 && half) break;
+    const int tl = half ? (t >> 3) & 31 : (t >> 4) & 31, omt = half ? (t >> 8) : it;
+    const float* rbuf = Rb + (ont * 2 + omt) * kRbMT + ont * kRbSkew;
+    const int tg = omt * 32 + tl;
+    const int ty2 = tg >> 3, tx2 = tg & 7;
+    float4 rv[4][2];
+#pragma unroll
+    for (int i = 0; i < 4; ++i)
+#pragma unroll
+      for (int k = 0; k < 2; ++k) rv[i][k] = *reinterpret_cast<const float4*>(rbuf + ((i * 2 + k) * 32 + tl) * kMS + 4 * cq);
+    float y[2][2][4];
+#pragma unroll
+    for (int k = 0; k < 2; ++k) {
+      const float* r0 = reinterpret_cast<const float*>(&rv[0][k]); const float* r1 = reinterpret_cast<const float*>(&rv[1][k]);
+      const float* r2 = reinterpret_cast<const float*>(&rv[2][k]); const float* r3 = reinterpret_cast<const float*>(&rv[3][k]);
+#pragma unroll
+      for (int e = 0; e < 4; ++e) {
+        const int ex = -wt[e];
+        const float v0 = __builtin_ldexpf((r0[e] + r1[e]) + r2[e], ex) + bs[e];
+        const float v1 = __builtin_ldexpf((r1[e] - r2[e]) - r3[e], ex) + bs[e];
+        y[k][0][e] = v0 > 0.f ? v0 : v0 * a.slope;
+        y[k][1][e] = v1 > 0.f ? v1 : v1 * a.slope;
+      }
+    }
+    const int ox = tile_x + 2 * tx2, oy = tile_y + 2 * ty2;
+    float* op = oimg + ((long long)oy * a.w + ox) * a.Cout + co;
+    if (fast) {
+#pragma unroll
+      for (int l = 0; l < 2; ++l)
+#pragma unroll
+        for (int k = 0; k < 2; ++k) m4d_store16(op + ((long long)l * a.w + k) * a.Cout, y[k][l][0], y[k][l][1], y[k][l][2], y[k][l][3]);
+    } else if (co < a.Cout) {
+#pragma unroll
+      for (int l = 0; l < 2; ++l)
+#pragma unroll
+        for (int k = 0; k < 2; ++k)
+          if (ox + k < a.w && oy + l < a.h) {
+            float* o2 = op + ((long long)l * a.w + k) * a.Cout;
+            if (vec_ok && co + 3 < a.Cout) m4d_store16(o2, y[k][l][0], y[k][l][1], y[k][l][2], y[k][l][3]);
+            else { for (int e = 0; e < 4; ++e) if (co + e < a.Cout) o2[e] = y[k][l][e]; }
+          }
+    }
+  }
+}
+
+}
+
+extern "C" int m4d_conv3x3_winof16_bias_act_ks(const float* x, const void* wuh, const float* bias, int b, int h, int w,
+                                               int Cin, int Cout, int CoutPad, float slope, float* out,
+                                               int stagger_us, int stagger_phases, void* stream) {
+  M4D_CHECK_ARG(x && wuh && bias && out && b > 0 && h > 0 && w > 0 && Cin >= 16 && Cout > 0);
+  M4D_CHECK_ARG(CoutPad % 64 == 0 && CoutPad >= Cout && Cin % 16 == 0);
+  M4D_CHECK_ARG(((((uintptr_t)x) & 15u) == 0) && ((((uintptr_t)wuh) & 15u) == 0));
+  M4D_CHECK_ARG((long long)h * w * Cin * 4 < (1ll << 31));
+  M4D_CHECK_ARG(stagger_us >= 0 && stagger_us <= 1000);
+  M4D_CHECK_ARG(stagger_us == 0 || (stagger_phases >= 1 && stagger_phases <= 32 && !(stagger_phases & (stagger_phases - 1))));
+  WinoF16Args a;
+  a.x = x; a.wu = reinterpret_cast<const unsigned char*>(wuh); a.bias = bias; a.out = out;
+  a.b = b; a.h = h; a.w = w; a.Cin = Cin; a.Cout = Cout; a.CoutPad = CoutPad; a.n_chunks = Cin / 16; a.slope = slope;
+  a.wexp = reinterpret_cast<const short*>(a.wu + (long long)a.n_chunks * (CoutPad / 64) * 16 * kFrag);
+  a.tiles_x = (w + kT - 1) / kT; a.tiles_y = (h + kT - 1) / kT;
+  a.stagger = stagger_us * 100;
+  a.phases = stagger_us > 0 ? stagger_phases : 1;
+  const dim3 grid((unsigned)(a.tiles_x * a.tiles_y * (CoutPad / 64)), (unsigned)b);
+  M4D_LDS_OPT_IN(&conv3x3_winof16_kernel);
+  m4d_launch(conv3x3_winof16_kernel, grid, dim3(512), (size_t)kLdsBytes, (hipStream_t)stream, a);
+  return M4D_LAUNCH_RESULT();
+}
diff --git a/m4depth_amd/network.py b/m4depth_amd/network.py
--- a/m4depth_amd/network.py
+++ b/m4depth_amd/network.py
@@ -27,7 +27,8 @@
 winograd2_min_workgroups = int(_os.environ.get("M4D_WINO2_MIN_WG", "60"))
 
 
-conv_arith = _os.environ.get("M4D_CONV_ARITH", "bf16x3")
+conv_arith = _os.environ.get("M4D_CONV_ARITH", "f16x2")
+_SPLIT_ARITHS = ("bf16x3", "f16x2")
 wino6_min_workgroups = int(_os.environ.get("M4D_WINO6_MIN_WG", "30"))
 wino6_kernel = int(_os.environ.get("M4D_WINO6_KERNEL", "0"))
 wino6_pair_min_units = int(_os.environ.get("M4D_WINO6_PAIR_MIN_UNITS", "0"))
@@ -41,7 +42,7 @@
     if _os.environ.get("M4D_WINO6_HALF_MAX_WG"):
         lib.m4d_wino6_set_half_tile_max_workgroups(int(_os.environ["M4D_WINO6_HALF_MAX_WG"]))
 _small_conv_split_env = _os.environ.get("M4D_SMALL_CONV_SPLIT", "1") == "1"
-small_conv_split = _small_conv_split_env and conv_arith == "bf16x3"
+small_conv_split = _small_conv_split_env and conv_arith in _SPLIT_ARITHS
 
 
 tail_split = _os.environ.get("M4D_TAIL_SPLIT", "1") == "1"
@@ -54,10 +55,10 @@
 @_contextlib.contextmanager
 def conv_arithmetic(arith):
     global conv_arith, small_conv_split
-    if arith not in ("bf16x3", "f32"):
-        raise ValueError(f"conv arithmetic must be 'bf16x3' or 'f32', not {arith!r}")
+    if arith not in _SPLIT_ARITHS + ("f32",):
+        raise ValueError(f"conv arithmetic must be 'f16x2', 'bf16x3' or 'f32', not {arith!r}")
     old = (conv_arith, small_conv_split)
-    conv_arith, small_conv_split = arith, _small_conv_split_env and arith == "bf16x3"
+    conv_arith, small_conv_split = arith, _small_conv_split_env and arith in _SPLIT_ARITHS
     try:
         yield
     finally:
@@ -69,7 +70,7 @@
         return 0
     n32 = -(-cout // 32)
     t16 = b * (-(-h // 16)) * (-(-w // 16))
-    if conv_arith == "bf16x3" and cin % 16 == 0 and cin >= 32 and cout >= wino6_min_cout and t16 * (-(-cout // 64)) >= wino6_min_workgroups:
+    if conv_arith in _SPLIT_ARITHS and cin % 16 == 0 and cin >= 32 and cout >= wino6_min_cout and t16 * (-(-cout // 64)) >= wino6_min_workgroups:
         return 6
     if cin % 4 == 0 and t16 * n32 >= winograd2_min_workgroups:
         return 2
@@ -270,7 +271,7 @@
         return self._cache.get(("lat", cin_pad), _stamp(self.weight), build)
 
     def lat_eligible(self, b, h, w, cin):
-        if not (self.small_maps_ok and conv_arith == "bf16x3" and cin >= 16 and cin % 4 == 0 and self.stride in (1, 2)):
+        if not (self.small_maps_ok and conv_arith in _SPLIT_ARITHS and cin >= 16 and cin % 4 == 0 and self.stride in (1, 2)):
             return False
         eff_b = self.dispatch_batch if self.per_image_dispatch else b
         if self.stride == 2:
@@ -292,6 +293,15 @@
             wu, cpad = nops.pack_conv_weights_wino6(self._hwio_numpy(cin_pad))
             return torch.from_numpy(wu.view("int16")).to(self.weight.device), cpad
         return self._cache.get(("wino6", cin_pad), _stamp(self.weight), build)
+
+    def _packed_weights_winof16(self, cin_pad=None):
+        if cin_pad is not None and cin_pad == self.weight.shape[1]:
+            cin_pad = None
+
+        def build():
+            wu, cpad = nops.pack_conv_weights_winof16(self._hwio_numpy(cin_pad))
+            return torch.from_numpy(wu.view("int16")).to(self.weight.device), cpad
+        return self._cache.get(("winof16", cin_pad), _stamp(self.weight), build)
 
     def _hwio_device(self):
         return self._cache.get(("hwio",), _stamp(self.weight), lambda: self.weight.detach().permute(2, 3, 1, 0).contiguous())
@@ -329,16 +339,17 @@
                                                                      stride=self.stride))
         wino = _use_winograd(eff_b, h_, w_, cin_, self.out_channels, self.stride)
         if wino == 6:
-            wu, cpad = self._packed_weights_wino6(cin_)
+            f16 = conv_arith == "f16x2"
+            wu, cpad = self._packed_weights_winof16(cin_) if f16 else self._packed_weights_wino6(cin_)
             stag = self.launch_stagger_us(b_, h_, w_)
             kern = wino6_kernel
-            if kern == 0 and wino6_pair_min_units > 0 and b_ <= wino6_stagger_max_batch and cin_ >= 32:
+            if not f16 and kern == 0 and wino6_pair_min_units > 0 and b_ <= wino6_stagger_max_batch and cin_ >= 32:
                 units = b_ * (-(-h_ // 16)) * (-(-w_ // 16)) * (cpad // 64)
                 if wino6_pair_min_units <= units < int(lib.m4d_wino6_persistent_min_units()):
                     kern = 16 + max(1, min(wino6_pair_units, 15))
             return _timed("conv", self.tag, lambda: nops.conv3x3_wino6_bias_act(
                 x_nhwc, wu, self.bias, self.out_channels, cpad, act, kernel=kern, stagger_us=stag,
-                stagger_phases=wino6_stagger_phases))
+                stagger_phases=wino6_stagger_phases, arith=conv_arith))
         if wino:
             wu, cpad = self._packed_weights_winograd(16 if wino == 1 else 8, cin_)
             fn = nops.conv3x3_wino_bias_act if wino == 1 else nops.conv3x3_wino2_bias_act
@@ -699,7 +710,7 @@
                 x = conv(x, slope=0.1, final=(ci == 4))
                 if debug_tap is not None:
                     debug_tap(f"refiner_conv{ci + 1}", self.lvl_depth, x.dense() if isinstance(x, nops.PartialAct) else x)
-            split = tail_split and conv_arith == "bf16x3"
+            split = tail_split and conv_arith in _SPLIT_ARITHS
             w6p, w7p = self._tail_weights(convs, split)
             tail_fn = nops.refiner_tail6 if split else nops.refiner_tail
             para_curr_l, depth, other = _timed("tail", self.lvl_depth, lambda: tail_fn(
@@ -1024,7 +1035,7 @@
                 conv._packed_weights()
                 if small_conv_split and conv.small_maps_ok and conv.stride == 1 and 16 <= cin <= 256 and cin % 4 == 0:
                     conv._packed_weights_small6()
-                if conv.small_maps_ok and conv_arith == "bf16x3" and cin >= 16 and cin % 4 == 0 and (
+                if conv.small_maps_ok and conv_arith in _SPLIT_ARITHS and cin >= 16 and cin % 4 == 0 and (
                         (conv.stride == 1 and max(lat_conv_max_pixels, lat_conv_narrow_max_pixels) > 0)
                         or (conv.stride == 2 and max(lat_conv_s2_max_pixels, lat_conv_mw_max_pixels) > 0)):
                     conv._packed_weights_lat()
@@ -1036,6 +1047,7 @@
                         conv._packed_weights_winograd(8)
                     if cin % 16 == 0 and cin >= 32 and conv.out_channels >= min(wino6_min_cout, 32):
                         conv._packed_weights_wino6()
+                        conv._packed_weights_winof16()
         for lvl in self.d_estimator.levels:
             convs = list(lvl.disp_refiner.prep_conv_layers) + list(lvl.disp_refiner.est_d_conv_layers)
             c0 = convs[0] if convs else None
@@ -1046,13 +1058,14 @@
                 c0._packed_weights_winograd(8, cin_pad)
                 if small_conv_split and cin_pad <= 256:
                     c0._packed_weights_small6(cin_pad)
-                if conv_arith == "bf16x3" and lat_conv_max_pixels > 0:
+                if conv_arith in _SPLIT_ARITHS and lat_conv_max_pixels > 0:
                     c0._packed_weights_lat(cin_pad)
                 if cin_pad % 16 == 0 and cin_pad >= 32 and c0.out_channels >= min(wino6_min_cout, 32):
                     c0._packed_weights_wino6(cin_pad)
+                    c0._packed_weights_winof16(cin_pad)
             if len(convs) == 7 and convs[5].weight is not None and convs[5].weight.is_cuda \
                     and tuple(convs[5].weight.shape[:2]) == (16, 32) and tuple(convs[6].weight.shape[:2]) == (5, 16):
-                lvl._tail_weights(convs, tail_split and conv_arith == "bf16x3")
+                lvl._tail_weights(convs, tail_split and conv_arith in _SPLIT_ARITHS)
         return self
 
     def invalidate_packed(self):
diff --git a/m4depth_amd/network_ops.py b/m4depth_amd/network_ops.py
--- a/m4depth_amd/network_ops.py
+++ b/m4depth_amd/network_ops.py
@@ -342,6 +342,30 @@
     return w.reshape(nch, ng, 16, 2, 3, 64, 8), cpad
 
 
+def pack_conv_weights_winof16(kernel_hwio):
+    import numpy as np
+    k = np.asarray(kernel_hwio, dtype=np.float64)
+    assert k.shape[:2] == (3, 3)
+    cin, cout = k.shape[2], k.shape[3]
+    G = np.array(_WINO_G, np.float64)
+    U = np.einsum('ij,jkco,lk->ilco', G, k, G)
+    nch, ng = -(-cin // 16), -(-cout // 64)
+    cpad = ng * 64
+    full = np.zeros((16, nch * 16, cpad), np.float32)
+    full[:, :cin, :cout] = U.reshape(16, cin, cout).astype(np.float32)
+    if not np.isfinite(full).all():
+        raise ValueError("pack_conv_weights_winof16: non-finite weight")
+    amax = np.abs(full).max(axis=(0, 1)).astype(np.float64)
+    texp = np.where(amax > 0, 15 - np.frexp(amax)[1], 0).astype(np.int64)
+    scaled = full.astype(np.float64) * np.ldexp(1.0, texp)[None, None, :]
+    hi = scaled.astype(np.float16)
+    lo = (scaled - hi.astype(np.float64)).astype(np.float16)
+    parts = np.stack([hi, lo]).view(np.uint16)
+    parts = parts.reshape(2, 16, nch, 2, 8, ng, 2, 32)
+    w = np.ascontiguousarray(parts.transpose(2, 5, 1, 6, 0, 3, 7, 4))
+    return np.concatenate([w.reshape(-1), texp.astype(np.int16).view(np.uint16)]), cpad
+
+
 def pack_conv_weights_small6(kernel_hwio):
     import numpy as np
     k = np.asarray(kernel_hwio, dtype=np.float32)
@@ -456,7 +480,20 @@
     return out
 
 
-def conv3x3_wino6_bias_act(x, wu6, bias, cout, cout_pad, slope=0.1, kernel=0, stagger_us=0, stagger_phases=16):
+def conv3x3_winof16_bias_act(x, wuh, bias, cout, cout_pad, slope=0.1, stagger_us=0, stagger_phases=16):
+    x = as_f32(x, "x")
+    b, h, w, cin = x.shape
+    out = torch.empty((b, h, w, cout), dtype=torch.float32, device=x.device)
+    check(lib.m4d_conv3x3_winof16_bias_act_ks(dptr(x, "x"), dptr(wuh, "wuh", torch.int16), dptr(bias, "bias"), b, h, w, cin,
+                                              int(cout), int(cout_pad), float(slope), dptr(out), int(stagger_us),
+                                              int(stagger_phases), stream_ptr()),
+          "m4d_conv3x3_winof16_bias_act_ks")
+    return out
+
+
+def conv3x3_wino6_bias_act(x, wu6, bias, cout, cout_pad, slope=0.1, kernel=0, stagger_us=0, stagger_phases=16, arith="bf16x3"):
+    if arith == "f16x2":
+        return conv3x3_winof16_bias_act(x, wu6, bias, cout, cout_pad, slope, stagger_us=stagger_us, stagger_phases=stagger_phases)
     x = as_f32(x, "x")
     b, h, w, cin = x.shape
     out = torch.empty((b, h, w, cout), dtype=torch.float32, device=x.device)
diff --git a/m4depth_amd/training.py b/m4depth_amd/training.py
--- a/m4depth_amd/training.py
+++ b/m4depth_amd/training.py
@@ -48,7 +48,7 @@
 
 def _lat_ok(b, h, w, cin, stride):
     from . import network as net
-    return (stride == 1 and net.conv_arith == "bf16x3" and cin >= 16 and cin % 4 == 0 and b * h * w <= net.lat_conv_max_pixels
+    return (stride == 1 and net.conv_arith in net._SPLIT_ARITHS and cin >= 16 and cin % 4 == 0 and b * h * w <= net.lat_conv_max_pixels
             and train_lat_convs)
 
 
```

Measured after the change: 1759, median of 6. 1.06x the previous value.
